# SegataLab/metamlst

Hardware: AMD Instinct MI355X
Metric: Mreads/s aligned+ST-typed, metamlstDB_2022; ST concordance vs CPU ref (higher is better)
Workload: dtype int32

## Files before the change

include/mlst.h:

```cpp
#ifndef MLST_H
#define MLST_H

#include <stdint.h>

#ifdef __cplusplus
extern "C" {
#endif

#define MLST_OK              0
#define MLST_E_INVALID      -1
#define MLST_E_NOGPU        -2
#define MLST_E_HIP          -3
#define MLST_E_CAPACITY     -4
#define MLST_E_LIMIT        -5

typedef struct mlst_handle mlst_handle;

typedef struct mlst_params {
    int32_t minscore;
    int32_t max_xm;
    int32_t min_read_len;
    int32_t minqual;
    int32_t mincov;
    int32_t match_bonus;
// ... 77 lines not shown
                           uint32_t words_per_read, uint32_t qual_stride);

int mlst_submit_packed_device(mlst_handle* h, const uint32_t* d_packed, const uint8_t* d_qual_rows,
                              const uint16_t* d_lens, uint64_t n_reads,
                              uint32_t words_per_read, uint32_t qual_stride, int paired);

int mlst_get_allele_stats(mlst_handle* h, int64_t* sum_score, uint32_t* n_hits,
                          uint64_t* locus_read_len_sum, uint64_t* locus_first_read,
                          uint64_t* counters);

int mlst_stats_flat_sizes(mlst_handle* h, uint64_t* n_sum, uint64_t* n_min);
int mlst_export_stats_device(mlst_handle* h, int64_t* d_sum, int64_t* d_min);
int mlst_import_stats_device(mlst_handle* h, const int64_t* d_sum, const int64_t* d_min);

int mlst_pileup(mlst_handle* h, const uint32_t* chosen_allele_idx, uint32_t n, uint32_t* counts);
int mlst_pileup_device(mlst_handle* h, const uint32_t* chosen_allele_idx, uint32_t n,
                       uint32_t* d_counts , uint64_t* n_cols);
int mlst_set_depth_cap(mlst_handle* h, uint32_t cap);

int mlst_consensus(mlst_handle* h, const uint32_t* chosen_allele_idx, uint32_t n, uint32_t mincov,
                   char none_char, uint8_t* out_seq, uint32_t* counts);

int mlst_consensus_from_counts_device(mlst_handle* h, const uint32_t* d_counts, uint64_t n_cols, uint32_t mincov,
                                      char none_char, uint8_t* out_seq);

int mlst_pileup_alignments(mlst_handle* h, const uint32_t* chosen_allele_idx, uint32_t n_chosen, uint64_t n_rec,
                           const uint32_t* rec_allele, const int32_t* rec_pos0, const int32_t* rec_as, const int32_t* rec_xm,
                           const uint64_t* cigar_off, const uint32_t* cigar, const uint64_t* seq_off,
                           const uint8_t* seq, const uint8_t* qual, int32_t minscore, int32_t max_xm, int32_t minqual,
                           uint32_t* counts);

int mlst_alignments_export(mlst_handle* h, const uint32_t* chosen_allele_idx, uint32_t n,
                           uint64_t* n_rec_out, uint64_t* n_cigar_out, uint64_t* n_bases_out);
int mlst_alignments_fetch(mlst_handle* h, uint64_t* read_index, uint32_t* rec_allele, int32_t* rec_pos0, int32_t* rec_as,
                          int32_t* rec_xm, int32_t* rec_diag, uint8_t* rec_flags ,
                          uint64_t* cigar_off , uint32_t* cigar, uint64_t* seq_off ,
                          uint8_t* seq, uint8_t* qual);

int mlst_alignments_text_open(mlst_handle* h, const uint8_t* names, const uint64_t* name_off , int paired,
                              uint64_t round_bytes );
int mlst_alignments_text_next(mlst_handle* h, uint8_t* text, uint64_t cap, uint64_t* n_bytes, uint64_t* n_records, int* done);
int mlst_alignments_text_close(mlst_handle* h);

int mlst_reads_text_open(mlst_handle* h, int paired, uint64_t round_bytes );
int mlst_reads_text_next(mlst_handle* h, uint8_t* text, uint64_t cap, uint64_t* n_bytes, uint64_t* n_reads, int* done);
int mlst_reads_text_close(mlst_handle* h);

int mlst_set_read_names(mlst_handle* h, int on);
int mlst_get_read_names(mlst_handle* h, int* on);
int mlst_read_names_info(mlst_handle* h, uint64_t out[4]);
int mlst_read_names_fetch(mlst_handle* h, uint64_t* read_index , uint64_t* off , uint8_t* bytes);

typedef struct { uint32_t trim5, trim3, trim_qual, phred_base; } mlst_read_prep;
int mlst_set_read_prep(mlst_handle* h, const mlst_read_prep* p);
int mlst_get_read_prep(mlst_handle* h, mlst_read_prep* out);
int mlst_read_prep_info(mlst_handle* h, uint64_t out[4]);

int mlst_set_read_adapters(mlst_handle* h, const char* adapters, uint32_t min_overlap, uint32_t error_permille);
int mlst_get_read_adapters(mlst_handle* h, char* adapters, uint64_t cap, uint32_t* min_overlap, uint32_t* error_permille);
int mlst_get_read_adapters_info(mlst_handle* h, uint64_t out[12]);

int mlst_set_export_md(mlst_handle* h, int on);
int mlst_get_export_md(mlst_handle* h, int* on);

int mlst_bam_open(mlst_handle* h, int pass, const int32_t* ref_allele, const int32_t* ref_locus, const uint8_t* ref_flags, uint32_t n_ref,
                  uint32_t skip_bytes, const uint32_t* chosen_allele_idx, uint32_t n_chosen);
int mlst_submit_bam_bgzf(mlst_handle* h, const uint8_t* data, uint64_t n_bytes, int final_chunk, uint64_t* n_records_out, uint64_t* n_consumed_out);
int mlst_bam_set_capacity(mlst_handle* h, uint64_t max_entries);
int mlst_bam_pileup_fetch(mlst_handle* h, uint32_t* counts);

int mlst_sam_open(mlst_handle* h, int pass, const uint8_t* names, const uint64_t* name_off ,
                  const int32_t* ref_allele, const int32_t* ref_locus, const uint8_t* ref_flags, uint32_t n_ref,
                  const uint32_t* chosen_allele_idx, uint32_t n_chosen);
int mlst_submit_sam_text(mlst_handle* h, const uint8_t* text, uint64_t n_bytes, int final_chunk, uint64_t* n_records_out);

int mlst_bam_reads_open(mlst_handle* h, uint32_t n_ref, uint32_t skip_bytes, int paired);
int mlst_bam_reads_info(mlst_handle* h, uint64_t out[4]);

int mlst_submit_fasta(mlst_handle* h, const uint8_t* text, uint64_t n_bytes, uint32_t read_len, uint32_t stride, uint32_t min_len,
                      uint64_t* n_contigs_out, uint64_t* n_reads_out);

int mlst_typing_layout(mlst_handle* h, uint64_t* colbase , uint64_t* total_cols);
int mlst_typing_enqueue(mlst_handle* h, int32_t penalty, uint32_t mincov, char none_char);
int mlst_typing_choose_pileup(mlst_handle* h, int32_t penalty, uint32_t* d_counts);
int mlst_typing_finish(mlst_handle* h, uint32_t mincov, char none_char, const uint32_t* d_counts);
int mlst_typing_choose_pileup_compact(mlst_handle* h, int32_t penalty, uint32_t* d_counts, uint64_t cap_cols);
int mlst_typing_finish_compact(mlst_handle* h, uint32_t mincov, char none_char, const uint32_t* d_counts);
int mlst_typing_compact_info(mlst_handle* h, uint64_t* need_cols, uint32_t* overflow);
int mlst_typing_fetch(mlst_handle* h, int64_t* sum_score, uint32_t* n_hits, uint64_t* locus_read_len_sum,
                      uint64_t* locus_first_read, uint64_t* counters, int32_t* chosen, uint8_t* letters);
int mlst_typing_wait(mlst_handle* h);
int mlst_typing_fetch_waited(mlst_handle* h, int64_t* sum_score, uint32_t* n_hits, uint64_t* locus_read_len_sum,
                             uint64_t* locus_first_read, uint64_t* counters, int32_t* chosen, uint8_t* letters);
long long mlst_round_tenths(long long p, uint32_t q);

int mlst_hamming_le(mlst_handle* h, uint32_t locus, const uint8_t* query, uint32_t len,
                    uint32_t z, int32_t* first_allele_idx, uint32_t* n_within);
int mlst_hamming_all(mlst_handle* h, uint32_t locus, const uint8_t* query, uint32_t len,
                     uint32_t* dist);

int mlst_msa_align(mlst_handle* h, const uint8_t* seqs, const uint64_t* off , uint32_t n, uint32_t* center_out, uint32_t* width_out);
int mlst_msa_fetch(mlst_handle* h, uint8_t* rows );

int mlst_set_read_index_base(mlst_handle* h, uint64_t base);

int mlst_reset_sample(mlst_handle* h);

typedef struct mlst_item {
    uint64_t read_index;
    uint32_t locus;
    int32_t  diag;
    uint16_t strand;
    uint16_t votes;
    uint32_t reserved;
} mlst_item;
int mlst_get_items(mlst_handle* h, mlst_item* out, uint64_t cap, uint64_t* n);

int mlst_set_stream(mlst_handle* h, void* stream);
int mlst_set_cu_partition(mlst_handle* h, uint32_t part, uint32_t n_parts);
int mlst_get_stream(mlst_handle* h, void** stream);
int mlst_busy(mlst_handle* h);
int mlst_export_stats_device_async(mlst_handle* h, int64_t* d_sum, int64_t* d_min);
int mlst_import_stats_device_async(mlst_handle* h, const int64_t* d_sum, const int64_t* d_min);

int mlst_set_profiling(mlst_handle* h, int on);
int mlst_get_kernel_time(mlst_handle* h, int which, double* total_ms, uint64_t* launches);
int mlst_reset_kernel_time(mlst_handle* h);
int mlst_get_index_bytes(mlst_handle* h, uint64_t out[4]);
int mlst_get_sieve_info(mlst_handle* h, uint64_t out[4]);
int mlst_get_extend_info(mlst_handle* h, uint64_t out[8]);
int mlst_synchronize(mlst_handle* h);

#ifdef __cplusplus
}
#endif
#endif
```

metamlst_amd/csrc/mlst_engine.hip:

```cpp
#include <hip/hip_runtime.h>
#include <algorithm>
#include <cmath>
#include <cstdarg>
#include <cstdio>
#include <cstdlib>
#include <cstring>
#include <cstddef>
#include <functional>
#include <atomic>
#include <memory>
#include <mutex>
#include <string>
#include <thread>
#include <vector>
#include <chrono>
#include <unistd.h>

#include "mlst.h"
#include "mlst_debug.h"
#include "bgzf_host.h"
#include "inflate_dev.h"
#include "inflate_wave.h"
#include "inflate_lane.h"
#include "inflate_canon.h"
// ... 3079 lines not shown
        else if (i < 2 * nA) E.n_hits[i - nA] = (u32)d_sum[i];
        else if (i < 2 * nA + nL) E.locus_len[i - 2 * nA] = (u64)d_sum[i];
        else if (i < total) E.ctr->cnt[i - 2 * nA - nL] = (u64)d_sum[i];
        else { u64 l = i - total; long long f = d_min[l]; E.locus_first[l] = f == 0x7FFFFFFFFFFFFFFFll ? 0xFFFFFFFFFFFFFFFFull : (u64)f; }
    }
}
__global__ void k_fill_u64(u64* p, u64 n, u64 v) {
    for (u64 i = (u64)blockIdx.x * blockDim.x + threadIdx.x; i < n; i += (u64)gridDim.x * blockDim.x) p[i] = v;
}

#include "bam_dev.h"
#include "sam_dev.h"
#include "bam_reads.h"
#include "fasta_dev.h"
#include "fastq_tile.h"
#include "bam_tile.h"
#include "msa_dev.h"
#include "aln_export.h"
#include "read_names.h"
#include "read_prep.h"
#include "read_adapt.h"
#include "aln_text.h"
#include "reads_text.h"

struct EvPair { hipEvent_t a, b; int which; };

struct mlst_handle {
    int device = 0;
    hipStream_t stream = nullptr;
    mlst_params prm;
    KParams kp;
    std::string err;
    std::vector<LocusDev> loci;
    std::vector<u64> aoff;
    u32 n_alleles = 0, n_loci = 0;
    std::vector<u32> allele_locus;
    u32* d_arena = nullptr; u32* d_planes = nullptr; u32* d_nmask = nullptr; u16* d_allele_len = nullptr; u32* d_allele_locus = nullptr;
    LocusDev* d_loci = nullptr; uint4* d_sieve = nullptr; u32* d_bitmap = nullptr; u32* d_gbitmap = nullptr; u64* d_keys = nullptr; u32* d_vals = nullptr; u32* d_posts = nullptr;
    int* d_floor = nullptr; u8* d_pen = nullptr; u8* d_ascii = nullptr; u64* d_aoff = nullptr;
    HapRec* d_hap_rec = nullptr; u32* d_hap_blk = nullptr; u32* d_hap_id = nullptr; u64 bytes_hap = 0, n_hap_rec = 0; u32 hap_win_max[2] = {0, 0}, hap_loci = 0;
    u32 ext_lds_recs[2] = {0, 0};
    u32 ext_acc_cap = 0;
    u8* h_qc = nullptr; u8* d_qc = nullptr; u64 cap_hostq = 0, cap_qc = 0;
    u64* d_acc64 = nullptr;
    u32* d_xrec[2] = {nullptr, nullptr}; u64 cap_xrec[2] = {0, 0};
    u64 bytes_arena = 0, bytes_sieve = 0, bytes_table = 0; double bitmap_fill = 0.0;
    EngineDev E; EngineDev* d_E = nullptr;
    bool have_ref = false, have_state = false;
    u32* d_cand = nullptr; u64 cap_cand = 0;
    int sieve_kind = 0; u32 sieve_chain = 0; u64 n_keys = 0;
    u32* d_rfilter = nullptr; u32* d_rt_arena = nullptr; u64 cap_rt_arena = 0; u32* d_rt_counts = nullptr; u32* d_rt_emitted = nullptr; u64 cap_rt_emitted = 0;
    u32 rt_prod = 0, rt_cap = 0, rt_tiles_max = 0, rt_nw = 16, rt_pf = 2, rt_exam = RT_EXAM_DEFAULT, rt_wo = 1; u64 rt_slice = 0;
    u64* d_rt_parked = nullptr; u64 cap_rt_parked = 0;
    u64* d_rt_trace = nullptr; bool rt_trace_on = false; const void* rt_last_packed = nullptr;
    std::vector<void*> dbg_pads;
    u32* d_bin_flags = nullptr; u64 cap_bin_flags = 0;
    u8* d_in_bases = nullptr; u8* d_in_quals = nullptr; u64* d_in_off = nullptr; u64 cap_in_bytes = 0, cap_in_reads = 0;
    u32* d_packed = nullptr; u8* d_qrows = nullptr; u16* d_lens = nullptr; u64 cap_packed_words = 0, cap_qrow_bytes = 0, cap_lens = 0;
    u64 reads_seen = 0;
    u32 max_wpr = 0;
    int ext_threads = 64, ext_blocks = 5120;
    int extp_threads = 256, extp_blocks = 1792; u32 pair_loci = 0;
    int sieve_g_blocks = 256 * 5;
    u8* d_fq_text = nullptr;
    u32* d_fq_blk = nullptr; u64 cap_fq_blk = 0;
    u8* d_bgzf = nullptr; u64 cap_bgzf = 0; void* d_bgzf_blk = nullptr; u64 cap_bgzf_blk = 0; u8* d_fq_carry = nullptr; u64 cap_fq_carry = 0, fq_carry_len = 0;
    u64* d_fq_lines = nullptr; u64 cap_fq_lines = 0; u64* d_fq_soff = nullptr; u64* d_fq_qoff = nullptr; u64 cap_fq_reads = 0; u64* d_fq_meta = nullptr;
    int* d_locus_chosen = nullptr; u64* d_locus_colbase = nullptr; u64* d_pl_list = nullptr; u8* d_tb = nullptr;
    u32* d_itok = nullptr; u32* d_intok = nullptr; u64 cap_itok_blocks = 0; int inflate_mode = 0;
    u64 dbg_infl_blocks = 0, dbg_infl_left = 0; bool dbg_infl_known = false;
    struct BlkList { BgzfBlk* d = nullptr; BgzfBlk* h = nullptr; u64 cap = 0; };
    struct BzSlot { BlkList blk; hipEvent_t ev_copied = nullptr, ev_inflated = nullptr; u32* d_err = nullptr; u32* h_err = nullptr; };
    BzSlot bz[2]; int bz_slot = 0, bz_mode = -1; hipStream_t infl_stream = nullptr;
    bool bgzf_verify = false; struct { u32* d_out = nullptr; hipEvent_t e0 = nullptr, e1 = nullptr; } crc_hook;
    enum { BZ_SUB = 8 };
    struct BzChunk { u8* d = nullptr; u64 cap = 0; hipEvent_t ev[BZ_SUB] = {}; u64 upto[BZ_SUB] = {}; int n_ev = 0; hipEvent_t ev_used = nullptr; bool used = false; };
    BzChunk bzc[2]; int bz_chunk = 0;
    struct { bool on = false, counted = false; int slot = 0, tslot = 0, paired = 0; u64 text_bytes = 0; u32 blk_base = 0 ; } bz_pend;
    u8* d_pc[2] = {nullptr, nullptr}; u64 cap_pc[2] = {0, 0}, pc_len[2] = {0, 0}; bool pair_open = false; u64* d_pr_meta = nullptr;
    struct BzPair { bool on = false, counted = false; int slot = 0, tslot = 0; u32 nblk1 = 0; u64 base[2] = {0, 0}, head[2] = {0, 0}, text[2] = {0, 0}; } bzp;
    u32 depth_cap = 0; u64* d_capbuf = nullptr; u64 cap_capcols = 0;
    u32* d_counts = nullptr; u64 cap_counts = 0;
    int* d_allele_no = nullptr; int* d_auto_chosen = nullptr; u64* d_fixed_colbase = nullptr; std::vector<u64> fixed_colbase; u64 fixed_cols = 0;
    u32* d_auto_counts = nullptr; u8* d_auto_letters = nullptr; bool auto_pending = false;
    u8* h_tstats[2] = {nullptr, nullptr}; u8* h_tauto[2] = {nullptr, nullptr}; int t_slot = 0, t_last = 0, t_ready = -1;
    u64* d_compact_colbase = nullptr; int* d_compact_chosen = nullptr; u64* d_compact_info = nullptr; u64 off_compact_info = 0; bool compact_pending = false;
    hipStream_t copy_stream = nullptr; hipEvent_t stage_done = nullptr;
    u8* d_fq_slot[2] = {nullptr, nullptr}; u64 cap_fq_slot[2] = {0, 0}; hipEvent_t ev_packed[2] = {nullptr, nullptr}; int fq_slot = 0;
    u32* d_fq_nl[2] = {nullptr, nullptr};
    int cu_split = 1, cu_part = 0;
    hipStream_t own_stream = nullptr;
    u32* d_dist = nullptr; u8* d_query = nullptr; u64 cap_dist = 0, cap_query = 0;
    u8* d_stats = nullptr; u8* h_stats = nullptr; u64 stats_bytes = 0, stats_zero_bytes = 0;
    u64 off_sum = 0, off_len = 0, off_ctr = 0, off_hits = 0, off_first = 0;
    u8* h_pin = nullptr; u64 cap_pin = 0;
    bool profiling = false;
    bool window = false;
    struct GraphSlot { hipGraphExec_t exec = nullptr; std::vector<u64> sig; };
    GraphSlot g_submit, g_typing; bool use_graphs = true;
    std::vector<EvPair> events;
    std::vector<hipEvent_t> ev_pool;
    double k_ms[20] = {0}; u64 k_n[20] = {0};
    double wall_khz = 100000.0;
    struct BamStream* bam = nullptr;
    u32 bam_force_miss = 0; u64 bam_max_entries = 0;
    struct { u64 n_reads = 0; u32 wpr = 0, qstride = 0; } last_pack;
    struct { FaDev* d_desc = nullptr; FaMeta* d_meta = nullptr; u8* h_fa = nullptr; u8* d_flat = nullptr; u64 cap_flat = 0;
             u32* d_kind = nullptr; u64* d_cseq = nullptr; u64* d_chdr = nullptr; u64 cap_cells = 0; u64* d_cstart = nullptr; u64* d_wcnt = nullptr; u64 cap_contigs = 0;
             u64 last_cells = 0, last_contigs = 0; u32 last_passes = 0; } fa;
    struct { u32 read_len = 0, stride = 0; u64 round = 16ull << 20; u64 info[4] = {0, 0, 0, 0};
             FqtDev* d_desc = nullptr; FqtMeta* d_meta = nullptr; u8* h_fqt = nullptr; u64* d_rlen = nullptr; u64* d_wex = nullptr; u64 cap_recs = 0;
             u64* d_gsum = nullptr; u64 cap_groups = 0; u64* d_soff = nullptr; u64* d_qoff = nullptr; u64 cap_win = 0; } tile;
    struct { u64 batch_bytes = 1ull << 30; bool done = false; u32 n = 0, width = 0;
             u8* d_seq = nullptr; u64 cap_seq = 0; u64* d_off = nullptr; u64 cap_off = 0; u16* d_tab = nullptr; u64 cap_tab = 0;
             u32* d_slot = nullptr; u8* d_end = nullptr; u64 cap_end = 0; u32* d_tb = nullptr; u64 cap_tb = 0; u8* d_rows = nullptr; u64 cap_rows = 0;
             u32* h_width = nullptr; } msa;
    struct { bool done = false; u64 n_rec = 0, n_cig = 0, n_seq = 0; int* d_lc = nullptr; u64 cap_lc = 0; AxItem* d_meta = nullptr; u64* d_dp = nullptr;
             u64* d_off = nullptr; u64 cap_items = 0; u64* d_gs = nullptr; u64 cap_groups = 0; u8* d_desc = nullptr; u8* h_tot = nullptr;
             u8* d_out = nullptr; u64 cap_out = 0; AxOut out; } ax;
    struct AtState { bool open = false, ready = false, with_names = false, md = false, with_md = false, reads = false; u64 max_reads = 0; u16* d_mdw = nullptr; size_t next = 0; std::vector<AtRound> rounds; u64 round_bytes = 0, round_recs = 0, max_pairs = 0;
             u32* d_perm = nullptr; u64* d_pair_off = nullptr; u32* d_item_read = nullptr; u64* d_read_first = nullptr; u8* d_names = nullptr; u64* d_name_off = nullptr;
             AtPair* d_meta = nullptr; AtRead* d_reads = nullptr; u64* d_wex = nullptr; u64* d_gsum = nullptr; u64* d_dp = nullptr; u8* d_desc = nullptr;
             u8* d_text = nullptr; u64 cap_text = 0; u8* h_tot = nullptr; } at;
    struct { bool on = false; u64 want_bytes = 256ull << 20; RnCtr* d_ctr = nullptr; u8* d_bytes = nullptr; u64 cap_bytes = 0; u64* d_off = nullptr; u16* d_len = nullptr;
             RnSrc src = {nullptr, nullptr, 0}; } rn;
    struct { bool on = false; RpSet set = {0, 0, 0, 33}; RpCtr* d_ctr = nullptr; } rp;
    struct { bool on = false; RaSet set = {}; std::string text; RaCtr* d_ctr = nullptr; } ra;
};

static std::string g_create_err;

static int fail(mlst_handle* h, int code, const char* fmt, ...) {
    char buf[512]; va_list ap; va_start(ap, fmt); vsnprintf(buf, sizeof buf, fmt, ap); va_end(ap);
    if (h) h->err = buf; else g_create_err = buf;
    return code;
}
#define HIPCHK(h, call) do { hipError_t e_ = (call); if (e_ != hipSuccess) return fail(h, MLST_E_HIP, "%s: %s", #call, hipGetErrorString(e_)); } while (0)

static int bz_flush(mlst_handle* h);
static int bzp_finish(mlst_handle* h, bool whole, uint64_t* n_reads_out);
static void bz_free(mlst_handle* h);
static int bam_flush(mlst_handle* h);
static void bam_drop(mlst_handle* h, bool release);
static bool bam_is_open(const mlst_handle* h);
static int rn_refuse(mlst_handle* h, const char* entry);
static int rp_refuse(mlst_handle* h, const char* entry);
static int ra_refuse(mlst_handle* h, const char* entry);
static void at_free(mlst_handle* h);
static const char* bam_kind(const mlst_handle* h);
template <typename T> static hipError_t dmalloc(T** p, u64 n) { return hipMalloc((void**)p, (n ? n : 1) * sizeof(T)); }
template <typename T> static hipError_t dmalloc(GP<T>* p, u64 n) { return hipMalloc((void**)&p->p, (n ? n : 1) * sizeof(T)); }

static hipEvent_t ev_get(mlst_handle* h) {
    if (!h->ev_pool.empty()) { hipEvent_t e = h->ev_pool.back(); h->ev_pool.pop_back(); return e; }
    hipEvent_t e; if (hipEventCreateWithFlags(&e, hipEventDisableSystemFence) != hipSuccess) hipEventCreate(&e); return e;
}
__global__ void k_nop() {}
struct Prof {
    mlst_handle* h; int which; hipEvent_t a = nullptr, b = nullptr;
    Prof(mlst_handle* h_, int w) : h(h_), which(w) {
        if (h->profiling) { a = ev_get(h); b = ev_get(h); hipLaunchKernelGGL(k_nop, dim3(1), dim3(64), 0, h->stream); hipEventRecord(a, h->stream); }
    }
    ~Prof() { if (h->profiling) { hipEventRecord(b, h->stream); h->events.push_back({a, b, which}); } }
};
static void drain_events(mlst_handle* h) {
    if (h->events.empty()) return;
    hipStreamSynchronize(h->stream);
    for (auto& e : h->events) { float ms = 0; hipEventElapsedTime(&ms, e.a, e.b); h->k_ms[e.which] += ms; h->k_n[e.which]++; h->ev_pool.push_back(e.a); h->ev_pool.push_back(e.b); }
    h->events.clear();
}

static int graph_enter(mlst_handle* h, mlst_handle::GraphSlot& g, const std::vector<u64>& sig) {
    if (!h->use_graphs || h->profiling || h->stream != h->own_stream) return 0;
    if (g.exec && g.sig == sig) return hipGraphLaunch(g.exec, h->stream) == hipSuccess ? 1 : 0;
    if (g.exec) { hipGraphExecDestroy(g.exec); g.exec = nullptr; }
    if (g.sig != sig) { g.sig = sig; return 0; }
    if (hipStreamBeginCapture(h->stream, hipStreamCaptureModeThreadLocal) != hipSuccess) { h->use_graphs = false; return 0; }
    return 2;
}
static int graph_leave(mlst_handle* h, mlst_handle::GraphSlot& g) {
    hipGraph_t graph = nullptr;
    if (hipStreamEndCapture(h->stream, &graph) != hipSuccess || !graph) { h->use_graphs = false; return fail(h, MLST_E_HIP, "hipStreamEndCapture failed"); }
    hipError_t e = hipGraphInstantiate(&g.exec, graph, nullptr, nullptr, 0);
    hipGraphDestroy(graph);
    if (e != hipSuccess) { g.exec = nullptr; h->use_graphs = false; return fail(h, MLST_E_HIP, "hipGraphInstantiate: %s", hipGetErrorString(e)); }
    HIPCHK(h, hipGraphLaunch(g.exec, h->stream));
    return MLST_OK;
}

extern "C" void mlst_default_params(mlst_params* p) {
    memset(p, 0, sizeof *p);
    p->minscore = MLST_DEF_MINSCORE; p->max_xm = MLST_DEF_MAX_XM; p->min_read_len = MLST_DEF_MIN_READ_LEN;
    p->minqual = MLST_DEF_MINQUAL; p->mincov = MLST_DEF_MINCOV; p->match_bonus = MLST_DEF_MATCH_BONUS;
    p->mm_max = MLST_DEF_MM_MAX; p->mm_min = MLST_DEF_MM_MIN; p->n_penalty = MLST_DEF_N_PENALTY;
    p->gap_open = MLST_DEF_GAP_OPEN; p->gap_ext = MLST_DEF_GAP_EXT; p->gbar = MLST_DEF_GBAR; p->band_w = MLST_DEF_BAND_W;
    p->gap_trigger_mm = MLST_DEF_GAP_TRIGGER_MM; p->xm_field_quirk = MLST_DEF_XM_FIELD_QUIRK; p->gap_trigger_clip = MLST_DEF_GAP_TRIGGER_CLIP;
    p->minscore_const = MLST_DEF_MINSCORE_CONST; p->minscore_coef = MLST_DEF_MINSCORE_COEF;
}

extern "C" const char* mlst_last_error(const mlst_handle* h) { return h ? h->err.c_str() : g_create_err.c_str(); }

extern "C" int mlst_create(int device, const mlst_params* p, mlst_handle** out) {
    if (!out) return fail(nullptr, MLST_E_INVALID, "out is NULL");
    *out = nullptr;
    int ndev = 0;
    if (hipGetDeviceCount(&ndev) != hipSuccess || ndev <= 0)
        return fail(nullptr, MLST_E_NOGPU, "no HIP device visible: this library has no CPU path");
    if (device < 0 || device >= ndev) return fail(nullptr, MLST_E_INVALID, "device %d out of range (%d devices)", device, ndev);
    mlst_params prm; if (p) prm = *p; else mlst_default_params(&prm);
    if (prm.band_w < 1 || prm.band_w > MAX_W) return fail(nullptr, MLST_E_INVALID, "band_w must be in 1..%d", MAX_W);
    if (prm.max_xm > 254 || prm.minscore > 1000) return fail(nullptr, MLST_E_INVALID, "max_xm/minscore out of range");
    if (prm.match_bonus < 1 || prm.match_bonus > 127) return fail(nullptr, MLST_E_INVALID, "match_bonus must be in 1..127");
    {
        const int pmin = std::min(prm.n_penalty, prm.mm_min), gap1 = prm.gap_open + prm.gap_ext;
        if (pmin < 0 || prm.mm_max < prm.mm_min || prm.gap_open < 0 || prm.gap_ext < 0) return fail(nullptr, MLST_E_INVALID, "penalties must not be negative, mm_max not below mm_min");
        if (prm.match_bonus * MLST_MAX_READ_LEN >= 1024)
            return fail(nullptr, MLST_E_LIMIT, "match_bonus %d: the score of a %d-base read does not fit 10 bits", prm.match_bonus, MLST_MAX_READ_LEN);
        if (prm.match_bonus > 4 * pmin)
            return fail(nullptr, MLST_E_LIMIT, "match_bonus %d against a cheapest mismatch of %d: xm of a %d-base read does not fit 8 bits", prm.match_bonus, pmin, MLST_MAX_READ_LEN);
        if (5 * prm.match_bonus > 2 * gap1)
            return fail(nullptr, MLST_E_LIMIT, "match_bonus %d against a one-base gap of %d: xo of a %d-base read does not fit 7 bits", prm.match_bonus, gap1, MLST_MAX_READ_LEN);
    }
    if (!prm.max_retained_reads) prm.max_retained_reads = 4ull << 20;
    if (!prm.max_items) prm.max_items = 8ull << 20;
    if (prm.max_items >= (1ull << 32)) return fail(nullptr, MLST_E_INVALID, "max_items must be below 2^32");
    if (!prm.max_pair_results) prm.max_pair_results = 256ull << 20;
    mlst_handle* h = new mlst_handle();
    h->device = device; h->prm = prm;
    if (hipSetDevice(device) != hipSuccess) { delete h; return fail(nullptr, MLST_E_HIP, "cannot initialise device %d", device); }
    if (hipStreamCreate(&h->stream) != hipSuccess) { delete h; return fail(nullptr, MLST_E_HIP, "cannot initialise device %d", device); }
    h->own_stream = h->stream;
    { const char* g = getenv("MLST_GRAPHS"); if (g && g[0] == '0') h->use_graphs = false; }
    { const char* g = getenv("MLST_BGZF_CRC"); h->bgzf_verify = g && g[0] == '1'; }
    { const char* g = getenv("MLST_MSA_BATCH_BYTES"); if (g && atoll(g) > 0) h->msa.batch_bytes = (u64)atoll(g); }
    { const char* g = getenv("MLST_TILE_ROUND"); if (g && atoll(g) > 0) h->tile.round = (u64)atoll(g); }
    { const char* g = getenv("MLST_NAMES_BYTES"); if (g && atoll(g) > 0) h->rn.want_bytes = (u64)atoll(g); }
    { int khz = 0; if (hipDeviceGetAttribute(&khz, hipDeviceAttributeWallClockRate, device) == hipSuccess && khz > 0) h->wall_khz = (double)khz; }
    KParams& k = h->kp;
    k.minscore = prm.minscore; k.max_xm = prm.max_xm; k.min_read_len = prm.min_read_len; k.minqual = prm.minqual;
    k.match_bonus = prm.match_bonus; k.n_penalty = prm.n_penalty;
    k.open_p = ((prm.gap_open + prm.gap_ext) << MLST_P_SHIFT) + (1 << 8); k.ext_p = prm.gap_ext << MLST_P_SHIFT;
    k.gbar = prm.gbar; k.band_w = prm.band_w; k.trig = prm.gap_trigger_mm; k.quirk = prm.xm_field_quirk; k.clip = prm.gap_trigger_clip;
    memset(&h->E, 0, sizeof h->E);
    *out = h;
    return MLST_OK;
}

static void free_ref(mlst_handle* h) {
    hipFree(h->d_arena); hipFree(h->d_planes); hipFree(h->d_nmask); hipFree(h->d_allele_len); hipFree(h->d_allele_locus); hipFree(h->d_loci);
    hipFree(h->d_sieve); hipFree(h->d_bitmap); h->d_bitmap = nullptr; hipFree(h->d_gbitmap); h->d_gbitmap = nullptr; hipFree(h->d_keys); hipFree(h->d_vals); hipFree(h->d_posts); hipFree(h->d_floor); hipFree(h->d_pen);
    hipFree(h->d_ascii); hipFree(h->d_aoff);
    hipFree(h->d_hap_rec); hipFree(h->d_hap_blk); hipFree(h->d_hap_id); h->d_hap_rec = nullptr; h->d_hap_blk = nullptr; h->d_hap_id = nullptr;
    hipFree(h->d_rfilter); h->d_rfilter = nullptr;
    hipFree(h->d_allele_no); hipFree(h->d_auto_chosen); hipFree(h->d_fixed_colbase); hipFree(h->d_auto_counts); hipFree(h->d_auto_letters);
    hipFree(h->d_compact_colbase); hipFree(h->d_compact_chosen); hipFree(h->d_compact_info); h->d_compact_colbase = nullptr; h->d_compact_chosen = nullptr; h->d_compact_info = nullptr;
    for (int k = 0; k < 2; k++) if (h->h_tauto[k]) { hipHostFree(h->h_tauto[k]); h->h_tauto[k] = nullptr; }
    h->d_allele_no = h->d_auto_chosen = nullptr; h->d_fixed_colbase = nullptr; h->d_auto_counts = nullptr; h->d_auto_letters = nullptr; h->auto_pending = false;
    h->d_arena = h->d_planes = h->d_nmask = nullptr; h->d_allele_len = nullptr; h->d_allele_locus = nullptr; h->d_loci = nullptr; h->d_sieve = nullptr;
    h->d_keys = nullptr; h->d_vals = h->d_posts = nullptr; h->d_floor = nullptr; h->d_pen = nullptr; h->d_ascii = nullptr; h->d_aoff = nullptr;
    h->have_ref = false;
}
static void free_state(mlst_handle* h) {
    EngineDev& E = h->E;
    hipFree(h->d_bin_flags); h->d_bin_flags = nullptr; h->cap_bin_flags = 0;
    hipFree(h->d_rt_arena); hipFree(h->d_rt_counts); hipFree(h->d_rt_emitted); hipFree(h->d_rt_trace); h->d_rt_trace = nullptr;
    hipFree(h->d_rt_parked); h->d_rt_parked = nullptr; h->cap_rt_parked = 0;
    for (void* q : h->dbg_pads) hipFree(q);
    h->dbg_pads.clear();
    h->d_rt_arena = nullptr; h->d_rt_counts = nullptr; h->d_rt_emitted = nullptr; h->cap_rt_arena = 0; h->cap_rt_emitted = 0; h->rt_prod = 0;
    hipFree(h->d_E); h->d_E = nullptr;
    hipFree(h->d_stats); h->d_stats = nullptr; if (h->h_stats) { hipHostFree(h->h_stats); h->h_stats = nullptr; }
    for (int k = 0; k < 2; k++) if (h->h_tstats[k]) { hipHostFree(h->h_tstats[k]); h->h_tstats[k] = nullptr; }
    hipFree(E.ret_bases); hipFree(E.ret_quals); hipFree(E.ret_len); hipFree(E.ret_ridx); hipFree(E.ret_nrec);
    hipFree(E.ret_mate); hipFree(E.ret_item0); hipFree(E.ret_nitems); hipFree(E.ret_cpos); E.ret_mate = nullptr; E.ret_item0 = nullptr; E.ret_nitems = nullptr; E.ret_cpos = nullptr;
    hipFree(E.items); hipFree(E.item_state); hipFree(E.res); hipFree(E.dp_list);
    for (int k = 0; k < 2; k++) { hipFree(h->d_xrec[k]); h->d_xrec[k] = nullptr; h->cap_xrec[k] = 0; }
    hipFree(h->d_acc64); h->d_acc64 = nullptr;
    hipFree(h->rn.d_ctr); hipFree(h->rn.d_bytes); hipFree(h->rn.d_off); hipFree(h->rn.d_len);
    h->rn.d_ctr = nullptr; h->rn.d_bytes = nullptr; h->rn.d_off = nullptr; h->rn.d_len = nullptr; h->rn.cap_bytes = 0;
    hipFree(h->d_qc); h->d_qc = nullptr; h->cap_qc = 0; if (h->h_qc) { hipHostFree(h->h_qc); h->h_qc = nullptr; h->cap_hostq = 0; }
    hipFree(h->d_locus_chosen); hipFree(h->d_locus_colbase); hipFree(h->d_pl_list); hipFree(h->d_tb);
    hipFree(h->d_capbuf); h->d_capbuf = nullptr; h->cap_capcols = 0;
    hipFree(h->d_itok); hipFree(h->d_intok); h->d_itok = nullptr; h->d_intok = nullptr; h->cap_itok_blocks = 0;
    E.sum_score = nullptr; E.n_hits = nullptr; E.locus_len = E.locus_first = nullptr; E.ctr = nullptr; E.ret_bases = nullptr; E.ret_quals = nullptr;
    E.ret_len = nullptr; E.ret_ridx = nullptr; E.ret_nrec = nullptr; E.items = nullptr; E.item_state = nullptr; E.res = nullptr; E.dp_list = nullptr;
    h->d_locus_chosen = nullptr; h->d_locus_colbase = nullptr; h->d_pl_list = nullptr; h->d_tb = nullptr;
    h->have_state = false;
}

extern "C" void mlst_destroy(mlst_handle* h) {
    if (!h) return;
    hipSetDevice(h->device);
    if (h->stream) hipStreamSynchronize(h->stream);
    bz_free(h);
    bam_drop(h, true);
    for (auto& e : h->events) { hipEventDestroy(e.a); hipEventDestroy(e.b); }
    for (auto& e : h->ev_pool) hipEventDestroy(e);
    free_ref(h); free_state(h);
    if (h->h_pin) hipHostFree(h->h_pin);
    for (int k = 0; k < 2; k++) { if (h->ev_packed[k]) hipEventDestroy(h->ev_packed[k]); }
    if (h->stage_done) hipEventDestroy(h->stage_done);
    if (h->copy_stream) hipStreamDestroy(h->copy_stream);
    hipFree(h->d_cand); hipFree(h->d_in_bases); hipFree(h->d_in_quals); hipFree(h->d_in_off);
    hipFree(h->d_fq_slot[0]); hipFree(h->d_fq_slot[1]); hipFree(h->d_fq_nl[0]); hipFree(h->d_fq_nl[1]); hipFree(h->d_fq_blk); hipFree(h->d_fq_lines); hipFree(h->d_fq_soff); hipFree(h->d_fq_qoff); hipFree(h->d_fq_meta);
    hipFree(h->d_pc[0]); hipFree(h->d_pc[1]); hipFree(h->d_pr_meta); hipFree(h->rp.d_ctr); hipFree(h->ra.d_ctr);
    hipFree(h->fa.d_desc); hipFree(h->fa.d_meta); hipFree(h->fa.d_flat); hipFree(h->fa.d_kind); hipFree(h->fa.d_cseq); hipFree(h->fa.d_chdr); hipFree(h->fa.d_cstart); hipFree(h->fa.d_wcnt);
    if (h->fa.h_fa) hipHostFree(h->fa.h_fa);
    hipFree(h->tile.d_desc); hipFree(h->tile.d_meta); hipFree(h->tile.d_rlen); hipFree(h->tile.d_wex); hipFree(h->tile.d_gsum); hipFree(h->tile.d_soff); hipFree(h->tile.d_qoff);
    if (h->tile.h_fqt) hipHostFree(h->tile.h_fqt);
    hipFree(h->msa.d_seq); hipFree(h->msa.d_off); hipFree(h->msa.d_tab); hipFree(h->msa.d_slot); hipFree(h->msa.d_end); hipFree(h->msa.d_tb); hipFree(h->msa.d_rows);
    if (h->msa.h_width) hipHostFree(h->msa.h_width);
    hipFree(h->ax.d_lc); hipFree(h->ax.d_meta); hipFree(h->ax.d_dp); hipFree(h->ax.d_off); hipFree(h->ax.d_gs); hipFree(h->ax.d_desc); hipFree(h->ax.d_out);
    if (h->ax.h_tot) hipHostFree(h->ax.h_tot);
    at_free(h); hipFree(h->at.d_text); hipFree(h->at.d_desc); if (h->at.h_tot) hipHostFree(h->at.h_tot);
    hipFree(h->d_bgzf); hipFree(h->d_bgzf_blk); hipFree(h->d_fq_carry); h->d_bgzf = nullptr; h->d_bgzf_blk = nullptr; h->d_fq_carry = nullptr; h->cap_bgzf = h->cap_bgzf_blk = h->cap_fq_carry = h->fq_carry_len = 0;
    hipFree(h->d_packed); hipFree(h->d_qrows); hipFree(h->d_lens); hipFree(h->d_counts); hipFree(h->d_dist); hipFree(h->d_query);
    for (auto* g : {&h->g_submit, &h->g_typing}) if (g->exec) hipGraphExecDestroy(g->exec);
    if (h->own_stream) hipStreamDestroy(h->own_stream);
    delete h;
}

static inline int base_code(u8 c) {
    switch (c) { case 'A': case 'a': return 0; case 'C': case 'c': return 1; case 'G': case 'g': return 2; case 'T': case 't': return 3; default: return 4; }
}

static int reset_sample_state(mlst_handle* h) {
    HIPCHK(h, hipMemsetAsync(h->d_stats, 0, h->stats_zero_bytes, h->stream));
    HIPCHK(h, hipMemsetAsync(h->d_stats + h->off_first, 0xFF, h->stats_bytes - h->off_first, h->stream));
    if (h->d_acc64 && h->n_alleles) HIPCHK(h, hipMemsetAsync(h->d_acc64, 0, (u64)h->n_alleles * 8, h->stream));
    if (h->rn.d_ctr) HIPCHK(h, hipMemsetAsync(h->rn.d_ctr, 0, sizeof(RnCtr), h->stream));
    if (h->rp.d_ctr) HIPCHK(h, hipMemsetAsync(h->rp.d_ctr, 0, sizeof(RpCtr), h->stream));
    if (h->ra.d_ctr) HIPCHK(h, hipMemsetAsync(h->ra.d_ctr, 0, sizeof(RaCtr), h->stream));
    h->reads_seen = 0; h->fq_carry_len = 0; h->max_wpr = 0;
    h->last_pack.n_reads = 0; h->last_pack.wpr = h->last_pack.qstride = 0;
    for (u64& x : h->tile.info) x = 0;
    h->pc_len[0] = h->pc_len[1] = 0; h->pair_open = false;
    bam_drop(h, false);
    h->at.open = false;
    return MLST_OK;
}

struct HostIndex {
    std::vector<LocusDev> loci; std::vector<u16> alen;
    std::vector<u32> arena, nmask, planes;
    std::vector<HapRec> hap_rec; std::vector<u32> hap_blk; std::vector<u32> hap_id;
    u32 hap_win_max[2] = {0, 0}; u32 hap_loci = 0;
    std::vector<u64> tkeys; std::vector<u32> tvals, posts; u32 tmask = 0;
    std::vector<u16> sv; u64 nb = 0; u32 smask = 0, sieve_chain = 0;
    std::vector<u32> bitmap; double bitmap_fill = 0.0;
    std::vector<u32> gbitmap; u32 gbits = 0;
    std::vector<u32> rfilter;
    u64 n_keys = 0; u32 n_loci = 0; int kind = 0;
    std::string err; int err_code = 0;
};
enum { MLST_SIEVE_LDS = 0, MLST_SIEVE_GLOBAL = 1, MLST_SIEVE_ROUTED = 3 };
struct KP { u64 key; u32 post; };

static u64 fnv1a(const void* p, u64 n, u64 hsh) {
    const u8* b = (const u8*)p; u64 i = 0;
    for (; i + 8 <= n; i += 8) { u64 v; memcpy(&v, b + i, 8); hsh = (hsh ^ v) * 0x100000001B3ull; hsh ^= hsh >> 29; }
    for (; i < n; i++) hsh = (hsh ^ b[i]) * 0x100000001B3ull;
    return hsh;
}

static std::shared_ptr<HostIndex> build_host_index(const uint8_t* ascii, const uint64_t* off, const uint32_t* locus_id,
                                                   const uint32_t* species_id, uint32_t n_alleles, int want_kind) {
    auto H = std::make_shared<HostIndex>();
    auto bad = [&](int code, const char* fmt, ...) { char buf[256]; va_list ap; va_start(ap, fmt); vsnprintf(buf, sizeof buf, fmt, ap); va_end(ap); H->err = buf; H->err_code = code; return H; };
    u32 n_loci = 0;
    for (u32 a = 0; a < n_alleles; a++) {
        if (locus_id[a] > MLST_MAX_LOCI) return bad(MLST_E_LIMIT, "locus id %u exceeds %d", locus_id[a], MLST_MAX_LOCI);
        n_loci = std::max(n_loci, locus_id[a] + 1);
        if (off[a + 1] - off[a] > MLST_MAX_ALLELE_LEN) return bad(MLST_E_LIMIT, "allele %u longer than %d", a, MLST_MAX_ALLELE_LEN);
    }
    H->n_loci = n_loci;
    std::vector<LocusDev>& loci = H->loci; loci.resize(n_loci); for (auto& L : loci) memset(&L, 0, sizeof L);
    std::vector<char> seen(n_loci, 0);
    for (u32 a = 0; a < n_alleles; a++) {
        LocusDev& L = loci[locus_id[a]];
        if (!seen[locus_id[a]]) { seen[locus_id[a]] = 1; L.a_begin = a; L.species = species_id ? species_id[a] : 0; }
        else if (L.a_begin + L.n_alleles != a) return bad(MLST_E_INVALID, "alleles of locus %u are not contiguous", locus_id[a]);
        L.n_alleles++; L.max_len = std::max(L.max_len, (u32)(off[a + 1] - off[a]));
    }
    u64 arena_words = 0, nmask_words = 0, plane_words = 0;
    std::vector<u16>& alen = H->alen; alen.resize(n_alleles);
    for (u32 a = 0; a < n_alleles; a++) alen[a] = (u16)(off[a + 1] - off[a]);
    for (auto& L : loci) {
        if (L.n_alleles >= (1u << 20)) return bad(MLST_E_LIMIT, "locus with %u alleles exceeds 2^20", L.n_alleles);
        L.n_pad = (L.n_alleles + 63) & ~63u; L.words = (L.max_len + 15) / 16 + 2; L.nwords = (L.max_len + 31) / 32 + 1;
        if ((u64)L.words * L.n_pad * 4 >= (1ull << 32)) return bad(MLST_E_LIMIT, "a locus arena exceeds 4 GB");
        L.arena_off = arena_words; arena_words += (u64)L.words * L.n_pad;
        L.pblocks = (L.max_len + 31) / 32 + 1; L.plane_off = plane_words; plane_words += (u64)L.pblocks * 2 * L.n_pad;
    }
    std::vector<u32>& arena = H->arena; std::vector<u32>& planes = H->planes;
    arena.assign(arena_words ? arena_words : 1, 0); planes.assign(plane_words ? plane_words : 1, 0);
    if (planes.size() * 4 >= (1ull << 32)) return bad(MLST_E_LIMIT, "allele bit-plane arena exceeds 4 GB (32-bit offsets in k_extend)");
    std::vector<std::vector<KP>> lkp(n_loci);
    std::vector<std::vector<std::pair<u32, u32>>> lnpos(n_loci);
    std::vector<std::vector<HapRec>> lhrec(n_loci); std::vector<std::vector<u32>> lhblk(n_loci); std::vector<std::vector<u32>> lhid(n_loci);
    {
        unsigned nthr = std::thread::hardware_concurrency(); if (nthr < 1) nthr = 1; if (nthr > 64) nthr = 64; if (nthr > n_loci) nthr = n_loci ? n_loci : 1;
        std::atomic<u32> next(0);
        auto work = [&]() {
            std::vector<u8> code; std::vector<u64> prev;
            struct HK { HapRec r; u32 al; };
            std::vector<HK> hk; std::vector<std::pair<u64, u32>> nmv;
            for (;;) {
                const u32 l = next.fetch_add(1); if (l >= n_loci) break;
                const LocusDev& L = loci[l]; std::vector<KP>& out = lkp[l];
                prev.assign(L.max_len + 1, ~0ull);
                for (u32 a = L.a_begin; a < L.a_begin + L.n_alleles; a++) {
                    const u32 al = a - L.a_begin, len = alen[a];
// ... 254 lines not shown
    {
        u64 key[5];
        key[3] = n_alleles; key[4] = off[n_alleles];
        key[0] = fnv1a(off, ((u64)n_alleles + 1) * 8, 0xCBF29CE484222325ull ^ n_alleles);
        key[1] = fnv1a(ascii, off[n_alleles], fnv1a(locus_id, (u64)n_alleles * 4, 0x9E3779B97F4A7C15ull));
        key[2] = (u64)(want_kind + 2);
        for (const char* v : {"MLST_GBM_BITS"}) { const char* e = getenv(v); if (e) key[2] = fnv1a(e, strlen(e), key[2]); }
        if (species_id) key[2] = fnv1a(species_id, (u64)n_alleles * 4, key[2]);
        std::lock_guard<std::mutex> lk(g_index_mu);
        const char* nocache = getenv("MLST_INDEX_CACHE");
        if (nocache && nocache[0] == '0') g_index_last.reset();
        if (g_index_last && memcmp(g_index_key, key, sizeof key) == 0) HI = g_index_last;
        else {
            std::string rc_path; { std::lock_guard<std::mutex> lk2(g_refcache_mu); rc_path = g_refcache_path; }
            if (!rc_path.empty()) HI = refcache_load(rc_path, key);
            if (!HI) {
                HI = build_host_index(ascii, off, locus_id, species_id, n_alleles, want_kind);
                if (HI->err_code) return fail(h, HI->err_code, "%s", HI->err.c_str());
                if (!rc_path.empty()) refcache_store(rc_path, key, *HI);
            }
            if (!(nocache && nocache[0] == '0')) { g_index_last = HI; memcpy(g_index_key, key, sizeof key); }
        }
    }
    const u32 n_loci = HI->n_loci; h->n_loci = n_loci;
    const std::vector<LocusDev>& loci = HI->loci; const std::vector<u16>& alen = HI->alen;
    const std::vector<u32>&arena = HI->arena, &nmask = HI->nmask, &planes = HI->planes, &posts = HI->posts, &tvals = HI->tvals, &bitmap = HI->bitmap, &gbitmap = HI->gbitmap;
    const std::vector<u64>& tkeys = HI->tkeys; const std::vector<u16>& sv = HI->sv;
    const u64 tcap = tkeys.size(), nb = HI->nb; const u32 tmask = HI->tmask, smask = HI->smask, gbits = HI->gbits;
    h->allele_locus.assign(locus_id, locus_id + n_alleles);
    h->sieve_kind = HI->kind; h->sieve_chain = HI->sieve_chain; h->n_keys = HI->n_keys;
    std::vector<int> floor_tab(MLST_MAX_READ_LEN + 1);
    for (int n = 0; n <= MLST_MAX_READ_LEN; n++) {
        double f = h->prm.minscore_const + h->prm.minscore_coef * log((double)(n > 0 ? n : 1));
        long v = (long)f; if (v < 0) v = 0; floor_tab[n] = (int)v;
    }
    std::vector<u8> pen_tab(256);
    for (int q = 0; q < 256; q++) { int qq = q > 40 ? 40 : q; pen_tab[q] = (u8)(h->prm.mm_min + ((h->prm.mm_max - h->prm.mm_min) * qq) / 40); }
    HIPCHK(h, dmalloc(&h->d_arena, arena.size())); HIPCHK(h, hipMemcpy(h->d_arena, arena.data(), arena.size() * 4, hipMemcpyHostToDevice));
    HIPCHK(h, dmalloc(&h->d_planes, planes.size())); HIPCHK(h, hipMemcpy(h->d_planes, planes.data(), planes.size() * 4, hipMemcpyHostToDevice));
    HIPCHK(h, dmalloc(&h->d_nmask, nmask.size())); HIPCHK(h, hipMemcpy(h->d_nmask, nmask.data(), nmask.size() * 4, hipMemcpyHostToDevice));
    HIPCHK(h, dmalloc(&h->d_allele_len, (u64)n_alleles)); HIPCHK(h, hipMemcpy(h->d_allele_len, alen.data(), (u64)n_alleles * 2, hipMemcpyHostToDevice));
    HIPCHK(h, dmalloc(&h->d_allele_locus, (u64)n_alleles)); HIPCHK(h, hipMemcpy(h->d_allele_locus, locus_id, (u64)n_alleles * 4, hipMemcpyHostToDevice));
    HIPCHK(h, dmalloc(&h->d_loci, (u64)n_loci)); HIPCHK(h, hipMemcpy(h->d_loci, loci.data(), (u64)n_loci * sizeof(LocusDev), hipMemcpyHostToDevice));
    HIPCHK(h, dmalloc(&h->d_sieve, nb)); HIPCHK(h, hipMemcpy(h->d_sieve, sv.data(), nb * 16, hipMemcpyHostToDevice));
    if (!bitmap.empty()) { HIPCHK(h, dmalloc(&h->d_bitmap, (u64)bitmap.size())); HIPCHK(h, hipMemcpy(h->d_bitmap, bitmap.data(), bitmap.size() * 4, hipMemcpyHostToDevice)); }
    if (!HI->rfilter.empty()) { HIPCHK(h, dmalloc(&h->d_rfilter, (u64)HI->rfilter.size())); HIPCHK(h, hipMemcpy(h->d_rfilter, HI->rfilter.data(), HI->rfilter.size() * 4, hipMemcpyHostToDevice)); }
    if (!gbitmap.empty()) { HIPCHK(h, dmalloc(&h->d_gbitmap, (u64)gbitmap.size())); HIPCHK(h, hipMemcpy(h->d_gbitmap, gbitmap.data(), gbitmap.size() * 4, hipMemcpyHostToDevice)); }
    HIPCHK(h, dmalloc(&h->d_keys, tcap)); HIPCHK(h, hipMemcpy(h->d_keys, tkeys.data(), tcap * 8, hipMemcpyHostToDevice));
    HIPCHK(h, dmalloc(&h->d_vals, tcap)); HIPCHK(h, hipMemcpy(h->d_vals, tvals.data(), tcap * 4, hipMemcpyHostToDevice));
    HIPCHK(h, dmalloc(&h->d_posts, (u64)posts.size())); if (!posts.empty()) HIPCHK(h, hipMemcpy(h->d_posts, posts.data(), posts.size() * 4, hipMemcpyHostToDevice));
    HIPCHK(h, dmalloc(&h->d_floor, (u64)floor_tab.size())); HIPCHK(h, hipMemcpy(h->d_floor, floor_tab.data(), floor_tab.size() * 4, hipMemcpyHostToDevice));
    HIPCHK(h, dmalloc(&h->d_pen, (u64)256)); HIPCHK(h, hipMemcpy(h->d_pen, pen_tab.data(), 256, hipMemcpyHostToDevice));
    u64 abytes = off[n_alleles];
    HIPCHK(h, dmalloc(&h->d_ascii, abytes)); if (abytes) HIPCHK(h, hipMemcpy(h->d_ascii, ascii, abytes, hipMemcpyHostToDevice));
    HIPCHK(h, dmalloc(&h->d_aoff, (u64)n_alleles + 1)); HIPCHK(h, hipMemcpy(h->d_aoff, off, ((u64)n_alleles + 1) * 8, hipMemcpyHostToDevice));
    HIPCHK(h, dmalloc(&h->d_hap_rec, (u64)HI->hap_rec.size())); HIPCHK(h, hipMemcpy(h->d_hap_rec, HI->hap_rec.data(), HI->hap_rec.size() * sizeof(HapRec), hipMemcpyHostToDevice));
    HIPCHK(h, dmalloc(&h->d_hap_blk, (u64)HI->hap_blk.size())); HIPCHK(h, hipMemcpy(h->d_hap_blk, HI->hap_blk.data(), HI->hap_blk.size() * 4, hipMemcpyHostToDevice));
    HIPCHK(h, dmalloc(&h->d_hap_id, (u64)HI->hap_id.size())); HIPCHK(h, hipMemcpy(h->d_hap_id, HI->hap_id.data(), HI->hap_id.size() * 4, hipMemcpyHostToDevice));
    h->bytes_hap = HI->hap_rec.size() * sizeof(HapRec) + HI->hap_blk.size() * 4 + HI->hap_id.size() * 4; h->n_hap_rec = HI->hap_rec.size();
    h->hap_win_max[0] = HI->hap_win_max[0]; h->hap_win_max[1] = HI->hap_win_max[1]; h->hap_loci = HI->hap_loci;
    h->bytes_arena = arena.size() * 4 + planes.size() * 4 + nmask.size() * 4; h->bytes_sieve = nb * 16 + bitmap.size() * 4 + gbitmap.size() * 4 + HI->rfilter.size() * 4; h->bytes_table = tcap * 12 + posts.size() * 4;
    h->aoff.assign(off, off + n_alleles + 1);
    {
        HIPCHK(h, dmalloc(&h->d_allele_no, (u64)n_alleles)); HIPCHK(h, hipMemcpy(h->d_allele_no, allele_no, (u64)n_alleles * 4, hipMemcpyHostToDevice));
        h->fixed_colbase.assign(n_loci + 1, 0);
        for (u32 l = 0; l < n_loci; l++) h->fixed_colbase[l + 1] = h->fixed_colbase[l] + loci[l].max_len;
        h->fixed_cols = h->fixed_colbase[n_loci];
        HIPCHK(h, dmalloc(&h->d_fixed_colbase, (u64)n_loci + 1)); HIPCHK(h, hipMemcpy(h->d_fixed_colbase, h->fixed_colbase.data(), ((u64)n_loci + 1) * 8, hipMemcpyHostToDevice));
        HIPCHK(h, dmalloc(&h->d_auto_chosen, (u64)n_loci));
        HIPCHK(h, dmalloc(&h->d_auto_counts, h->fixed_cols * 4 + 4)); HIPCHK(h, dmalloc(&h->d_auto_letters, h->fixed_cols + 16));
        h->off_compact_info = (((u64)n_loci * 4 + 15) & ~15ull) + ((h->fixed_cols + 15) & ~15ull);
        for (int k = 0; k < 2; k++) { if (h->h_tauto[k]) hipHostFree(h->h_tauto[k]); HIPCHK(h, hipHostMalloc((void**)&h->h_tauto[k], h->off_compact_info + 64, hipHostMallocDefault)); }
        HIPCHK(h, dmalloc(&h->d_compact_colbase, (u64)n_loci + 1)); HIPCHK(h, dmalloc(&h->d_compact_chosen, (u64)n_loci + 1)); HIPCHK(h, dmalloc(&h->d_compact_info, 2));
    }
    EngineDev& E = h->E;
    E.arena = h->d_arena; E.planes = h->d_planes; E.nmask = h->d_nmask; E.allele_len = h->d_allele_len; E.allele_locus = h->d_allele_locus; E.loci = h->d_loci;
    h->bitmap_fill = HI->bitmap_fill;
    E.sieve = h->d_sieve; E.sieve_mask = smask; E.bitmap = h->d_bitmap; E.gbitmap = h->d_gbitmap; E.gbitmap_bits = gbitmap.empty() ? 0 : gbits; E.keys = h->d_keys; E.vals = h->d_vals; E.posts = h->d_posts; E.table_mask = tmask;
    E.floor_tab = h->d_floor; E.pen_tab = h->d_pen; E.n_alleles = n_alleles; E.n_loci = n_loci;
    E.hap_rec = h->d_hap_rec; E.hap_blk = h->d_hap_blk; E.hap_id = h->d_hap_id;
    E.cap_ret = h->prm.max_retained_reads; E.cap_items = h->prm.max_items; E.cap_res = h->prm.max_pair_results; E.cap_dp = h->prm.max_items * 4;
    {
        u64 o = 0;
        h->off_sum = o; o += (u64)n_alleles * 8;
        h->off_len = o; o += (u64)n_loci * 8;
        h->off_ctr = o; o += (sizeof(Counters) + 7) & ~7ull;
        h->off_hits = o; o += ((u64)n_alleles * 4 + 7) & ~7ull;
        h->stats_zero_bytes = o;
        h->off_first = o; o += (u64)n_loci * 8;
        h->stats_bytes = o ? o : 8;
        HIPCHK(h, dmalloc(&h->d_stats, h->stats_bytes));
        HIPCHK(h, hipHostMalloc((void**)&h->h_stats, h->stats_bytes, hipHostMallocDefault));
        for (int k = 0; k < 2; k++) { if (h->h_tstats[k]) hipHostFree(h->h_tstats[k]); HIPCHK(h, hipHostMalloc((void**)&h->h_tstats[k], h->stats_bytes, hipHostMallocDefault)); }
        h->t_slot = 0; h->t_ready = -1;
        E.sum_score = (long long*)(h->d_stats + h->off_sum); E.locus_len = (u64*)(h->d_stats + h->off_len);
        E.ctr = (Counters*)(h->d_stats + h->off_ctr); E.n_hits = (u32*)(h->d_stats + h->off_hits);
        E.locus_first = (u64*)(h->d_stats + h->off_first);
    }
    HIPCHK(h, dmalloc(&E.ret_bases, E.cap_ret * RW)); HIPCHK(h, dmalloc(&E.ret_quals, E.cap_ret * RQ));
    HIPCHK(h, dmalloc(&E.ret_len, E.cap_ret)); HIPCHK(h, dmalloc(&E.ret_ridx, E.cap_ret)); HIPCHK(h, dmalloc(&E.ret_nrec, E.cap_ret));
    HIPCHK(h, dmalloc(&E.ret_mate, E.cap_ret)); HIPCHK(h, dmalloc(&E.ret_item0, E.cap_ret)); HIPCHK(h, dmalloc(&E.ret_nitems, E.cap_ret)); HIPCHK(h, dmalloc(&E.ret_cpos, E.cap_ret));
    HIPCHK(h, dmalloc(&E.items, E.cap_items)); HIPCHK(h, dmalloc(&E.item_state, E.cap_items)); HIPCHK(h, dmalloc(&E.res, E.cap_res)); HIPCHK(h, dmalloc(&E.dp_list, E.cap_dp));
    HIPCHK(h, dmalloc(&h->d_locus_colbase, (u64)n_loci * 2 + 2));
    HIPCHK(h, dmalloc(&h->d_pl_list, E.cap_items));
    HIPCHK(h, dmalloc(&h->d_tb, (u64)64 * 64 * MLST_MAX_READ_LEN * (2 * MAX_W + 1)));
    HIPCHK(h, dmalloc(&h->d_acc64, (u64)n_alleles)); HIPCHK(h, hipMemset(h->d_acc64, 0, (u64)(n_alleles ? n_alleles : 1) * 8)); E.acc64 = h->d_acc64;
    HIPCHK(h, dmalloc(&h->d_E, (u64)1)); HIPCHK(h, hipMemcpy(h->d_E, &h->E, sizeof(EngineDev), hipMemcpyHostToDevice));
    {
        u32 hap_max = 512; const char* e0 = getenv("MLST_EXT_HAP_MAX"); if (e0 && atoi(e0) >= 0) hap_max = (u32)atoi(e0);
        u32 budget_kb = 96; const char* e4 = getenv("MLST_EXT_LDS_KB"); if (e4 && atoi(e4) >= 0 && atoi(e4) <= 150) budget_kb = (u32)atoi(e4);
        std::vector<LocusDev> lc = loci;
        u32 mx_hap = 0, mx_pair = 0, n_hap = 0, n_pair = 0; h->hap_win_max[0] = h->hap_win_max[1] = 0;
        for (auto& L : lc) {
            const bool take = L.hap_ok && L.n_alleles <= hap_max && (u64)L.hap_win[1] * 16 <= (u64)budget_kb * 1024;
            L.hap_ok = take ? 1u : 0u;
            if (take) { n_hap++; mx_hap = std::max(mx_hap, L.n_alleles); for (int k = 0; k < 2; k++) h->hap_win_max[k] = std::max(h->hap_win_max[k], L.hap_win[k]); }
            else { n_pair++; mx_pair = std::max(mx_pair, L.n_alleles); }
        }
        h->loci = lc; h->hap_loci = n_hap; h->pair_loci = n_pair;
        HIPCHK(h, hipMemcpy(h->d_loci, lc.data(), (u64)n_loci * sizeof(LocusDev), hipMemcpyHostToDevice));
        int thr = mx_hap <= 512 ? 64 : 256;
        const char* e1 = getenv("MLST_EXT_THREADS"); if (e1 && atoi(e1) >= 64 && atoi(e1) <= 1024 && atoi(e1) % 64 == 0) thr = atoi(e1);
        int blocks = 1280 * 256 / thr;
        const char* e2 = getenv("MLST_EXT_BLOCKS"); if (e2 && atoi(e2) > 0) blocks = atoi(e2);
        h->ext_threads = thr; h->ext_blocks = blocks;
        int thr2 = mx_pair <= 512 ? 64 : 256;
        const char* e5 = getenv("MLST_EXTP_THREADS"); if (e5 && atoi(e5) >= 64 && atoi(e5) <= 1024 && atoi(e5) % 64 == 0) thr2 = atoi(e5);
        int blocks2 = 1792 * 256 / thr2;
        const char* e6 = getenv("MLST_EXTP_BLOCKS"); if (e6 && atoi(e6) > 0) blocks2 = atoi(e6);
        h->extp_threads = thr2; h->extp_blocks = blocks2;
        h->ext_acc_cap = std::min<u32>((mx_hap + 63u) & ~63u, 16384u);
        for (int k = 0; k < 2; k++) {
            h->ext_lds_recs[k] = h->hap_win_max[k];
            if (ext_lds_bytes(h, k) > 48u * 1024u)
                HIPCHK(h, hipFuncSetAttribute(k ? (const void*)k_extend_320 : (const void*)k_extend_160, hipFuncAttributeMaxDynamicSharedMemorySize, (int)ext_lds_bytes(h, k)));
        }
        const char* e3 = getenv("MLST_SIEVE_BLOCKS"); if (e3 && atoi(e3) > 0) h->sieve_g_blocks = atoi(e3);
        const char* e7 = getenv("MLST_RT_SLICE"); h->rt_slice = (e7 && atoll(e7) > 0) ? (u64)atoll(e7) : 0;
    }
    h->have_ref = h->have_state = true;
    int rc = reset_sample_state(h); if (rc) return rc;
    HIPCHK(h, hipStreamSynchronize(h->stream));
    return MLST_OK;
}

extern "C" int mlst_set_read_index_base(mlst_handle* h, uint64_t base) {
    if (!h || !h->have_state) return fail(h, MLST_E_INVALID, "no reference loaded");
    h->reads_seen = base;
    return MLST_OK;
}

extern "C" int mlst_reset_sample(mlst_handle* h) {
    if (!h || !h->have_state) return fail(h, MLST_E_INVALID, "no reference loaded");
    hipSetDevice(h->device);
    drain_events(h);
    if (h->bz_pend.on || h->bzp.on) { if (h->infl_stream) hipStreamSynchronize(h->infl_stream); h->bz_pend.on = false; h->bzp.on = false; }
    return reset_sample_state(h);
}

static int grid_for(u64 n_units, int per_block, int cap = 2048) {
    u64 g = (n_units + per_block - 1) / per_block; if (g < 1) g = 1; if (g > (u64)cap) g = cap; return (int)g;
}
static void zero_words(mlst_handle* h, void* p, u64 n_words) {
    if (!n_words) return;
    hipLaunchKernelGGL(k_zero, dim3(grid_for((n_words + 255) / 256, 1, 1024)), dim3(256), 0, h->stream, (u32*)p, n_words);
}

extern "C" int mlst_pack_reads_device(mlst_handle* h, const uint8_t* d_bases, const uint8_t* d_quals, const uint64_t* d_off,
                                      uint64_t n_reads, uint32_t* d_packed, uint8_t* d_qrows, uint16_t* d_lens,
                                      uint32_t wpr, uint32_t qstride) {
    if (!h) return MLST_E_INVALID;
    hipSetDevice(h->device);
    if (wpr == 0 || wpr > RW || (wpr & 1)) return fail(h, MLST_E_INVALID, "words_per_read must be even and in 2..%d", RW);
    if (qstride < 4 || qstride > RQ || (qstride & 3)) return fail(h, MLST_E_INVALID, "qual_stride must be a multiple of 4 in 4..%d", RQ);
    if (((uintptr_t)d_qrows & 3) != 0) return fail(h, MLST_E_INVALID, "quality rows must be 4-byte aligned");
    if (n_reads == 0) return MLST_OK;
    Prof pf(h, 6);
    hipLaunchKernelGGL(k_pack, dim3(grid_for((n_reads + 63) / 64, 1, 8192)), dim3(256), 0, h->stream, d_bases, d_quals, (const u64*)d_off, (u64)n_reads,
                       d_packed, d_qrows, d_lens, wpr, qstride);
    HIPCHK(h, hipGetLastError());
    return MLST_OK;
}

static int ensure_route_buffers(mlst_handle* h, u64 n_reads, u32 wpr, u64 n_reads_flags = 0) {
    u32 nw = 16;
    { const char* e = getenv("MLST_ROUTE_WAVES"); if (e && atoi(e) == 8) nw = 8; }
    { const char* e = getenv("MLST_ROUTE_WRITEOUT"); h->rt_wo = (e && e[0] == '0' && e[1] == 0) ? 0u : 1u; }
    { const char* e = getenv("MLST_PROBE_PF"); h->rt_pf = (e && atoi(e) == 4) ? 4u : 2u; }
    { const char* e = getenv("MLST_PROBE_EXAM_WAVES"); const int v = e ? atoi(e) : RT_EXAM_DEFAULT; h->rt_exam = (v == 0 || v == 1 || v == 2 || v == 4) ? (u32)v : (u32)RT_EXAM_DEFAULT; }
    const u64 tile = (u64)nw * 64, n_tiles = (n_reads + tile - 1) / tile;
    u32 prod = (wpr <= 10 ? 512u : 256u) * (16u / nw) / (u32)h->cu_split;
    { const char* e = getenv("MLST_ROUTE_BLOCKS"); if (e && atoi(e) > 0) prod = (u32)atoi(e); }
    if (prod > RT_MAXP) prod = RT_MAXP;
    if (prod > n_tiles) prod = (u32)(n_tiles ? n_tiles : 1);
    u64 tiles_max = (n_tiles + prod - 1) / prod * 3 / 2 + 8;
    u64 cap = (u64)((double)tiles_max * ((double)tile / 256.0 * (wpr - 1) + 0.15 * nw + 2.0) * 1.25) + 256; cap = (cap + 31) & ~31ull;
    if (h->rt_prod == prod && h->rt_nw == nw && h->rt_cap >= cap && h->rt_tiles_max >= tiles_max) { cap = h->rt_cap; tiles_max = h->rt_tiles_max; }
    if (cap >= (1ull << 31) || tiles_max > 0xFFFFull || (u64)RT_OWNERS * prod * (cap / 16) >= (1ull << 32)) return fail(h, MLST_E_LIMIT, "batch too large for the routed sieve (%llu tiles per producer workgroup)", (unsigned long long)tiles_max);
    const u64 need = (u64)RT_OWNERS * prod * cap;
    if (h->cap_rt_arena < need || h->rt_prod != prod || h->rt_cap != (u32)cap) {
        hipStreamSynchronize(h->stream);
        if (h->cap_rt_arena < need) { hipFree(h->d_rt_arena); h->d_rt_arena = nullptr; HIPCHK(h, dmalloc(&h->d_rt_arena, need)); h->cap_rt_arena = need; }
        hipFree(h->d_rt_counts); h->d_rt_counts = nullptr; HIPCHK(h, dmalloc(&h->d_rt_counts, (u64)RT_OWNERS * prod));
        h->rt_prod = prod; h->rt_cap = (u32)cap;
    }
    const u64 need_e = (u64)prod * (tiles_max + 1);
    if (h->cap_rt_emitted < need_e) { hipStreamSynchronize(h->stream); hipFree(h->d_rt_emitted); h->d_rt_emitted = nullptr; HIPCHK(h, dmalloc(&h->d_rt_emitted, need_e)); h->cap_rt_emitted = need_e; }
    h->rt_tiles_max = (u32)tiles_max; h->rt_nw = nw;
    if (h->rt_trace_on && !h->d_rt_trace) { hipStreamSynchronize(h->stream); HIPCHK(h, dmalloc(&h->d_rt_trace, (u64)(RT_MAXP + RT_OWNERS) * 4)); HIPCHK(h, hipMemsetAsync(h->d_rt_trace, 0, (u64)(RT_MAXP + RT_OWNERS) * 32, h->stream)); }
    const u64 need_p = std::max<u64>(n_reads / 4, 1ull << 16);
    if (h->cap_rt_parked < need_p) { hipStreamSynchronize(h->stream); hipFree(h->d_rt_parked); h->d_rt_parked = nullptr; HIPCHK(h, dmalloc(&h->d_rt_parked, need_p)); h->cap_rt_parked = need_p; }
    const u64 n_flag_words = ((n_reads_flags > n_reads ? n_reads_flags : n_reads) + 31) >> 5;
    if (h->cap_bin_flags < n_flag_words) { hipStreamSynchronize(h->stream); hipFree(h->d_bin_flags); h->d_bin_flags = nullptr; HIPCHK(h, dmalloc(&h->d_bin_flags, n_flag_words)); h->cap_bin_flags = n_flag_words;
                                            HIPCHK(h, hipMemsetAsync(h->d_bin_flags, 0, n_flag_words * 4, h->stream)); }
    return MLST_OK;
}

static int submit_impl(mlst_handle* h, const uint32_t* d_packed, const uint8_t* d_qrows, const uint16_t* d_lens,
                       uint64_t n_reads, uint32_t wpr, uint32_t qstride, int paired, int phase);
extern "C" int mlst_submit_packed_device(mlst_handle* h, const uint32_t* d_packed, const uint8_t* d_qrows, const uint16_t* d_lens,
                                         uint64_t n_reads, uint32_t wpr, uint32_t qstride, int paired) {
    { int rc_ = rn_refuse(h, "mlst_submit_packed_device"); if (rc_) return rc_; }
    { int rc_ = rp_refuse(h, "mlst_submit_packed_device"); if (rc_) return rc_; }
    { int rc_ = ra_refuse(h, "mlst_submit_packed_device"); if (rc_) return rc_; }
    return submit_impl(h, d_packed, d_qrows, d_lens, n_reads, wpr, qstride, paired, 0);
}
static int submit_impl(mlst_handle* h, const uint32_t* d_packed, const uint8_t* d_qrows, const uint16_t* d_lens,
                       uint64_t n_reads, uint32_t wpr, uint32_t qstride, int paired, int phase) {
    if (!h || !h->have_state) return fail(h, MLST_E_INVALID, "no reference loaded");
    hipSetDevice(h->device);
    if (wpr == 0 || wpr > RW || (wpr & 1)) return fail(h, MLST_E_INVALID, "words_per_read must be even and in 2..%d", RW);
    if (qstride < 4 || qstride > RQ || (qstride & 3)) return fail(h, MLST_E_INVALID, "qual_stride must be a multiple of 4 in 4..%d", RQ);
    if (phase != 1 && (!d_qrows || ((uintptr_t)d_qrows & 3) != 0)) return fail(h, MLST_E_INVALID, "quality rows must be 4-byte aligned");
    if (n_reads >= (1ull << 32)) return fail(h, MLST_E_LIMIT, "a batch holds at most 2^32-1 reads");
    if (((uintptr_t)d_packed & 15) != 0) return fail(h, MLST_E_INVALID, "packed rows must be 16-byte aligned");
    if (n_reads == 0) return MLST_OK;
    paired = paired ? 1 : 0;
    if (paired && ((n_reads | h->reads_seen) & 1ull)) return fail(h, MLST_E_INVALID, "paired submissions hold whole pairs (reads 2k, 2k+1) and start at an even read index");
    if (h->cap_cand < n_reads) { hipStreamSynchronize(h->stream); hipFree(h->d_cand); h->d_cand = nullptr; HIPCHK(h, dmalloc(&h->d_cand, n_reads)); h->cap_cand = n_reads; }
    EngineDev& E = h->E;
    if (wpr > h->max_wpr) h->max_wpr = wpr;
    u64 rt_slice = 0;
    if (h->sieve_kind == MLST_SIEVE_ROUTED && h->rt_slice) { rt_slice = (h->rt_slice + 1023) & ~1023ull; if (rt_slice >= n_reads) rt_slice = 0; }
    if (h->sieve_kind == MLST_SIEVE_ROUTED) { int rc = ensure_route_buffers(h, rt_slice ? rt_slice : n_reads, wpr, n_reads); if (rc) return rc; }
    {
        const int k = wpr <= 10 ? 0 : 1; const u64 words = k ? (u64)XRec<RW / 2>::WORDS : (u64)XRec<5>::WORDS;
        if (h->hap_loci && !h->d_xrec[k]) { hipStreamSynchronize(h->stream); HIPCHK(h, dmalloc(&h->d_xrec[k], h->E.cap_items * words)); h->cap_xrec[k] = h->E.cap_items; }
    }
    const int gs = phase ? 0 : graph_enter(h, h->g_submit, {(u64)(uintptr_t)d_packed, (u64)(uintptr_t)d_qrows, (u64)(uintptr_t)d_lens, (u64)n_reads, (u64)wpr,
                                               (u64)qstride, (u64)h->reads_seen, (u64)(uintptr_t)h->d_cand,
                                               (u64)(uintptr_t)h->d_bin_flags, (u64)(uintptr_t)h->d_rt_arena, (u64)(uintptr_t)h->d_rt_counts,
                                               (u64)(uintptr_t)h->d_rt_emitted, (u64)h->rt_cap, (u64)h->rt_prod, (u64)h->rt_nw, (u64)paired, (u64)(uintptr_t)h->d_rt_trace, (u64)(uintptr_t)h->d_rt_parked, (u64)h->cap_rt_parked, (u64)h->rt_pf, rt_slice, (u64)h->rt_exam, (u64)h->rt_wo});
    if (gs == 1) { h->reads_seen += n_reads; return MLST_OK; }
    if (phase != 2) { Prof pf(h, 0);
      if (h->sieve_kind == MLST_SIEVE_LDS) {
        dim3 grid(grid_for((n_reads + 1023) / 1024, 1, 256)), block(1024);
#define SIEVE_CASE(W) case W: hipLaunchKernelGGL((k_sieve_q<W, true>), grid, block, 0, h->stream, d_packed, d_lens, (u64)n_reads, E.sieve, E.sieve_mask, E.bitmap, 0u, h->d_cand, E.ctr, paired); break;
        switch (wpr) { SIEVE_CASE(2) SIEVE_CASE(4) SIEVE_CASE(6) SIEVE_CASE(8) SIEVE_CASE(10) SIEVE_CASE(12) SIEVE_CASE(14)
                       SIEVE_CASE(16) SIEVE_CASE(18) SIEVE_CASE(20) default: return fail(h, MLST_E_INVALID, "words_per_read %u unsupported", wpr); }
#undef SIEVE_CASE
      } else if (h->sieve_kind == MLST_SIEVE_ROUTED) {
        const u64 n_flag_words = (n_reads + 31) >> 5;
        for (u64 sl_first = 0; sl_first < n_reads; sl_first += (rt_slice ? rt_slice : n_reads)) {
        const u64 sl_n = rt_slice ? std::min<u64>(rt_slice, n_reads - sl_first) : n_reads;
        const u32* sl_packed = d_packed + (sl_first >> 6) * 64 * wpr; const u16* sl_lens = d_lens + sl_first;
        if (sl_first) hipLaunchKernelGGL(k_rt_reset, dim3(1), dim3(1), 0, h->stream, E.ctr);
        RouteDev R; R.arena = h->d_rt_arena; R.counts = h->d_rt_counts; R.emitted = h->d_rt_emitted; R.filter = h->d_rfilter; R.flags = h->d_bin_flags + (sl_first >> 5); R.trace = h->d_rt_trace; R.parked = h->d_rt_parked; R.parked_cap = h->cap_rt_parked;
        h->rt_last_packed = d_packed;
        R.cap = h->rt_cap; R.n_prod = h->rt_prod; R.tiles_max = h->rt_tiles_max; R.nw = h->rt_nw;
        { const char* e = getenv("MLST_RT_DEBUG"); R.dbg = e ? (u32)atoi(e) : 0u; if (R.dbg & 2u) R.parked_cap = 0; }
        { Prof pa(h, 9);
#define ROUTE_LAUNCH(W, N, WO) hipLaunchKernelGGL((k_route<W, N, WO>), dim3(h->rt_prod), dim3(N * 64), 0, h->stream, sl_packed, sl_lens, (u64)sl_n, R, E.ctr)
#define SIEVE_CASE(W) case W: if (h->rt_nw == 8) { if (h->rt_wo) ROUTE_LAUNCH(W, 8, true); else ROUTE_LAUNCH(W, 8, false); } \
                              else { if (h->rt_wo) ROUTE_LAUNCH(W, 16, true); else ROUTE_LAUNCH(W, 16, false); } break;
        switch (wpr) { SIEVE_CASE(2) SIEVE_CASE(4) SIEVE_CASE(6) SIEVE_CASE(8) SIEVE_CASE(10) SIEVE_CASE(12) SIEVE_CASE(14)
                       SIEVE_CASE(16) SIEVE_CASE(18) SIEVE_CASE(20) default: return fail(h, MLST_E_INVALID, "words_per_read %u unsupported", wpr); }
#undef SIEVE_CASE
#undef ROUTE_LAUNCH
        }
        { Prof pb(h, 10);
#define PROBE_LAUNCH(W, PF, EX) hipLaunchKernelGGL((k_route_probe<W, PF, EX>), dim3(RT_OWNERS), dim3(1024), 0, h->stream, sl_packed, (u64)sl_n, E.sieve, E.sieve_mask, R, E.ctr)
#define SIEVE_CASE(W) case W: if (h->rt_exam == 1) PROBE_LAUNCH(W, 2, 1); else if (h->rt_exam == 2) PROBE_LAUNCH(W, 2, 2); else if (h->rt_exam == 4) PROBE_LAUNCH(W, 2, 4); \
                              else if (h->rt_pf == 4) PROBE_LAUNCH(W, 4, 0); else PROBE_LAUNCH(W, 2, 0); break;
        switch (wpr) { SIEVE_CASE(2) SIEVE_CASE(4) SIEVE_CASE(6) SIEVE_CASE(8) SIEVE_CASE(10) SIEVE_CASE(12) SIEVE_CASE(14)
                       SIEVE_CASE(16) SIEVE_CASE(18) SIEVE_CASE(20) default: return fail(h, MLST_E_INVALID, "words_per_read %u unsupported", wpr); }
#undef SIEVE_CASE
#undef PROBE_LAUNCH
        }
        { Prof pc(h, 11);
#define SIEVE_CASE(W) case W: hipLaunchKernelGGL(k_route_verify<W>, dim3(2048), dim3(256), 0, h->stream, sl_packed, (u64)sl_n, E.sieve, E.sieve_mask, R, E.ctr); break;
        switch (wpr) { SIEVE_CASE(2) SIEVE_CASE(4) SIEVE_CASE(6) SIEVE_CASE(8) SIEVE_CASE(10) SIEVE_CASE(12) SIEVE_CASE(14)
                       SIEVE_CASE(16) SIEVE_CASE(18) SIEVE_CASE(20) default: return fail(h, MLST_E_INVALID, "words_per_read %u unsupported", wpr); }
#undef SIEVE_CASE
        }
        }
        hipLaunchKernelGGL(k_flag_compact, dim3(grid_for((n_flag_words + FLAG_U - 1) / FLAG_U, 1024, 512)), dim3(1024), 0, h->stream, h->d_bin_flags, (u64)n_reads, h->d_cand, E.ctr, paired);
      } else {
        dim3 grid(grid_for((n_reads + 255) / 256, 1, h->sieve_g_blocks)), block(256);
#define SIEVE_CASE(W) case W: hipLaunchKernelGGL((k_sieve_q<W, false>), grid, block, 0, h->stream, d_packed, d_lens, (u64)n_reads, E.sieve, E.sieve_mask, E.gbitmap.p, E.gbitmap_bits, h->d_cand, E.ctr, paired); break;
        switch (wpr) { SIEVE_CASE(2) SIEVE_CASE(4) SIEVE_CASE(6) SIEVE_CASE(8) SIEVE_CASE(10) SIEVE_CASE(12) SIEVE_CASE(14)
                       SIEVE_CASE(16) SIEVE_CASE(18) SIEVE_CASE(20) default: return fail(h, MLST_E_INVALID, "words_per_read %u unsupported", wpr); }
#undef SIEVE_CASE
      }
    }
    if (phase == 1) { HIPCHK(h, hipGetLastError()); return MLST_OK; }
    { Prof pf(h, 1);
      hipLaunchKernelGGL(k_seed, dim3(1024), dim3(256), 0, h->stream, h->d_E, d_packed, d_qrows, d_lens, wpr, qstride, h->reads_seen, h->d_cand, paired, phase == 2 ? 1 : 0);
      hipLaunchKernelGGL(k_retain, dim3(2048), dim3(256), 0, h->stream, h->d_E, d_packed, d_qrows, wpr, qstride, h->reads_seen, phase == 2 ? 1 : 0); }
    if (h->hap_loci) {
      { Prof pf(h, 12);
        if (wpr <= 10) hipLaunchKernelGGL(k_ext_prep<5>, dim3(2048), dim3(256), 0, h->stream, h->d_E, h->kp, h->d_xrec[0], h->cap_xrec[0]);
        else hipLaunchKernelGGL(k_ext_prep<RW / 2>, dim3(2048), dim3(256), 0, h->stream, h->d_E, h->kp, h->d_xrec[1], h->cap_xrec[1]); }
      { Prof pf(h, 2);
        const int thr = h->ext_threads, blocks = h->ext_blocks;
        if (wpr <= 10) hipLaunchKernelGGL(k_extend_160, dim3(blocks), dim3(thr), ext_lds_bytes(h, 0), h->stream, h->d_E, h->kp, h->ext_lds_recs[0], h->ext_acc_cap, h->d_xrec[0], h->cap_xrec[0]);
        else hipLaunchKernelGGL(k_extend_320, dim3(blocks), dim3(std::min(thr, 512)), ext_lds_bytes(h, 1), h->stream, h->d_E, h->kp, h->ext_lds_recs[1], h->ext_acc_cap, h->d_xrec[1], h->cap_xrec[1]); }
    }
    if (h->pair_loci) { Prof pf(h, 2);
      const int thr = h->extp_threads, blocks = h->extp_blocks;
      if (wpr <= 10) hipLaunchKernelGGL(k_extend_pairs_160, dim3(blocks), dim3(thr), 0, h->stream, h->d_E, h->kp);
      else hipLaunchKernelGGL(k_extend_pairs_320, dim3(blocks), dim3(thr), 0, h->stream, h->d_E, h->kp); }
    { Prof pf(h, 3); hipLaunchKernelGGL(k_banded, dim3(1024), dim3(256), 0, h->stream, h->d_E, h->kp); }
    { Prof pf(h, 4); hipLaunchKernelGGL(k_accumulate, dim3(1024), dim3(256), 0, h->stream, h->d_E, h->kp);
      hipLaunchKernelGGL(k_locus, dim3(128), dim3(1024), 0, h->stream, h->d_E, paired); }
    hipLaunchKernelGGL(k_advance, dim3(1), dim3(1), 0, h->stream, E.ctr, n_reads);
    if (gs == 2) { int rc = graph_leave(h, h->g_submit); if (rc) return rc; }
    HIPCHK(h, hipGetLastError());
    h->reads_seen += n_reads;
    return MLST_OK;
}

static int ensure_pack_buffers(mlst_handle* h, u64 n_reads, u32 wpr, u32 qstride) {
    h->last_pack.n_reads = 0; h->last_pack.wpr = h->last_pack.qstride = 0;
    if (h->cap_packed_words < packed_words(n_reads, wpr) + 4 || h->cap_qrow_bytes < n_reads * qstride || h->cap_lens < n_reads + 2) {
        hipStreamSynchronize(h->stream);
        hipFree(h->d_packed); hipFree(h->d_qrows); hipFree(h->d_lens); h->d_packed = nullptr; h->d_qrows = nullptr; h->d_lens = nullptr;
        HIPCHK(h, dmalloc(&h->d_packed, packed_words(n_reads, wpr) + 4)); HIPCHK(h, dmalloc(&h->d_qrows, n_reads * qstride)); HIPCHK(h, dmalloc(&h->d_lens, n_reads + 2));
        h->cap_packed_words = packed_words(n_reads, wpr) + 4; h->cap_qrow_bytes = n_reads * qstride; h->cap_lens = n_reads + 2;
    }
    return MLST_OK;
}

static int h2d_overlapped(mlst_handle* h, void* d_dst, const void* src, u64 n, hipEvent_t before) {
    if (n == 0) return MLST_OK;
    if (!h->copy_stream) HIPCHK(h, hipStreamCreateWithFlags(&h->copy_stream, hipStreamNonBlocking));
    if (!h->stage_done) HIPCHK(h, hipEventCreateWithFlags(&h->stage_done, hipEventDisableTiming));
    if (before) HIPCHK(h, hipStreamWaitEvent(h->copy_stream, before, 0));
    HIPCHK(h, hipMemcpyAsync(d_dst, src, n, hipMemcpyHostToDevice, h->copy_stream));
    HIPCHK(h, hipEventRecord(h->stage_done, h->copy_stream));
    HIPCHK(h, hipStreamWaitEvent(h->stream, h->stage_done, 0));
    HIPCHK(h, hipStreamSynchronize(h->copy_stream));
    return MLST_OK;
}

extern "C" int mlst_submit_reads_device(mlst_handle* h, const uint8_t* d_bases, const uint8_t* d_quals, const uint64_t* d_off,
                                        uint64_t n_reads, uint32_t max_len, int paired) {
    if (!h || !h->have_state) return fail(h, MLST_E_INVALID, "no reference loaded");
    { int rc_ = rn_refuse(h, "mlst_submit_reads_device"); if (rc_) return rc_; }
    { int rc_ = rp_refuse(h, "mlst_submit_reads_device"); if (rc_) return rc_; }
    { int rc_ = ra_refuse(h, "mlst_submit_reads_device"); if (rc_) return rc_; }
    if (bam_is_open(h)) return fail(h, MLST_E_INVALID, "a %s stream is open (its last chunk was not marked final)", bam_kind(h));
    { int rc_ = bz_flush(h); if (rc_) return rc_; }
    hipSetDevice(h->device);
    if (n_reads == 0) return MLST_OK;
    if (max_len > MLST_MAX_READ_LEN) return fail(h, MLST_E_LIMIT, "read longer than %d bases", MLST_MAX_READ_LEN);
    u32 wpr = (max_len + 15) / 16; if (wpr < 2) wpr = 2; wpr = (wpr + 1) & ~1u;
    u32 qstride = (max_len + 7) & ~7u; if (qstride < 8) qstride = 8;
    int rc = ensure_pack_buffers(h, n_reads, wpr, qstride); if (rc) return rc;
    rc = mlst_pack_reads_device(h, d_bases, d_quals, d_off, n_reads, h->d_packed, h->d_qrows, h->d_lens, wpr, qstride); if (rc) return rc;
    return mlst_submit_packed_device(h, h->d_packed, h->d_qrows, h->d_lens, n_reads, wpr, qstride, paired);
}

extern "C" int mlst_submit_reads(mlst_handle* h, const uint8_t* bases, const uint8_t* quals, const uint64_t* off,
                                 uint64_t n_reads, int paired) {
    if (!h || !h->have_state) return fail(h, MLST_E_INVALID, "no reference loaded");
    { int rc_ = rn_refuse(h, "mlst_submit_reads"); if (rc_) return rc_; }
    { int rc_ = rp_refuse(h, "mlst_submit_reads"); if (rc_) return rc_; }
    { int rc_ = ra_refuse(h, "mlst_submit_reads"); if (rc_) return rc_; }
    if (bam_is_open(h)) return fail(h, MLST_E_INVALID, "a %s stream is open (its last chunk was not marked final)", bam_kind(h));
    { int rc_ = bz_flush(h); if (rc_) return rc_; }
    if (n_reads == 0) return MLST_OK;
    if (!bases || !quals || !off) return fail(h, MLST_E_INVALID, "NULL argument");
    hipSetDevice(h->device);
    u64 nbytes = off[n_reads] - off[0]; u32 max_len = 0;
    for (u64 r = 0; r < n_reads; r++) { u64 l = off[r + 1] - off[r]; if (l > MLST_MAX_READ_LEN) return fail(h, MLST_E_LIMIT, "read %llu longer than %d bases", (unsigned long long)r, MLST_MAX_READ_LEN); max_len = std::max(max_len, (u32)l); }
    if (h->cap_in_bytes < nbytes || h->cap_in_reads < n_reads + 1) {
        hipStreamSynchronize(h->stream);
        hipFree(h->d_in_bases); hipFree(h->d_in_quals); hipFree(h->d_in_off); h->d_in_bases = h->d_in_quals = nullptr; h->d_in_off = nullptr;
        HIPCHK(h, dmalloc(&h->d_in_bases, nbytes)); HIPCHK(h, dmalloc(&h->d_in_quals, nbytes)); HIPCHK(h, dmalloc(&h->d_in_off, n_reads + 1));
        h->cap_in_bytes = nbytes; h->cap_in_reads = n_reads + 1;
    }
    hipStreamSynchronize(h->stream);
    std::vector<u64> rel(n_reads + 1); for (u64 r = 0; r <= n_reads; r++) rel[r] = off[r] - off[0];
    HIPCHK(h, hipMemcpyAsync(h->d_in_bases, bases + off[0], nbytes, hipMemcpyHostToDevice, h->stream));
    HIPCHK(h, hipMemcpyAsync(h->d_in_quals, quals + off[0], nbytes, hipMemcpyHostToDevice, h->stream));
    HIPCHK(h, hipMemcpyAsync(h->d_in_off, rel.data(), (n_reads + 1) * 8, hipMemcpyHostToDevice, h->stream));
    HIPCHK(h, hipStreamSynchronize(h->stream));
    return mlst_submit_reads_device(h, h->d_in_bases, h->d_in_quals, (const uint64_t*)h->d_in_off, n_reads, max_len, paired);
}

static int next_text_slot(mlst_handle* h, u64 bytes) {
    const int slot = h->fq_slot ^= 1;
    if (!h->ev_packed[slot]) HIPCHK(h, hipEventCreateWithFlags(&h->ev_packed[slot], hipEventDisableTiming));
    if (h->cap_fq_slot[slot] < bytes) {
        HIPCHK(h, hipEventSynchronize(h->ev_packed[slot]));
        hipFree(h->d_fq_slot[slot]); h->d_fq_slot[slot] = nullptr; HIPCHK(h, dmalloc(&h->d_fq_slot[slot], bytes + 16)); h->cap_fq_slot[slot] = bytes;
        hipFree(h->d_fq_nl[slot]); h->d_fq_nl[slot] = nullptr; HIPCHK(h, dmalloc(&h->d_fq_nl[slot], bytes / 4096 + 8));
    }
    h->d_fq_text = h->d_fq_slot[slot];
    return MLST_OK;
// ... 1812 lines not shown
    if (!h || !out) return fail(h, MLST_E_INVALID, "NULL argument");
    hipSetDevice(h->device);
    { int rc_ = bz_flush(h); if (rc_) return rc_; }
    RaCtr c; memset(&c, 0, sizeof c);
    if (h->ra.on && h->ra.d_ctr) {
        HIPCHK(h, hipMemcpyAsync(&c, h->ra.d_ctr, sizeof c, hipMemcpyDeviceToHost, h->stream));
        HIPCHK(h, hipStreamSynchronize(h->stream));
    }
    out[0] = c.trimmed; out[1] = c.removed; out[2] = c.emptied; out[3] = h->ra.set.K;
    for (int k = 0; k < RA_MAX_ADAPTERS; k++) out[4 + k] = c.per_adapter[k];
    return MLST_OK;
}
extern "C" int mlst_set_export_md(mlst_handle* h, int on) {
    if (!h) return MLST_E_INVALID;
    if (h->at.open && !h->at.reads) return fail(h, MLST_E_INVALID, "an export is open: mlst_set_export_md changes only before mlst_alignments_text_open or behind mlst_alignments_text_close");
    h->at.md = on != 0;
    return MLST_OK;
}
extern "C" int mlst_get_export_md(mlst_handle* h, int* on) {
    if (!h || !on) return fail(h, MLST_E_INVALID, "NULL argument");
    *on = h->at.md ? 1 : 0;
    return MLST_OK;
}
extern "C" int mlst_get_read_names(mlst_handle* h, int* on) {
    if (!h || !on) return fail(h, MLST_E_INVALID, "NULL argument");
    *on = h->rn.on ? 1 : 0;
    return MLST_OK;
}
extern "C" int mlst_read_names_info(mlst_handle* h, uint64_t out[4]) {
    if (!h || !out) return fail(h, MLST_E_INVALID, "NULL argument");
    hipSetDevice(h->device);
    { int rc_ = bz_flush(h); if (rc_) return rc_; }
    RnCtr c; { int rc_ = rn_fetch(h, &c); if (rc_) return rc_; }
    out[0] = c.done - c.fallbacks; out[1] = c.bytes; out[2] = c.fallbacks; out[3] = c.longest;
    return MLST_OK;
}
extern "C" int mlst_read_names_fetch(mlst_handle* h, uint64_t* read_index, uint64_t* off, uint8_t* bytes) {
    if (!h || !read_index || !off || !bytes) return fail(h, MLST_E_INVALID, "NULL argument");
    hipSetDevice(h->device);
    { int rc_ = bz_flush(h); if (rc_) return rc_; }
    RnCtr c; { int rc_ = rn_fetch(h, &c); if (rc_) return rc_; }
    off[0] = 0;
    if (!c.done) return MLST_OK;
    std::vector<u64> ridx(c.done), noff(c.done); std::vector<u16> nlen(c.done); std::vector<u8> arena(c.bytes ? c.bytes : 1);
    HIPCHK(h, hipMemcpyAsync(ridx.data(), h->E.ret_ridx, c.done * 8, hipMemcpyDeviceToHost, h->stream));
    HIPCHK(h, hipMemcpyAsync(noff.data(), h->rn.d_off, c.done * 8, hipMemcpyDeviceToHost, h->stream));
    HIPCHK(h, hipMemcpyAsync(nlen.data(), h->rn.d_len, c.done * 2, hipMemcpyDeviceToHost, h->stream));
    if (c.bytes) HIPCHK(h, hipMemcpyAsync(arena.data(), h->rn.d_bytes, c.bytes, hipMemcpyDeviceToHost, h->stream));
    HIPCHK(h, hipStreamSynchronize(h->stream));
    u64 n = 0, at = 0;
    for (u64 s = 0; s < c.done; s++) {
        if (!nlen[s]) continue;
        if (noff[s] + nlen[s] > c.bytes) return fail(h, MLST_E_HIP, "name arena inconsistent at slot %llu", (unsigned long long)s);
        read_index[n] = ridx[s]; memcpy(bytes + at, arena.data() + noff[s], nlen[s]); at += nlen[s]; off[++n] = at;
    }
    return MLST_OK;
}

extern "C" int mlst_selftest_inflate_canon(const uint8_t* in, uint64_t n_in, uint8_t* out, uint64_t cap, uint64_t* produced, int* left_to_other_kernel) {
    unsigned long long p = 0; bool over = false;
    const int rc = inflate_canon::inflate_raw_host(in, n_in, out, cap, &p, &over);
    if (produced) *produced = p;
    if (left_to_other_kernel) *left_to_other_kernel = over ? 1 : 0;
    return rc;
}
extern "C" int mlst_selftest_inflate(const uint8_t* in, uint64_t n_in, uint8_t* out, uint64_t cap, uint64_t* produced) {
    uint64_t p = 0; mlst_inflate::Tables tb; const int rc = mlst_inflate::inflate_raw(in, n_in, out, cap, &p, &tb);
    if (produced) *produced = p;
    return rc;
}

static int fetch_stats(mlst_handle* h, Counters** c_out) {
    HIPCHK(h, hipMemcpyAsync(h->h_stats, h->d_stats, h->stats_bytes, hipMemcpyDeviceToHost, h->stream));
    HIPCHK(h, hipStreamSynchronize(h->stream));
    Counters* c = (Counters*)(h->h_stats + h->off_ctr);
    if (c_out) *c_out = c;
    if (c->err) return fail(h, MLST_E_CAPACITY, "capacity exceeded (flags 0x%llx: 1=retained reads %llu/%llu, 2=items %llu/%llu, 4=pair results %llu/%llu, 8=banded-SW list); raise mlst_params.max_*",
                            (unsigned long long)c->err, (unsigned long long)c->n_ret, (unsigned long long)h->E.cap_ret, (unsigned long long)c->n_items, (unsigned long long)h->E.cap_items,
                            (unsigned long long)c->n_res, (unsigned long long)h->E.cap_res);
    if (h->rn.on) { RnCtr rnc; int rc_ = rn_fetch(h, &rnc); if (rc_) return rc_; }
    return MLST_OK;
}
static int check_overflow(mlst_handle* h) { return fetch_stats(h, nullptr); }
static void note_sieve_window(mlst_handle* h, const Counters* c) {
    if (!h->window || !c->sv_t1 || !c->sv_t0n) return;
    const u64 t0 = ~c->sv_t0n;
    if (c->sv_t1 > t0) { h->k_ms[7] += (double)(c->sv_t1 - t0) / h->wall_khz; h->k_n[7]++; }
    if (c->sv_wgmax) { h->k_ms[8] += (double)c->sv_wgmax / h->wall_khz; h->k_n[8]++; }
}

extern "C" int mlst_get_allele_stats(mlst_handle* h, int64_t* sum_score, uint32_t* n_hits, uint64_t* locus_len,
                                     uint64_t* locus_first, uint64_t* counters) {
    if (!h || !h->have_state) return fail(h, MLST_E_INVALID, "no reference loaded");
    { int rc_ = bz_flush(h); if (rc_) return rc_; }
    hipSetDevice(h->device);
    Counters* c = nullptr;
    int rc = fetch_stats(h, &c); if (rc) return rc;
    note_sieve_window(h, c);
    if (sum_score) memcpy(sum_score, h->h_stats + h->off_sum, (u64)h->n_alleles * 8);
    if (n_hits) memcpy(n_hits, h->h_stats + h->off_hits, (u64)h->n_alleles * 4);
    if (locus_len) memcpy(locus_len, h->h_stats + h->off_len, (u64)h->n_loci * 8);
    if (locus_first) memcpy(locus_first, h->h_stats + h->off_first, (u64)h->n_loci * 8);
    if (counters) { for (int i = 0; i < MLST_CNT_N; i++) counters[i] = c->cnt[i]; counters[MLST_CNT_RETAINED] = c->n_ret; counters[MLST_CNT_ITEMS] = c->n_items; }
    return MLST_OK;
}

extern "C" int mlst_stats_flat_sizes(mlst_handle* h, uint64_t* n_sum, uint64_t* n_min) {
    if (!h || !h->have_state) return fail(h, MLST_E_INVALID, "no reference loaded");
    if (n_sum) *n_sum = 2ull * h->n_alleles + h->n_loci + MLST_CNT_N;
    if (n_min) *n_min = h->n_loci;
    return MLST_OK;
}
extern "C" int mlst_export_stats_device(mlst_handle* h, int64_t* d_sum, int64_t* d_min) {
    if (!h || !h->have_state) return fail(h, MLST_E_INVALID, "no reference loaded");
    { int rc_ = bz_flush(h); if (rc_) return rc_; }
    hipSetDevice(h->device);
    int rc = check_overflow(h); if (rc) return rc;
    hipLaunchKernelGGL(k_export, dim3(256), dim3(256), 0, h->stream, h->d_E, (long long*)d_sum, (long long*)d_min);
    HIPCHK(h, hipGetLastError()); HIPCHK(h, hipStreamSynchronize(h->stream));
    return MLST_OK;
}
extern "C" int mlst_import_stats_device(mlst_handle* h, const int64_t* d_sum, const int64_t* d_min) {
    if (!h || !h->have_state) return fail(h, MLST_E_INVALID, "no reference loaded");
    hipSetDevice(h->device);
    hipLaunchKernelGGL(k_import, dim3(256), dim3(256), 0, h->stream, h->d_E, (const long long*)d_sum, (const long long*)d_min);
    HIPCHK(h, hipGetLastError()); HIPCHK(h, hipStreamSynchronize(h->stream));
    return MLST_OK;
}

static int ensure_pin(mlst_handle* h, u64 bytes) {
    if (h->cap_pin >= bytes) return MLST_OK;
    hipStreamSynchronize(h->stream);
    if (h->h_pin) hipHostFree(h->h_pin);
    h->h_pin = nullptr; h->cap_pin = 0;
    HIPCHK(h, hipHostMalloc((void**)&h->h_pin, bytes, hipHostMallocDefault));
    h->cap_pin = bytes;
    return MLST_OK;
}

static void launch_pileup(mlst_handle* h, const int* d_chosen, const u64* d_colbase, u32* d_counts) {
    if (h->max_wpr <= 10) hipLaunchKernelGGL(k_pileup_160, dim3(8192), dim3(64), 0, h->stream, h->d_E, h->kp, d_chosen, d_colbase, d_counts, h->d_pl_list);
    else hipLaunchKernelGGL(k_pileup_320, dim3(8192), dim3(64), 0, h->stream, h->d_E, h->kp, d_chosen, d_colbase, d_counts, h->d_pl_list);
}
static int pile_all(mlst_handle* h, const int* d_chosen, const u64* d_colbase, u32* d_counts, u64 ncols) {
    if (!h->depth_cap) {
        launch_pileup(h, d_chosen, d_colbase, d_counts);
        hipLaunchKernelGGL(k_pileup_dp, dim3(64), dim3(64), 0, h->stream, h->d_E, h->kp, d_chosen, d_colbase, d_counts, h->d_pl_list, h->d_tb, (const u64*)nullptr, 0u);
        return MLST_OK;
    }
    if (ncols == 0) return MLST_OK;
    if (h->cap_capcols < ncols) {
        HIPCHK(h, hipStreamSynchronize(h->stream));
        hipFree(h->d_capbuf); h->d_capbuf = nullptr; h->cap_capcols = 0;
        HIPCHK(h, hipMalloc((void**)&h->d_capbuf, ncols * 28));
        h->cap_capcols = ncols;
    }
    u64* lo = h->d_capbuf; u64* hi = lo + h->cap_capcols; u64* thr = hi + h->cap_capcols; u32* cnt = reinterpret_cast<u32*>(thr + h->cap_capcols);
    const unsigned gs = grid_for(ncols, 256, 1024);
    auto pass = [&](u32* out, u32 mode) {
        if (h->max_wpr <= 10) hipLaunchKernelGGL(k_pileup_cap_160, dim3(8192), dim3(64), 0, h->stream, h->d_E, h->kp, d_chosen, d_colbase, out, h->d_pl_list, (const u64*)thr, mode);
        else hipLaunchKernelGGL(k_pileup_cap_320, dim3(8192), dim3(64), 0, h->stream, h->d_E, h->kp, d_chosen, d_colbase, out, h->d_pl_list, (const u64*)thr, mode);
        hipLaunchKernelGGL(k_pileup_dp, dim3(64), dim3(64), 0, h->stream, h->d_E, h->kp, d_chosen, d_colbase, out, h->d_pl_list, h->d_tb, (const u64*)thr, mode);
    };
    hipLaunchKernelGGL(k_cap_search, dim3(gs), dim3(256), 0, h->stream, lo, hi, thr, cnt, (u64)ncols, h->depth_cap, 0);
    for (int it = 0; it < CAP_KEY_BITS; it++) {
        pass(cnt, 1u | (it ? 4u : 0u));
        hipLaunchKernelGGL(k_cap_search, dim3(gs), dim3(256), 0, h->stream, lo, hi, thr, cnt, (u64)ncols, h->depth_cap, it == CAP_KEY_BITS - 1 ? 2 : 1);
    }
    pass(d_counts, 2u | 4u);
    HIPCHK(h, hipGetLastError());
    return MLST_OK;
}
extern "C" int mlst_set_depth_cap(mlst_handle* h, uint32_t cap) {
    if (!h) return MLST_E_INVALID;
    hipSetDevice(h->device);
    HIPCHK(h, hipStreamSynchronize(h->stream));
    h->depth_cap = cap;
    if (h->g_typing.exec) { hipGraphExecDestroy(h->g_typing.exec); h->g_typing.exec = nullptr; }
    h->g_typing.sig.clear();
    return MLST_OK;
}
// ... 496 lines not shown
    if (T.with_names) hipLaunchKernelGGL((k_rt_mark<true>), dim3(gr), dim3(64), 0, h->stream, h->d_E, d_D, R);
    else hipLaunchKernelGGL((k_rt_mark<false>), dim3(gr), dim3(64), 0, h->stream, h->d_E, d_D, R);
    hipLaunchKernelGGL(k_at_local, dim3((unsigned)ng), dim3(1024), 0, h->stream, T.d_wex, n_ent, T.d_gsum);
    hipLaunchKernelGGL(k_fqt_scan, dim3(1), dim3(1024), 0, h->stream, (const FqtDev*)d_F, ng);
    hipLaunchKernelGGL(k_fqt_add, dim3((unsigned)ng), dim3(1024), 0, h->stream, (const FqtDev*)d_F);
    HIPCHK(h, hipGetLastError());
    HIPCHK(h, hipMemcpyAsync(T.h_tot, d_M, sizeof(FqtMeta), hipMemcpyDeviceToHost, h->stream));
    HIPCHK(h, hipMemcpyAsync(T.h_tot + sizeof(FqtMeta), dp_n + 1, 8, hipMemcpyDeviceToHost, h->stream));
    HIPCHK(h, hipStreamSynchronize(h->stream));
    T.round_bytes = ((const FqtMeta*)T.h_tot)->n_windows; memcpy(&T.round_recs, T.h_tot + sizeof(FqtMeta), 8);
    T.ready = true;
    return MLST_OK;
}
extern "C" int mlst_reads_text_next(mlst_handle* h, uint8_t* text, uint64_t cap, uint64_t* n_bytes, uint64_t* n_reads, int* done) {
    if (!h || !h->have_state) return fail(h, MLST_E_INVALID, "no reference loaded");
    auto& T = h->at;
    if (!T.open) return fail(h, MLST_E_INVALID, "no export is open (mlst_reads_text_open comes first)");
    if (!T.reads) return fail(h, MLST_E_INVALID, "the open export is the one of mlst_alignments_text_open: mlst_alignments_text_next takes its rounds");
    { int rc_ = ax_refuse_open(h); if (rc_) return rc_; }
    if (!n_bytes || !n_reads || !done) return fail(h, MLST_E_INVALID, "NULL argument");
    hipSetDevice(h->device);
    *n_bytes = 0; *n_reads = 0;
    while (T.next < T.rounds.size()) {
        if (!T.ready) { int rc_ = rt_prepare(h); if (rc_) return rc_; }
        if (T.round_bytes) break;
        T.next++; T.ready = false;
    }
    if (T.next >= T.rounds.size()) { *done = 1; return MLST_OK; }
    *n_bytes = T.round_bytes; *n_reads = T.round_recs; *done = 0;
    if (!text && !cap) return MLST_OK;
    if (!text) return fail(h, MLST_E_INVALID, "NULL argument");
    if (cap < T.round_bytes) return fail(h, MLST_E_INVALID, "cap %llu is smaller than the round: %llu bytes", (unsigned long long)cap, (unsigned long long)T.round_bytes);
    {
        const AtRound R = T.rounds[T.next];
        if (T.cap_text < T.round_bytes) { hipFree(T.d_text); T.d_text = nullptr; T.cap_text = 0; HIPCHK(h, dmalloc(&T.d_text, T.round_bytes)); T.cap_text = T.round_bytes; }
        const AtDev* d_D = (const AtDev*)T.d_desc;
        const unsigned gr = (unsigned)grid_for(R.r1 - R.r0, 1, 8192);
        if (T.with_names) hipLaunchKernelGGL((k_rt_write<true>), dim3(gr), dim3(64), 0, h->stream, h->d_E, d_D, R, T.d_text);
        else hipLaunchKernelGGL((k_rt_write<false>), dim3(gr), dim3(64), 0, h->stream, h->d_E, d_D, R, T.d_text);
        HIPCHK(h, hipGetLastError());
        HIPCHK(h, hipMemcpyAsync(text, T.d_text, T.round_bytes, hipMemcpyDeviceToHost, h->stream));
        HIPCHK(h, hipStreamSynchronize(h->stream));
    }
    T.next++; T.ready = false;
    while (T.next < T.rounds.size()) {
        int rc_ = rt_prepare(h); if (rc_) return rc_;
        if (T.round_bytes) break;
        T.next++; T.ready = false;
    }
    *done = T.next >= T.rounds.size() ? 1 : 0;
    return MLST_OK;
}
extern "C" int mlst_reads_text_close(mlst_handle* h) { return mlst_alignments_text_close(h); }

extern "C" long long mlst_round_tenths(long long p, uint32_t q) { return q ? round_tenths(p, q) : 0; }

extern "C" int mlst_typing_layout(mlst_handle* h, uint64_t* colbase, uint64_t* total_cols) {
    if (!h || !h->have_state) return fail(h, MLST_E_INVALID, "no reference loaded");
    if (colbase) memcpy(colbase, h->fixed_colbase.data(), ((u64)h->n_loci + 1) * 8);
    if (total_cols) *total_cols = h->fixed_cols;
    return MLST_OK;
}

extern "C" int mlst_typing_choose_pileup(mlst_handle* h, int32_t penalty, uint32_t* d_counts) {
    if (!h || !h->have_state) return fail(h, MLST_E_INVALID, "no reference loaded");
    { int rc_ = bz_flush(h); if (rc_) return rc_; }
    hipSetDevice(h->device);
    const u64 nl = h->n_loci, ncols = h->fixed_cols;
    u32* cnt = d_counts ? d_counts : h->d_auto_counts;
    if (nl) hipLaunchKernelGGL(k_choose, dim3((unsigned)nl), dim3(256), 0, h->stream, h->d_E, h->d_allele_no, (int)penalty, h->d_auto_chosen);
    zero_words(h, cnt, (ncols ? ncols : 1) * 4);
    { Prof pf(h, 5);
      const int rc = pile_all(h, h->d_auto_chosen, h->d_fixed_colbase, cnt, ncols); if (rc) return rc; }
    HIPCHK(h, hipGetLastError());
    return MLST_OK;
}
static int typing_finish_kernels(mlst_handle* h, uint32_t mincov, char none_char, const uint32_t* d_counts) {
    const u64 ncols = h->fixed_cols;
    const u32* cnt = d_counts ? d_counts : h->d_auto_counts;
    if (ncols) hipLaunchKernelGGL(k_consensus, dim3(grid_for(ncols, 256, 256)), dim3(256), 0, h->stream, cnt, (u64)ncols, mincov, (u8)none_char, h->d_auto_letters);
    HIPCHK(h, hipGetLastError());
    return MLST_OK;
}
static int typing_finish_copies(mlst_handle* h) {
    const u64 nl = h->n_loci, ncols = h->fixed_cols;
    u8* hs = h->h_tstats[h->t_slot]; u8* ha = h->h_tauto[h->t_slot];
    HIPCHK(h, hipMemcpyAsync(hs, h->d_stats, h->stats_bytes, hipMemcpyDeviceToHost, h->stream));
    if (nl) HIPCHK(h, hipMemcpyAsync(ha, h->d_auto_chosen, nl * 4, hipMemcpyDeviceToHost, h->stream));
    if (ncols) HIPCHK(h, hipMemcpyAsync(ha + ((nl * 4 + 15) & ~15ull), h->d_auto_letters, ncols, hipMemcpyDeviceToHost, h->stream));
    h->auto_pending = true; h->t_last = h->t_slot; h->t_slot ^= 1;
    return MLST_OK;
}
extern "C" int mlst_typing_finish(mlst_handle* h, uint32_t mincov, char none_char, const uint32_t* d_counts) {
    if (!h || !h->have_state) return fail(h, MLST_E_INVALID, "no reference loaded");
    hipSetDevice(h->device);
    int rc = typing_finish_kernels(h, mincov, none_char, d_counts);
    return rc ? rc : typing_finish_copies(h);
}
extern "C" int mlst_typing_choose_pileup_compact(mlst_handle* h, int32_t penalty, uint32_t* d_counts, uint64_t cap_cols) {
    if (!h || !h->have_state) return fail(h, MLST_E_INVALID, "no reference loaded");
    { int rc_ = bz_flush(h); if (rc_) return rc_; }
    if (!d_counts || cap_cols == 0) return fail(h, MLST_E_INVALID, "mlst_typing_choose_pileup_compact needs a counts buffer");
    hipSetDevice(h->device);
    const u64 nl = h->n_loci;
    if (nl) hipLaunchKernelGGL(k_choose, dim3((unsigned)nl), dim3(256), 0, h->stream, h->d_E, h->d_allele_no, (int)penalty, h->d_auto_chosen);
    hipLaunchKernelGGL(k_layout_compact, dim3(1), dim3(1024), 0, h->stream, h->d_auto_chosen, h->d_fixed_colbase, (u32)nl, (u64)cap_cols,
                       h->d_compact_colbase, h->d_compact_chosen, h->d_compact_info);
    zero_words(h, d_counts, cap_cols * 4);
    { Prof pf(h, 5);
      const int rc = pile_all(h, h->d_compact_chosen, h->d_compact_colbase, d_counts, cap_cols); if (rc) return rc; }
    HIPCHK(h, hipGetLastError());
    return MLST_OK;
}
extern "C" int mlst_typing_finish_compact(mlst_handle* h, uint32_t mincov, char none_char, const uint32_t* d_counts) {
    if (!h || !h->have_state) return fail(h, MLST_E_INVALID, "no reference loaded");
    if (!d_counts) return fail(h, MLST_E_INVALID, "mlst_typing_finish_compact needs the counts buffer");
    hipSetDevice(h->device);
    if (h->n_loci) hipLaunchKernelGGL(k_consensus_expand, dim3((unsigned)h->n_loci), dim3(256), 0, h->stream, d_counts, h->d_compact_chosen, h->d_compact_colbase,
                                      h->d_fixed_colbase, mincov, (u8)none_char, h->d_auto_letters);
    HIPCHK(h, hipGetLastError());
    HIPCHK(h, hipMemcpyAsync(h->h_tauto[h->t_slot] + h->off_compact_info, h->d_compact_info, 16, hipMemcpyDeviceToHost, h->stream));
    h->compact_pending = true;
    return typing_finish_copies(h);
}
extern "C" int mlst_typing_compact_info(mlst_handle* h, uint64_t* need_cols, uint32_t* overflow) {
    if (!h || !h->have_state) return fail(h, MLST_E_INVALID, "no reference loaded");
    if (!h->compact_pending || h->t_ready < 0) return fail(h, MLST_E_INVALID, "mlst_typing_compact_info follows mlst_typing_finish_compact and mlst_typing_fetch");
    const u64* info = (const u64*)(h->h_tauto[h->t_ready] + h->off_compact_info);
    if (need_cols) *need_cols = info[0];
    if (overflow) *overflow = (uint32_t)info[1];
    return MLST_OK;
}
extern "C" int mlst_typing_enqueue(mlst_handle* h, int32_t penalty, uint32_t mincov, char none_char) {
    if (!h || !h->have_state) return fail(h, MLST_E_INVALID, "no reference loaded");
    { int rc_ = bz_flush(h); if (rc_) return rc_; }
    hipSetDevice(h->device);
    const int gs = h->depth_cap ? 0 : graph_enter(h, h->g_typing, {(u64)(u32)penalty, (u64)mincov, (u64)(u8)none_char, (u64)(h->max_wpr <= 10)});
    int rc = MLST_OK;
    if (gs != 1) {
        rc = mlst_typing_choose_pileup(h, penalty, nullptr);
        if (!rc) rc = typing_finish_kernels(h, mincov, none_char, nullptr);
        if (gs == 2) { int rc2 = graph_leave(h, h->g_typing); if (!rc) rc = rc2; }
    }
    return rc ? rc : typing_finish_copies(h);
}

extern "C" int mlst_set_cu_partition(mlst_handle* h, uint32_t part, uint32_t n_parts) {
    if (!h) return MLST_E_INVALID;
    if (n_parts == 0 || part >= n_parts) return fail(h, MLST_E_INVALID, "CU partition %u of %u", part, n_parts);
    if (n_parts == 1 && h->cu_split == 1) return MLST_OK;
    if (h->cu_split == (int)n_parts && h->cu_part == (int)part && h->own_stream) return MLST_OK;
    hipSetDevice(h->device);
    { int rc_ = bz_flush(h); if (rc_) return rc_; }
    drain_events(h);
    HIPCHK(h, hipStreamSynchronize(h->stream));
    int n_cu_i = 0; HIPCHK(h, hipDeviceGetAttribute(&n_cu_i, hipDeviceAttributeMultiprocessorCount, h->device));
    const u32 n_cu = (u32)n_cu_i;
    if (n_parts > n_cu) return fail(h, MLST_E_INVALID, "more CU partitions (%u) than CUs (%u)", n_parts, n_cu);
    hipStream_t ns = nullptr;
    if (n_parts == 1) HIPCHK(h, hipStreamCreate(&ns));
    else {
        std::vector<uint32_t> mask((n_cu + 31) / 32, 0u);
        const u32 lo = (u32)((u64)n_cu * part / n_parts), hi = (u32)((u64)n_cu * (part + 1) / n_parts);
        for (u32 c = lo; c < hi; c++) mask[c >> 5] |= 1u << (c & 31);
        HIPCHK(h, hipExtStreamCreateWithCUMask(&ns, (uint32_t)mask.size(), mask.data()));
    }
    const bool was_own = h->stream == h->own_stream;
    for (auto& e : h->ev_packed) if (e) { hipEventDestroy(e); e = nullptr; }
    if (h->own_stream) hipStreamDestroy(h->own_stream);
    h->own_stream = ns;
    if (was_own) h->stream = ns;
    h->cu_split = (int)n_parts; h->cu_part = (int)part;
    for (auto* g : {&h->g_submit, &h->g_typing}) { if (g->exec) { hipGraphExecDestroy(g->exec); g->exec = nullptr; } g->sig.clear(); }
    return MLST_OK;
}
extern "C" int mlst_get_stream(mlst_handle* h, void** stream) {
    if (!h || !stream) return MLST_E_INVALID;
    *stream = (void*)h->own_stream;
    return MLST_OK;
}
extern "C" int mlst_busy(mlst_handle* h) {
    if (!h) return MLST_E_INVALID;
    hipSetDevice(h->device);
    const hipError_t e = hipStreamQuery(h->stream);
    if (e == hipSuccess) return 0;
    if (e == hipErrorNotReady) return 1;
    return fail(h, MLST_E_HIP, "hipStreamQuery: %s", hipGetErrorString(e));
}

extern "C" int mlst_set_stream(mlst_handle* h, void* stream) {
    if (!h) return MLST_E_INVALID;
    hipSetDevice(h->device);
    { int rc_ = bz_flush(h); if (rc_) return rc_; }
    drain_events(h);
    HIPCHK(h, hipStreamSynchronize(h->stream));
    h->stream = stream ? (hipStream_t)stream : h->own_stream;
    return MLST_OK;
}
extern "C" int mlst_export_stats_device_async(mlst_handle* h, int64_t* d_sum, int64_t* d_min) {
    if (!h || !h->have_state) return fail(h, MLST_E_INVALID, "no reference loaded");
    { int rc_ = bz_flush(h); if (rc_) return rc_; }
    hipSetDevice(h->device);
    hipLaunchKernelGGL(k_export, dim3(256), dim3(256), 0, h->stream, h->d_E, (long long*)d_sum, (long long*)d_min);
    HIPCHK(h, hipGetLastError());
    return MLST_OK;
}
extern "C" int mlst_import_stats_device_async(mlst_handle* h, const int64_t* d_sum, const int64_t* d_min) {
    if (!h || !h->have_state) return fail(h, MLST_E_INVALID, "no reference loaded");
    hipSetDevice(h->device);
    hipLaunchKernelGGL(k_import, dim3(256), dim3(256), 0, h->stream, h->d_E, (const long long*)d_sum, (const long long*)d_min);
    HIPCHK(h, hipGetLastError());
    return MLST_OK;
}

static int typing_hand_over(mlst_handle* h, int slot, int64_t* sum_score, uint32_t* n_hits, uint64_t* locus_len, uint64_t* locus_first,
                            uint64_t* counters, int32_t* chosen, uint8_t* letters) {
    const u8* hs = h->h_tstats[slot]; const u8* ha = h->h_tauto[slot];
    Counters* c = (Counters*)(hs + h->off_ctr);
    if (c->err) return fail(h, MLST_E_CAPACITY, "capacity exceeded (flags 0x%llx); raise mlst_params.max_*", (unsigned long long)c->err);
    const u64 nl = h->n_loci;
    if (sum_score) memcpy(sum_score, hs + h->off_sum, (u64)h->n_alleles * 8);
    if (n_hits) memcpy(n_hits, hs + h->off_hits, (u64)h->n_alleles * 4);
    if (locus_len) memcpy(locus_len, hs + h->off_len, nl * 8);
    if (locus_first) memcpy(locus_first, hs + h->off_first, nl * 8);
    note_sieve_window(h, c);
    if (counters) { for (int i = 0; i < MLST_CNT_N; i++) counters[i] = c->cnt[i]; counters[MLST_CNT_RETAINED] = c->n_ret; counters[MLST_CNT_ITEMS] = c->n_items; }
    if (chosen) memcpy(chosen, ha, nl * 4);
    if (letters) memcpy(letters, ha + ((nl * 4 + 15) & ~15ull), h->fixed_cols);
    return MLST_OK;
}
extern "C" int mlst_typing_fetch(mlst_handle* h, int64_t* sum_score, uint32_t* n_hits, uint64_t* locus_len, uint64_t* locus_first,
                                 uint64_t* counters, int32_t* chosen, uint8_t* letters) {
    if (!h || !h->have_state) return fail(h, MLST_E_INVALID, "no reference loaded");
    if (!h->auto_pending) return fail(h, MLST_E_INVALID, "mlst_typing_fetch without mlst_typing_enqueue");
    hipSetDevice(h->device);
    HIPCHK(h, hipStreamSynchronize(h->stream));
    h->auto_pending = false; h->t_ready = h->t_last;
    return typing_hand_over(h, h->t_ready, sum_score, n_hits, locus_len, locus_first, counters, chosen, letters);
}
extern "C" int mlst_typing_wait(mlst_handle* h) {
    if (!h || !h->have_state) return fail(h, MLST_E_INVALID, "no reference loaded");
    if (!h->auto_pending) return fail(h, MLST_E_INVALID, "mlst_typing_wait without mlst_typing_enqueue");
    hipSetDevice(h->device);
    HIPCHK(h, hipStreamSynchronize(h->stream));
    h->auto_pending = false; h->t_ready = h->t_last;
    return MLST_OK;
}
extern "C" int mlst_typing_fetch_waited(mlst_handle* h, int64_t* sum_score, uint32_t* n_hits, uint64_t* locus_len, uint64_t* locus_first,
                                        uint64_t* counters, int32_t* chosen, uint8_t* letters) {
    if (!h || !h->have_state) return fail(h, MLST_E_INVALID, "no reference loaded");
    if (h->t_ready < 0) return fail(h, MLST_E_INVALID, "mlst_typing_fetch_waited without mlst_typing_wait");
    return typing_hand_over(h, h->t_ready, sum_score, n_hits, locus_len, locus_first, counters, chosen, letters);
}

extern "C" int mlst_hamming_all(mlst_handle* h, uint32_t locus, const uint8_t* query, uint32_t len, uint32_t* dist) {
    if (!h || !h->have_ref) return fail(h, MLST_E_INVALID, "no reference loaded");
    if (locus >= h->n_loci) return fail(h, MLST_E_INVALID, "locus %u out of range", locus);
    hipSetDevice(h->device);
    const LocusDev& L = h->loci[locus];
    if (h->cap_dist < L.n_alleles) { hipFree(h->d_dist); h->d_dist = nullptr; HIPCHK(h, dmalloc(&h->d_dist, (u64)L.n_alleles)); h->cap_dist = L.n_alleles; }
    if (h->cap_query < (u64)len + 1) { hipFree(h->d_query); h->d_query = nullptr; HIPCHK(h, dmalloc(&h->d_query, (u64)len + 1)); h->cap_query = (u64)len + 1; }
    if (len > 60000) return fail(h, MLST_E_LIMIT, "query longer than 60000 bytes");
    if (len) HIPCHK(h, hipMemcpyAsync(h->d_query, query, len, hipMemcpyHostToDevice, h->stream));
    hipLaunchKernelGGL(k_hamming, dim3((L.n_alleles + 255) / 256), dim3(256), len ? len : 1, h->stream, h->d_ascii, h->d_aoff, L.a_begin,
                       L.n_alleles, h->d_query, len, h->d_dist);
    HIPCHK(h, hipGetLastError());
    HIPCHK(h, hipMemcpyAsync(dist, h->d_dist, (u64)L.n_alleles * 4, hipMemcpyDeviceToHost, h->stream));
    HIPCHK(h, hipStreamSynchronize(h->stream));
    return MLST_OK;
}

extern "C" int mlst_hamming_le(mlst_handle* h, uint32_t locus, const uint8_t* query, uint32_t len, uint32_t z,
                               int32_t* first_allele_idx, uint32_t* n_within) {
    if (!h || !h->have_ref) return fail(h, MLST_E_INVALID, "no reference loaded");
    if (locus >= h->n_loci) return fail(h, MLST_E_INVALID, "locus %u out of range", locus);
    std::vector<u32> d(h->loci[locus].n_alleles);
    int rc = mlst_hamming_all(h, locus, query, len, d.data()); if (rc) return rc;
    int first = -1; u32 nw = 0;
    for (u32 a = 0; a < d.size(); a++) if (d[a] <= z) { if (first < 0) first = (int)(h->loci[locus].a_begin + a); nw++; }
    if (first_allele_idx) *first_allele_idx = first;
    if (n_within) *n_within = nw;
    return MLST_OK;
}

extern "C" int mlst_get_items(mlst_handle* h, mlst_item* out, uint64_t cap, uint64_t* n) {
    if (!h || !h->have_state) return fail(h, MLST_E_INVALID, "no reference loaded");
    hipSetDevice(h->device);
    Counters c; HIPCHK(h, hipMemcpy(&c, h->E.ctr, sizeof c, hipMemcpyDeviceToHost));
    u64 ni = std::min<u64>(c.n_items, h->E.cap_items);
    if (n) *n = ni;
    u64 k = std::min<u64>(ni, cap);
    if (!k || !out) return MLST_OK;
    std::vector<ItemDev> items(k); HIPCHK(h, hipMemcpy(items.data(), h->E.items, k * sizeof(ItemDev), hipMemcpyDeviceToHost));
    u64 nr = std::min<u64>(c.n_ret, h->E.cap_ret);
    std::vector<u64> ridx(nr ? nr : 1); if (nr) HIPCHK(h, hipMemcpy(ridx.data(), h->E.ret_ridx, nr * 8, hipMemcpyDeviceToHost));
    for (u64 i = 0; i < k; i++) {
        out[i].read_index = items[i].ret < nr ? ridx[items[i].ret] : ~0ull; out[i].locus = items[i].locus; out[i].diag = items[i].diag;
        out[i].strand = items[i].strand; out[i].votes = items[i].votes; out[i].reserved = 0;
    }
    return MLST_OK;
}

extern "C" int mlst_set_profiling(mlst_handle* h, int on) { if (!h) return MLST_E_INVALID; drain_events(h); h->profiling = on == 1; h->window = on != 0; return MLST_OK; }
extern "C" int mlst_get_kernel_time(mlst_handle* h, int which, double* total_ms, uint64_t* launches) {
    if (!h || which < 0 || which >= 20) return MLST_E_INVALID;
    hipSetDevice(h->device); drain_events(h);
    if (total_ms) *total_ms = h->k_ms[which];
    if (launches) *launches = h->k_n[which];
    return MLST_OK;
}
extern "C" int mlst_reset_kernel_time(mlst_handle* h) { if (!h) return MLST_E_INVALID; drain_events(h); for (int i = 0; i < 20; i++) { h->k_ms[i] = 0; h->k_n[i] = 0; } return MLST_OK; }
extern "C" int mlst_get_index_bytes(mlst_handle* h, uint64_t out[4]) {
    if (!h || !out) return MLST_E_INVALID;
    out[0] = h->bytes_arena + h->bytes_hap; out[1] = h->bytes_sieve; out[2] = h->bytes_table; out[3] = (u64)(h->bitmap_fill * 1e6); return MLST_OK;
}
extern "C" int mlst_get_sieve_info(mlst_handle* h, uint64_t out[4]) {
    if (!h || !out || !h->have_ref) return fail(h, MLST_E_INVALID, "no reference loaded");
    out[0] = (u64)h->sieve_kind; out[1] = h->n_keys; out[2] = h->sieve_chain; out[3] = (u64)h->E.sieve_mask + 1; return MLST_OK;
}
extern "C" int mlst_get_extend_info(mlst_handle* h, uint64_t out[8]) {
    if (!h || !out || !h->have_ref) return fail(h, MLST_E_INVALID, "no reference loaded");
    out[0] = h->n_hap_rec; out[1] = h->bytes_hap; out[2] = h->hap_loci; out[3] = h->hap_win_max[0]; out[4] = h->hap_win_max[1];
    out[5] = h->ext_lds_recs[0] ? (u64)ext_lds_bytes(h, 0) : 0; out[6] = h->ext_lds_recs[1] ? (u64)ext_lds_bytes(h, 1) : 0; out[7] = (u64)h->ext_threads; return MLST_OK;
}
extern "C" void mlst_release_index_cache(void) { std::lock_guard<std::mutex> lk(g_index_mu); g_index_last.reset(); memset(g_index_key, 0, sizeof g_index_key); }
extern "C" int mlst_get_route_trace(mlst_handle* h, uint64_t* out, uint64_t cap_words, uint64_t* n_words) {
    if (!h) return MLST_E_INVALID;
    hipSetDevice(h->device);
    if (n_words) *n_words = 0;
    if (!h->rt_trace_on) { h->rt_trace_on = true; return MLST_OK; }
    if (!h->d_rt_trace || !h->rt_prod) return MLST_OK;
    HIPCHK(h, hipStreamSynchronize(h->stream));
    const u64 n_wg = (u64)h->rt_prod + RT_OWNERS, need = 8 + n_wg * 4;
    if (n_words) *n_words = need;
// ... 116 lines not shown
```

metamlst_amd/engine.py:

```python
from __future__ import annotations

import ctypes as C
import dataclasses
import os

import numpy as np

from .index import AlleleIndex
from .typing import SampleStats

_HERE = os.path.dirname(os.path.abspath(__file__))
LIB_PATH = os.environ.get("MLST_LIB", os.path.join(_HERE, "libmlst_hip.so"))

MLST_CNT_N = 8
CNT_TOTAL_RECORDS, CNT_IGNORED, CNT_READS_SEEN, CNT_CANDIDATES, CNT_RETAINED, CNT_ITEMS, CNT_DP_PAIRS = range(7)
KERNELS = ("sieve", "seed", "extend", "banded_sw", "accumulate", "pileup", "pack", "sieve_inkernel", "sieve_wg_longest",
           "sieve_route", "sieve_probe", "sieve_verify", "extend_prep")
SIEVE_KINDS = ("lds", "global", "binned (round 1, removed)", "routed")


class MlstParams(C.Structure):
    _fields_ = [("minscore", C.c_int32), ("max_xm", C.c_int32), ("min_read_len", C.c_int32),
                ("minqual", C.c_int32), ("mincov", C.c_int32), ("match_bonus", C.c_int32),
                ("mm_max", C.c_int32), ("mm_min", C.c_int32), ("n_penalty", C.c_int32),
                ("gap_open", C.c_int32), ("gap_ext", C.c_int32), ("gbar", C.c_int32),
                ("band_w", C.c_int32), ("gap_trigger_mm", C.c_int32), ("xm_field_quirk", C.c_int32),
                ("gap_trigger_clip", C.c_int32), ("minscore_const", C.c_double), ("minscore_coef", C.c_double),
                ("max_retained_reads", C.c_uint64), ("max_items", C.c_uint64), ("max_pair_results", C.c_uint64)]


class MlstItem(C.Structure):
    _fields_ = [("read_index", C.c_uint64), ("locus", C.c_uint32), ("diag", C.c_int32),
                ("strand", C.c_uint16), ("votes", C.c_uint16), ("reserved", C.c_uint32)]


def default_params() -> MlstParams:
    p = MlstParams()
    p.minscore, p.max_xm, p.min_read_len, p.minqual, p.mincov = 80, 5, 50, 20, 1
    p.match_bonus, p.mm_max, p.mm_min, p.n_penalty = 2, 6, 2, 1
    p.gap_open, p.gap_ext, p.gbar, p.band_w = 5, 3, 4, 8
    p.gap_trigger_mm, p.xm_field_quirk, p.gap_trigger_clip = 12, 1, 8
    p.minscore_const, p.minscore_coef = 20.0, 8.0
    p.max_retained_reads = p.max_items = p.max_pair_results = 0
    return p


class MlstError(RuntimeError):
    pass


@dataclasses.dataclass
class Alignments:
    read_index: np.ndarray
    allele: np.ndarray
    pos0: np.ndarray
    as_: np.ndarray
    xm: np.ndarray
    diag: np.ndarray
    flags: np.ndarray
    cigar_off: np.ndarray
    cigar: np.ndarray
    seq_off: np.ndarray
    seq: np.ndarray
    qual: np.ndarray

    def __len__(self) -> int:
        return len(self.read_index)

    def pileup_arrays(self) -> tuple:
        return (self.allele, self.pos0, self.as_, self.xm, self.cigar_off, self.cigar, self.seq_off, self.seq, self.qual)


class BgzfCrcMismatch(MlstError):

    def __init__(self, text: str, file: int | None):
        super().__init__(text)
        self.file = file


class HostPathNeeded(MlstError):
    """The library's "host path needed: <reason> at record <n>" (mlst_submit_bam_bgzf, mlst_submit_sam_text): the BAM or the SAM
    text holds a record the device does not treat; the caller runs samin.AlignmentSample on the file, which raises or answers as
    the reference would.  Also "... at byte
    <n>" (mlst_submit_fasta): a sequence line only Python's strip() treats; the caller tiles the file with fastq.tile_fasta."""


class CorruptInput(Exception):

    def __init__(self, path: str, message: str):
        super().__init__("%s: %s" % (path, message))
        self.path = path


def crc_checked(paths, fn):
    from .fastq import BgzfCrcError
    try:
        return fn()
# ... 5 lines not shown

_lib = None


def load_library(path: str | None = None):
    global _lib
    if _lib is not None and path is None:
        return _lib
    path = path or LIB_PATH
    try:
        import torch
    except Exception:
        pass
    if not os.path.exists(path):
        raise MlstError("HIP engine library not built: %s is missing (run __graft_entry__.build()); "
                        "there is no CPU fallback" % path)
    lib = C.CDLL(path)
    vp, u8p, u64p, u32p, i32p, i64p, u16p = (C.c_void_p, C.c_void_p, C.c_void_p, C.c_void_p, C.c_void_p, C.c_void_p, C.c_void_p)
    H = C.c_void_p
    sig = {
        "mlst_default_params": (None, [C.POINTER(MlstParams)]),
        "mlst_create": (C.c_int, [C.c_int, C.POINTER(MlstParams), C.POINTER(H)]),
        "mlst_destroy": (None, [H]),
        "mlst_last_error": (C.c_char_p, [H]),
        "mlst_load_reference": (C.c_int, [H, u8p, u64p, u32p, u32p, i32p, C.c_uint32]),
        "mlst_set_reference_cache": (C.c_int, [C.c_char_p]),
        "mlst_submit_reads": (C.c_int, [H, u8p, u8p, u64p, C.c_uint64, C.c_int]),
        "mlst_submit_fastq": (C.c_int, [H, u8p, C.c_uint64, C.c_int, C.POINTER(C.c_uint64)]),
        "mlst_submit_fasta": (C.c_int, [H, u8p, C.c_uint64, C.c_uint32, C.c_uint32, C.c_uint32, C.POINTER(C.c_uint64), C.POINTER(C.c_uint64)]),
        "mlst_submit_fastq_bgzf": (C.c_int, [H, u8p, C.c_uint64, C.c_int, C.c_int, C.POINTER(C.c_uint64), C.POINTER(C.c_uint64)]),
        "mlst_submit_fastq_bgzf_pair": (C.c_int, [H, u8p, C.c_uint64, u8p, C.c_uint64, C.c_int, C.POINTER(C.c_uint64), C.POINTER(C.c_uint64),
                                                  C.POINTER(C.c_uint64)]),
        "mlst_selftest_inflate": (C.c_int, [u8p, C.c_uint64, u8p, C.c_uint64, C.POINTER(C.c_uint64)]),
        "mlst_selftest_inflate_canon": (C.c_int, [u8p, C.c_uint64, u8p, C.c_uint64, C.POINTER(C.c_uint64), C.POINTER(C.c_int)]),
        "mlst_debug_bgzf_walk": (C.c_int, [u8p, C.c_uint64, C.POINTER(C.c_uint64), C.POINTER(C.c_uint64), C.POINTER(C.c_int)]),
        "mlst_selftest_inflate_device": (C.c_int, [H, u8p, C.c_uint64, u8p, C.c_uint64, C.POINTER(C.c_uint64), C.POINTER(C.c_double)]),
        "mlst_selftest_bgzf_crc": (C.c_int, [H, u8p, C.c_uint64, u32p, C.c_uint64, C.POINTER(C.c_uint64), C.POINTER(C.c_double)]),
        "mlst_debug_inflate_paths": (C.c_int, [H, C.POINTER(C.c_uint64), C.POINTER(C.c_uint64)]),
        "mlst_set_bgzf_verify": (C.c_int, [H, C.c_int]),
        "mlst_get_bgzf_verify": (C.c_int, [H, C.POINTER(C.c_int)]),
        "mlst_set_read_tiling": (C.c_int, [H, C.c_uint32, C.c_uint32]),
        "mlst_get_read_tiling": (C.c_int, [H, C.POINTER(C.c_uint32), C.POINTER(C.c_uint32)]),
        "mlst_get_read_tiling_info": (C.c_int, [H, C.POINTER(C.c_uint64)]),
        "mlst_set_read_names": (C.c_int, [H, C.c_int]),
        "mlst_get_read_names": (C.c_int, [H, C.POINTER(C.c_int)]),
        "mlst_set_read_prep": (C.c_int, [H, C.POINTER(C.c_uint32)]),
        "mlst_get_read_prep": (C.c_int, [H, C.POINTER(C.c_uint32)]),
        "mlst_read_prep_info": (C.c_int, [H, C.POINTER(C.c_uint64)]),
        "mlst_set_read_adapters": (C.c_int, [H, C.c_char_p, C.c_uint32, C.c_uint32]),
        "mlst_get_read_adapters": (C.c_int, [H, C.c_char_p, C.c_uint64, C.POINTER(C.c_uint32), C.POINTER(C.c_uint32)]),
        "mlst_get_read_adapters_info": (C.c_int, [H, C.POINTER(C.c_uint64)]),
        "mlst_set_export_md": (C.c_int, [H, C.c_int]),
        "mlst_get_export_md": (C.c_int, [H, C.POINTER(C.c_int)]),
        "mlst_read_names_info": (C.c_int, [H, C.POINTER(C.c_uint64)]),
        "mlst_read_names_fetch": (C.c_int, [H, C.POINTER(C.c_uint64), C.POINTER(C.c_uint64), C.POINTER(C.c_uint8)]),
        "mlst_submit_reads_device": (C.c_int, [H, u8p, u8p, u64p, C.c_uint64, C.c_uint32, C.c_int]),
        "mlst_pack_reads_device": (C.c_int, [H, u8p, u8p, u64p, C.c_uint64, u32p, u8p, u16p, C.c_uint32, C.c_uint32]),
        "mlst_submit_packed_device": (C.c_int, [H, u32p, u8p, u16p, C.c_uint64, C.c_uint32, C.c_uint32, C.c_int]),
        "mlst_pack_fastq_host": (C.c_int, [u8p, C.c_uint64, C.c_uint32, C.c_uint32, u32p, u8p, u16p, C.c_uint64, C.POINTER(C.c_uint64), C.c_int]),
        "mlst_submit_packed_host": (C.c_int, [H, u32p, u8p, u16p, C.c_uint64, C.c_uint32, C.c_uint32, C.c_int]),
        "mlst_alloc_host": (C.c_int, [C.c_uint64, C.POINTER(C.c_void_p)]),
        "mlst_free_host": (C.c_int, [C.c_void_p]),
        "mlst_get_allele_stats": (C.c_int, [H, i64p, u32p, u64p, u64p, u64p]),
        "mlst_stats_flat_sizes": (C.c_int, [H, C.POINTER(C.c_uint64), C.POINTER(C.c_uint64)]),
        "mlst_export_stats_device": (C.c_int, [H, i64p, i64p]),
        "mlst_import_stats_device": (C.c_int, [H, i64p, i64p]),
        "mlst_pileup": (C.c_int, [H, u32p, C.c_uint32, u32p]),
        "mlst_set_depth_cap": (C.c_int, [H, C.c_uint32]),
        "mlst_pileup_device": (C.c_int, [H, u32p, C.c_uint32, u32p, C.POINTER(C.c_uint64)]),
        "mlst_consensus": (C.c_int, [H, u32p, C.c_uint32, C.c_uint32, C.c_char, u8p, u32p]),
        "mlst_consensus_from_counts_device": (C.c_int, [H, u32p, C.c_uint64, C.c_uint32, C.c_char, u8p]),
        "mlst_pileup_alignments": (C.c_int, [H, u32p, C.c_uint32, C.c_uint64, u32p, i32p, i32p, i32p, u64p, u32p, u64p, u8p, u8p,
                                             C.c_int32, C.c_int32, C.c_int32, u32p]),
        "mlst_alignments_export": (C.c_int, [H, u32p, C.c_uint32, C.POINTER(C.c_uint64), C.POINTER(C.c_uint64), C.POINTER(C.c_uint64)]),
        "mlst_alignments_fetch": (C.c_int, [H, u64p, u32p, i32p, i32p, i32p, i32p, u8p, u64p, u32p, u64p, u8p, u8p]),
        "mlst_alignments_text_open": (C.c_int, [H, u8p, u64p, C.c_int, C.c_uint64]),
        "mlst_alignments_text_next": (C.c_int, [H, u8p, C.c_uint64, C.POINTER(C.c_uint64), C.POINTER(C.c_uint64), C.POINTER(C.c_int)]),
        "mlst_alignments_text_close": (C.c_int, [H]),
        "mlst_reads_text_open": (C.c_int, [H, C.c_int, C.c_uint64]),
        "mlst_reads_text_next": (C.c_int, [H, u8p, C.c_uint64, C.POINTER(C.c_uint64), C.POINTER(C.c_uint64), C.POINTER(C.c_int)]),
        "mlst_reads_text_close": (C.c_int, [H]),
        "mlst_typing_layout": (C.c_int, [H, u64p, C.POINTER(C.c_uint64)]),
        "mlst_typing_enqueue": (C.c_int, [H, C.c_int32, C.c_uint32, C.c_char]),
        "mlst_typing_choose_pileup": (C.c_int, [H, C.c_int32, u32p]),
        "mlst_typing_finish": (C.c_int, [H, C.c_uint32, C.c_char, u32p]),
        "mlst_typing_choose_pileup_compact": (C.c_int, [H, C.c_int32, u32p, C.c_uint64]),
        "mlst_typing_finish_compact": (C.c_int, [H, C.c_uint32, C.c_char, u32p]),
        "mlst_typing_compact_info": (C.c_int, [H, C.POINTER(C.c_uint64), C.POINTER(C.c_uint32)]),
        "mlst_set_stream": (C.c_int, [H, C.c_void_p]),
        "mlst_set_cu_partition": (C.c_int, [H, C.c_uint32, C.c_uint32]),
        "mlst_get_stream": (C.c_int, [H, C.POINTER(C.c_void_p)]),
        "mlst_busy": (C.c_int, [H]),
        "mlst_export_stats_device_async": (C.c_int, [H, i64p, i64p]),
        "mlst_import_stats_device_async": (C.c_int, [H, i64p, i64p]),
        "mlst_typing_fetch": (C.c_int, [H, i64p, u32p, u64p, u64p, u64p, i32p, u8p]),
        "mlst_typing_wait": (C.c_int, [H]),
        "mlst_typing_fetch_waited": (C.c_int, [H, i64p, u32p, u64p, u64p, u64p, i32p, u8p]),
        "mlst_round_tenths": (C.c_longlong, [C.c_longlong, C.c_uint32]),
        "mlst_hamming_le": (C.c_int, [H, C.c_uint32, u8p, C.c_uint32, C.c_uint32, C.POINTER(C.c_int32), C.POINTER(C.c_uint32)]),
        "mlst_hamming_all": (C.c_int, [H, C.c_uint32, u8p, C.c_uint32, u32p]),
        "mlst_msa_align": (C.c_int, [H, u8p, u64p, C.c_uint32, C.POINTER(C.c_uint32), C.POINTER(C.c_uint32)]),
        "mlst_msa_fetch": (C.c_int, [H, u8p]),
        "mlst_reset_sample": (C.c_int, [H]),
        "mlst_set_read_index_base": (C.c_int, [H, C.c_uint64]),
        "mlst_get_items": (C.c_int, [H, C.c_void_p, C.c_uint64, C.POINTER(C.c_uint64)]),
        "mlst_set_profiling": (C.c_int, [H, C.c_int]),
        "mlst_get_kernel_time": (C.c_int, [H, C.c_int, C.POINTER(C.c_double), C.POINTER(C.c_uint64)]),
        "mlst_reset_kernel_time": (C.c_int, [H]),
        "mlst_get_index_bytes": (C.c_int, [H, C.POINTER(C.c_uint64)]),
        "mlst_get_sieve_info": (C.c_int, [H, C.POINTER(C.c_uint64)]),
        "mlst_get_extend_info": (C.c_int, [H, C.POINTER(C.c_uint64)]),
        "mlst_release_index_cache": (None, []),
        "mlst_submit_fastq_stream": (C.c_int, [H, u8p, C.c_uint64, C.c_int, C.c_int, C.POINTER(C.c_uint64)]),
        "mlst_submit_fastq_pair": (C.c_int, [H, u8p, C.c_uint64, u8p, C.c_uint64, C.POINTER(C.c_uint64)]),
        "mlst_get_route_trace": (C.c_int, [H, u64p, C.c_uint64, C.POINTER(C.c_uint64)]),
        "mlst_debug_route_realloc": (C.c_int, [H, C.c_uint64]),
        "mlst_debug_route_probe": (C.c_int, [H, C.POINTER(C.c_uint64), u32p, C.c_uint64, C.POINTER(C.c_uint64)]),
        "mlst_bam_open": (C.c_int, [H, C.c_int, i32p, i32p, u8p, C.c_uint32, C.c_uint32, u32p, C.c_uint32]),
        "mlst_submit_bam_bgzf": (C.c_int, [H, u8p, C.c_uint64, C.c_int, C.POINTER(C.c_uint64), C.POINTER(C.c_uint64)]),
        "mlst_bam_set_capacity": (C.c_int, [H, C.c_uint64]),
        "mlst_bam_pileup_fetch": (C.c_int, [H, u32p]),
        "mlst_debug_bam_split": (C.c_int, [H, C.c_uint32, C.POINTER(C.c_uint64)]),
        "mlst_sam_open": (C.c_int, [H, C.c_int, u8p, u64p, i32p, i32p, u8p, C.c_uint32, u32p, C.c_uint32]),
        "mlst_submit_sam_text": (C.c_int, [H, u8p, C.c_uint64, C.c_int, C.POINTER(C.c_uint64)]),
        "mlst_bam_reads_open": (C.c_int, [H, C.c_uint32, C.c_uint32, C.c_int]),
        "mlst_bam_reads_info": (C.c_int, [H, C.POINTER(C.c_uint64)]),
        "mlst_debug_last_packed": (C.c_int, [H, u32p, C.c_uint64, u8p, C.c_uint64, u16p, C.c_uint64, C.POINTER(C.c_uint64)]),
        "mlst_debug_fasta_info": (C.c_int, [H, C.POINTER(C.c_uint64)]),
        "mlst_synchronize": (C.c_int, [H]),
    }
    tolerant = bool(os.environ.get("MLST_LIB_ALLOW_MISSING"))
    for name, (res, args) in sig.items():
        if tolerant and not hasattr(lib, name):
            continue
        fn = getattr(lib, name)
        fn.restype, fn.argtypes = res, args
    lib._mlst_symbols = tuple(sig)
    if path == LIB_PATH:
        _lib = lib
    return lib


def _ptr(a: np.ndarray):
    return a.ctypes.data_as(C.c_void_p)


def pack_fastq_host(text, read_len_max: int = 160, threads: int = 0):
    lib = load_library()
    buf = np.frombuffer(text, dtype=np.uint8) if not isinstance(text, np.ndarray) else text
    wpr = ((int(read_len_max) + 31) // 32) * 2
    qstride = (int(read_len_max) + 7) // 8 * 8
    cap = int(buf.size // 8 + 64)
    cap = min(cap, int(np.count_nonzero(buf[:1 << 20] == 10) * (buf.size / max(1, min(buf.size, 1 << 20))) / 4 * 1.1) + 4096)
    packed = np.zeros(((cap + 63) // 64) * 64 * wpr, np.uint32)
    qrows = np.empty((cap, qstride), np.uint8)
    lens = np.empty(cap, np.uint16)
    n = C.c_uint64()
    rc = lib.mlst_pack_fastq_host(_ptr(buf), buf.size, wpr, qstride, _ptr(packed), _ptr(qrows), _ptr(lens), cap, C.byref(n), int(threads))
    if rc == -4:
        cap = int(buf.size // 8 + 64)
        packed = np.zeros(((cap + 63) // 64) * 64 * wpr, np.uint32); qrows = np.empty((cap, qstride), np.uint8); lens = np.empty(cap, np.uint16)
        rc = lib.mlst_pack_fastq_host(_ptr(buf), buf.size, wpr, qstride, _ptr(packed), _ptr(qrows), _ptr(lens), cap, C.byref(n), int(threads))
    if rc != 0:
        raise MlstError("mlst_pack_fastq_host failed (%d): not whole 4-line FASTQ records, or a read longer than %d bases" % (rc, read_len_max))
    return packed, qrows, lens, int(n.value), wpr, qstride

# ... 549 lines not shown
        s = SampleStats(np.zeros(nA, np.int64), np.zeros(nA, np.uint32), np.zeros(nL, np.uint64),
                        np.zeros(nL, np.uint64), np.zeros(MLST_CNT_N, np.uint64))
        self._check(self.lib.mlst_get_allele_stats(self._h, _ptr(s.sum_score), _ptr(s.n_hits), _ptr(s.locus_len_sum),
                                                   _ptr(s.locus_first), _ptr(s.counters)), "mlst_get_allele_stats")
        return s

    def pileup_alignments(self, chosen, rec_allele, rec_pos0, rec_as, rec_xm, cigar_off, cigar, seq_off, seq, qual,
                          minscore: int = 80, max_xm: int = 5, minqual: int = 20) -> dict[int, np.ndarray]:
        ch = np.ascontiguousarray(chosen, np.uint32)
        lens = [int(self.index.off[a + 1] - self.index.off[a]) for a in ch]
        counts = np.zeros((max(1, sum(lens)), 4), np.uint32)
        arr = [np.ascontiguousarray(x, t) for x, t in ((rec_allele, np.uint32), (rec_pos0, np.int32), (rec_as, np.int32), (rec_xm, np.int32),
                                                       (cigar_off, np.uint64), (cigar, np.uint32), (seq_off, np.uint64), (seq, np.uint8), (qual, np.uint8))]
        self._check(self.lib.mlst_pileup_alignments(self._h, _ptr(ch), len(ch), len(arr[0]), *[_ptr(x) for x in arr],
                                                    int(minscore), int(max_xm), int(minqual), _ptr(counts)), "mlst_pileup_alignments")
        out, at = {}, 0
        for a, L in zip(ch, lens):
            out[int(a)] = counts[at:at + L]
            at += L
        return out

    def export_alignments(self, chosen) -> Alignments:
        ch = np.ascontiguousarray(chosen, np.uint32)
        nr, nc, ns = C.c_uint64(), C.c_uint64(), C.c_uint64()
        self._check(self.lib.mlst_alignments_export(self._h, _ptr(ch) if len(ch) else None, len(ch), C.byref(nr), C.byref(nc), C.byref(ns)),
                    "mlst_alignments_export")
        nr, nc, ns = int(nr.value), int(nc.value), int(ns.value)
        a = Alignments(np.zeros(nr, np.uint64), np.zeros(nr, np.uint32), np.zeros(nr, np.int32), np.zeros(nr, np.int32), np.zeros(nr, np.int32),
                       np.zeros(nr, np.int32), np.zeros(nr, np.uint8), np.zeros(nr + 1, np.uint64), np.zeros(nc, np.uint32),
                       np.zeros(nr + 1, np.uint64), np.zeros(ns, np.uint8), np.zeros(ns, np.uint8))
        self._check(self.lib.mlst_alignments_fetch(self._h, *[_ptr(getattr(a, f.name)) for f in dataclasses.fields(a)]), "mlst_alignments_fetch")
        return a

    def export_sam_text(self, idx, paired: bool = False, round_bytes: int = 0, md: bool = False):
        labels = [idx.label(a).encode() for a in range(idx.n_alleles)]
        name_off = np.zeros(len(labels) + 1, np.uint64)
        name_off[1:] = np.cumsum([len(x) for x in labels], dtype=np.uint64)
        names = np.frombuffer(b"".join(labels) or b"\0", np.uint8)
        set_md = bool(md) and not self.get_export_md()
        if set_md:
            self.lib.mlst_alignments_text_close(self._h)
            self.set_export_md(True)
        try:
            self._check(self.lib.mlst_alignments_text_open(self._h, _ptr(names), _ptr(name_off), int(bool(paired)), int(round_bytes)), "mlst_alignments_text_open")
            buf = None
            nb, nr, done = C.c_uint64(), C.c_uint64(), C.c_int()
            while True:
                self._check(self.lib.mlst_alignments_text_next(self._h, None, 0, C.byref(nb), C.byref(nr), C.byref(done)), "mlst_alignments_text_next")
                if done.value:
                    break
                need = int(nb.value)
                if buf is None or len(buf) < need:
                    buf = pinned_array(max(need, 1 << 16))
                self._check(self.lib.mlst_alignments_text_next(self._h, _ptr(buf), len(buf), C.byref(nb), C.byref(nr), C.byref(done)), "mlst_alignments_text_next")
                if nb.value:
                    yield buf[:int(nb.value)].tobytes()
                if done.value:
                    break
        finally:
            self.lib.mlst_alignments_text_close(self._h)
            if set_md:
                self.set_export_md(False)

    def export_reads_text(self, paired: bool = False, round_bytes: int = 0):
        try:
            self._check(self.lib.mlst_reads_text_open(self._h, int(bool(paired)), int(round_bytes)), "mlst_reads_text_open")
            buf = None
            nb, nr, done = C.c_uint64(), C.c_uint64(), C.c_int()
            while True:
                self._check(self.lib.mlst_reads_text_next(self._h, None, 0, C.byref(nb), C.byref(nr), C.byref(done)), "mlst_reads_text_next")
                if done.value:
                    break
                need = int(nb.value)
                if buf is None or len(buf) < need:
                    buf = pinned_array(max(need, 1 << 16))
                self._check(self.lib.mlst_reads_text_next(self._h, _ptr(buf), len(buf), C.byref(nb), C.byref(nr), C.byref(done)), "mlst_reads_text_next")
                if nb.value:
                    yield buf[:int(nb.value)].tobytes()
                if done.value:
                    break
        finally:
            self.lib.mlst_reads_text_close(self._h)

    def typing_enqueue(self, penalty: int = 100, mincov: int = 1, none_char: str = "N"):
        self._check(self.lib.mlst_typing_enqueue(self._h, int(penalty), int(mincov), none_char.encode()), "mlst_typing_enqueue")

    def typing_choose_pileup(self, penalty: int = 100, d_counts: int = 0):
        self._check(self.lib.mlst_typing_choose_pileup(self._h, int(penalty), d_counts or None), "mlst_typing_choose_pileup")

    def typing_finish(self, mincov: int = 1, none_char: str = "N", d_counts: int = 0):
        self._check(self.lib.mlst_typing_finish(self._h, int(mincov), none_char.encode(), d_counts or None), "mlst_typing_finish")

    def typing_choose_pileup_compact(self, penalty: int, d_counts: int, cap_cols: int):
        self._check(self.lib.mlst_typing_choose_pileup_compact(self._h, int(penalty), d_counts, int(cap_cols)), "mlst_typing_choose_pileup_compact")

    def typing_finish_compact(self, mincov: int, none_char: str, d_counts: int):
        self._check(self.lib.mlst_typing_finish_compact(self._h, int(mincov), none_char.encode(), d_counts), "mlst_typing_finish_compact")

    def typing_compact_info(self) -> tuple[int, bool]:
        need, over = C.c_uint64(), C.c_uint32()
        self._check(self.lib.mlst_typing_compact_info(self._h, C.byref(need), C.byref(over)), "mlst_typing_compact_info")
        return int(need.value), bool(over.value)

    def typing_total_cols(self) -> int:
        tot = C.c_uint64()
        self._check(self.lib.mlst_typing_layout(self._h, None, C.byref(tot)), "mlst_typing_layout")
        return int(tot.value)

    def set_stream(self, stream: int = 0):
        self._check(self.lib.mlst_set_stream(self._h, stream or None), "mlst_set_stream")

    def set_cu_partition(self, part: int, n_parts: int):
        self._check(self.lib.mlst_set_cu_partition(self._h, int(part), int(n_parts)), "mlst_set_cu_partition")

    def own_stream(self) -> int:
        p = C.c_void_p()
        self._check(self.lib.mlst_get_stream(self._h, C.byref(p)), "mlst_get_stream")
        return int(p.value or 0)

    def busy(self) -> bool:
        rc = self.lib.mlst_busy(self._h)
        if rc < 0:
            self._check(rc, "mlst_busy")
        return rc == 1

    def export_stats_device_async(self, d_sum: int, d_min: int):
        self._check(self.lib.mlst_export_stats_device_async(self._h, d_sum, d_min), "mlst_export_stats_device_async")

    def import_stats_device_async(self, d_sum: int, d_min: int):
        self._check(self.lib.mlst_import_stats_device_async(self._h, d_sum, d_min), "mlst_import_stats_device_async")

    def typing_wait(self):
        self._check(self.lib.mlst_typing_wait(self._h), "mlst_typing_wait")

    def typing_fetch(self, per_allele: bool = True, waited: bool = False):
        nA, nL = self.index.n_alleles, self.index.n_loci
        if getattr(self, "_colbase", None) is None or len(self._colbase) != nL + 1:
            self._colbase = np.zeros(nL + 1, np.uint64)
            tot = C.c_uint64()
            self._check(self.lib.mlst_typing_layout(self._h, _ptr(self._colbase), C.byref(tot)), "mlst_typing_layout")
            self._cb_list = [int(x) for x in self._colbase]
        nA_out = nA if per_allele else 0
        s = SampleStats(np.empty(nA_out, np.int64), np.empty(nA_out, np.uint32), np.empty(nL, np.uint64),
                        np.empty(nL, np.uint64), np.empty(MLST_CNT_N, np.uint64))
        chosen = np.empty(nL, np.int32)
        letters = np.empty(self._cb_list[-1], np.uint8)
        fn = self.lib.mlst_typing_fetch_waited if waited else self.lib.mlst_typing_fetch
        self._check(fn(self._h, _ptr(s.sum_score) if per_allele else None, _ptr(s.n_hits) if per_allele else None,
                       _ptr(s.locus_len_sum), _ptr(s.locus_first), _ptr(s.counters), _ptr(chosen), _ptr(letters)), "mlst_typing_fetch")
        raw = letters.tobytes()
        ch, let = {}, {}
        off = self.index.off
        for l in np.nonzero(chosen >= 0)[0].tolist():
            a = int(chosen[l]); ch[l] = a
            b = self._cb_list[l]
            let[a] = raw[b:b + int(off[a + 1] - off[a])]
        return s, ch, let

    def flat_sizes(self) -> tuple[int, int]:
        a, b = C.c_uint64(), C.c_uint64()
        self._check(self.lib.mlst_stats_flat_sizes(self._h, C.byref(a), C.byref(b)), "mlst_stats_flat_sizes")
        return int(a.value), int(b.value)

    def export_stats_device(self, d_sum: int, d_min: int):
        self._check(self.lib.mlst_export_stats_device(self._h, d_sum, d_min), "mlst_export_stats_device")

    def import_stats_device(self, d_sum: int, d_min: int):
        self._check(self.lib.mlst_import_stats_device(self._h, d_sum, d_min), "mlst_import_stats_device")
# ... 138 lines not shown
```

metamlst_amd/pipeline.py:

```python
from __future__ import annotations

import time
from collections import deque
from typing import Callable, Iterable

_END = object()


class TypingPipeline:

    def __init__(self, engines: list, penalty: int = 100, mincov: int = 1, none_char: str = "N", shards: list | None = None,
                 stagger_s: float = 0.0, feed_threads: bool = False):
        if not engines:
            raise ValueError("a pipeline needs at least one engine")
        self.engines = list(engines)
        self.depth = len(self.engines)
        self.penalty, self.mincov, self.none_char = penalty, mincov, none_char
        self.shards = shards
        self.stagger_s = stagger_s
        self.feed_threads = bool(feed_threads) and shards is None
        self._pool = None
        self._pending: dict = {}
        self.partitions = 1
        self.host_ms = {"submit": 0.0, "wait_device": 0.0, "tail": 0.0}

    def place(self, partitions: int) -> None:
        partitions = max(1, min(int(partitions), self.depth))
        for k, e in enumerate(self.engines):
            e.synchronize()
            e.set_cu_partition(k % partitions if partitions > 1 else 0, partitions)
        self.partitions = partitions

    @staticmethod
    def default_partitions(depth: int) -> int:
        return max(p for p in (1, 2, 4, 8) if p <= depth)

    def _launch(self, k: int, job, feed: Callable) -> None:
        t0 = time.perf_counter()
        e = self.engines[k % self.depth]
        if self.shards is not None:
            self.shards[k % self.depth].enqueue(lambda: self._pass1(e, job, feed), penalty=self.penalty)
        elif self.feed_threads:
            if self._pool is None:
                from concurrent.futures import ThreadPoolExecutor
                self._pool = ThreadPoolExecutor(self.depth, thread_name_prefix="feed")
            self._pending[k % self.depth] = self._pool.submit(self._feed_and_enqueue, e, job, feed)
        else:
            self._feed_and_enqueue(e, job, feed)
        self.host_ms["submit"] += (time.perf_counter() - t0) * 1e3

    def _feed_and_enqueue(self, e, job, feed: Callable) -> None:
        self._pass1(e, job, feed)
        e.typing_enqueue(penalty=self.penalty, mincov=self.mincov, none_char=self.none_char)

    def _fed(self, slot: int) -> None:
        fut = self._pending.pop(slot, None)
        if fut is not None:
            fut.result()

    @staticmethod
    def _pass1(e, job, feed: Callable) -> None:
        e.reset_sample()
        feed(e, job)

    def run(self, jobs: Iterable, feed: Callable, tail: Callable, per_allele: bool = True) -> list:
        it = iter(jobs)
        inflight: deque = deque()
        results = []
        k = 0
        for _ in range(self.depth):
            job = next(it, _END)
            if job is _END:
                break
            if k and self.stagger_s and self.partitions > 1:
                time.sleep(self.stagger_s)
            self._launch(k, job, feed)
            inflight.append((k, job))
            k += 1
        while inflight:
            kk, job = inflight.popleft()
            e = self.engines[kk % self.depth]
            t0 = time.perf_counter()
            if self.shards is not None:
                got = self.shards[kk % self.depth].fetch(per_allele)
                self.host_ms["wait_device"] += (time.perf_counter() - t0) * 1e3
                nxt = next(it, _END)
                if nxt is not _END:
                    self._launch(k, nxt, feed)
                    inflight.append((k, nxt))
                    k += 1
            else:
                self._fed(kk % self.depth)
                e.typing_wait()
                self.host_ms["wait_device"] += (time.perf_counter() - t0) * 1e3
                got = e.typing_fetch(per_allele, waited=True) if self.feed_threads else None
                nxt = next(it, _END)
                if nxt is not _END:
                    self._launch(k, nxt, feed)
                    inflight.append((k, nxt))
                    k += 1
                if got is None:
                    got = e.typing_fetch(per_allele, waited=True)
            t1 = time.perf_counter()
            results.append(tail(job, *got))
            self.host_ms["tail"] += (time.perf_counter() - t1) * 1e3
        return results

    def synchronize(self) -> None:
        for slot in list(self._pending):
            self._fed(slot)
        for e in self.engines:
            e.synchronize()

    def stop_feeders(self) -> None:
        if self._pool is not None:
            self._pool.shutdown(wait=True)
            self._pool = None

    def close(self) -> None:
        self.stop_feeders()
        for e in self.engines:
            e.close()


def make_engines(idx, device: int = 0, depth: int = 4, params=None, read_prep: dict | None = None) -> list:
    from .engine import Engine
    engines = [Engine(device, params) for _ in range(depth)]
    for e in engines:
        if read_prep:
            e.set_read_prep(**read_prep)
        e.load_reference(idx)
    return engines
```

Baseline: 21930.

## Allow two queued typing steps per engine and skip per-allele copies

Each engine can now hold two typing steps in flight, each with its own pinned host slot and completion event. The pipeline runner uses this to launch the next sample on the same engine before the previous one is fetched, aiming to remove the device idle gap between consensus and the next routing. The stats buffer is laid out again so per-locus and counter fields sit at the front, which lets an optional flag copy only that front part and skip the per-allele arrays. The accumulator memset is skipped unless the accumulator was left dirty. The new slot bookkeeping and the error fallback in the runner make the code more complex and add risk.

```diff
diff --git a/include/mlst.h b/include/mlst.h
--- a/include/mlst.h
+++ b/include/mlst.h
@@ -183,6 +183,8 @@
 
 int mlst_typing_layout(mlst_handle* h, uint64_t* colbase , uint64_t* total_cols);
 int mlst_typing_enqueue(mlst_handle* h, int32_t penalty, uint32_t mincov, char none_char);
+#define MLST_TYPING_NO_PER_ALLELE 1u
+int mlst_typing_enqueue_ex(mlst_handle* h, int32_t penalty, uint32_t mincov, char none_char, uint32_t flags);
 int mlst_typing_choose_pileup(mlst_handle* h, int32_t penalty, uint32_t* d_counts);
 int mlst_typing_finish(mlst_handle* h, uint32_t mincov, char none_char, const uint32_t* d_counts);
 int mlst_typing_choose_pileup_compact(mlst_handle* h, int32_t penalty, uint32_t* d_counts, uint64_t cap_cols);
diff --git a/metamlst_amd/csrc/mlst_engine.hip b/metamlst_amd/csrc/mlst_engine.hip
--- a/metamlst_amd/csrc/mlst_engine.hip
+++ b/metamlst_amd/csrc/mlst_engine.hip
@@ -3185,16 +3185,19 @@
     u32 depth_cap = 0; u64* d_capbuf = nullptr; u64 cap_capcols = 0;
     u32* d_counts = nullptr; u64 cap_counts = 0;
     int* d_allele_no = nullptr; int* d_auto_chosen = nullptr; u64* d_fixed_colbase = nullptr; std::vector<u64> fixed_colbase; u64 fixed_cols = 0;
-    u32* d_auto_counts = nullptr; u8* d_auto_letters = nullptr; bool auto_pending = false;
-    u8* h_tstats[2] = {nullptr, nullptr}; u8* h_tauto[2] = {nullptr, nullptr}; int t_slot = 0, t_last = 0, t_ready = -1;
-    u64* d_compact_colbase = nullptr; int* d_compact_chosen = nullptr; u64* d_compact_info = nullptr; u64 off_compact_info = 0; bool compact_pending = false;
+    u32* d_auto_counts = nullptr; u8* d_auto_letters = nullptr;
+    struct TSlot { hipEvent_t done = nullptr; bool synced = false ,
+                   no_per_allele = false, compact = false, window = false; };
+    u8* h_tstats[2] = {nullptr, nullptr}; u8* h_tauto[2] = {nullptr, nullptr}; TSlot t_slots[2]; int t_slot = 0, t_pend[2] = {0, 0}, t_npend = 0, t_ready = -1;
+    bool acc_dirty = false;
+    u64* d_compact_colbase = nullptr; int* d_compact_chosen = nullptr; u64* d_compact_info = nullptr; u64 off_compact_info = 0;
     hipStream_t copy_stream = nullptr; hipEvent_t stage_done = nullptr;
     u8* d_fq_slot[2] = {nullptr, nullptr}; u64 cap_fq_slot[2] = {0, 0}; hipEvent_t ev_packed[2] = {nullptr, nullptr}; int fq_slot = 0;
     u32* d_fq_nl[2] = {nullptr, nullptr};
     int cu_split = 1, cu_part = 0;
     hipStream_t own_stream = nullptr;
     u32* d_dist = nullptr; u8* d_query = nullptr; u64 cap_dist = 0, cap_query = 0;
-    u8* d_stats = nullptr; u8* h_stats = nullptr; u64 stats_bytes = 0, stats_zero_bytes = 0;
+    u8* d_stats = nullptr; u8* h_stats = nullptr; u64 stats_bytes = 0, stats_front_bytes = 0;
     u64 off_sum = 0, off_len = 0, off_ctr = 0, off_hits = 0, off_first = 0;
     u8* h_pin = nullptr; u64 cap_pin = 0;
     bool profiling = false;
@@ -3358,7 +3361,7 @@
     hipFree(h->d_allele_no); hipFree(h->d_auto_chosen); hipFree(h->d_fixed_colbase); hipFree(h->d_auto_counts); hipFree(h->d_auto_letters);
     hipFree(h->d_compact_colbase); hipFree(h->d_compact_chosen); hipFree(h->d_compact_info); h->d_compact_colbase = nullptr; h->d_compact_chosen = nullptr; h->d_compact_info = nullptr;
     for (int k = 0; k < 2; k++) if (h->h_tauto[k]) { hipHostFree(h->h_tauto[k]); h->h_tauto[k] = nullptr; }
-    h->d_allele_no = h->d_auto_chosen = nullptr; h->d_fixed_colbase = nullptr; h->d_auto_counts = nullptr; h->d_auto_letters = nullptr; h->auto_pending = false;
+    h->d_allele_no = h->d_auto_chosen = nullptr; h->d_fixed_colbase = nullptr; h->d_auto_counts = nullptr; h->d_auto_letters = nullptr; h->t_npend = 0; h->t_ready = -1;
     h->d_arena = h->d_planes = h->d_nmask = nullptr; h->d_allele_len = nullptr; h->d_allele_locus = nullptr; h->d_loci = nullptr; h->d_sieve = nullptr;
     h->d_keys = nullptr; h->d_vals = h->d_posts = nullptr; h->d_floor = nullptr; h->d_pen = nullptr; h->d_ascii = nullptr; h->d_aoff = nullptr;
     h->have_ref = false;
@@ -3399,6 +3402,7 @@
     bam_drop(h, true);
     for (auto& e : h->events) { hipEventDestroy(e.a); hipEventDestroy(e.b); }
     for (auto& e : h->ev_pool) hipEventDestroy(e);
+    for (auto& s : h->t_slots) if (s.done) hipEventDestroy(s.done);
     free_ref(h); free_state(h);
     if (h->h_pin) hipHostFree(h->h_pin);
     for (int k = 0; k < 2; k++) { if (h->ev_packed[k]) hipEventDestroy(h->ev_packed[k]); }
@@ -3428,9 +3432,9 @@
 }
 
 static int reset_sample_state(mlst_handle* h) {
-    HIPCHK(h, hipMemsetAsync(h->d_stats, 0, h->stats_zero_bytes, h->stream));
-    HIPCHK(h, hipMemsetAsync(h->d_stats + h->off_first, 0xFF, h->stats_bytes - h->off_first, h->stream));
-    if (h->d_acc64 && h->n_alleles) HIPCHK(h, hipMemsetAsync(h->d_acc64, 0, (u64)h->n_alleles * 8, h->stream));
+    HIPCHK(h, hipMemsetAsync(h->d_stats + h->off_first, 0xFF, h->off_len - h->off_first, h->stream));
+    HIPCHK(h, hipMemsetAsync(h->d_stats + h->off_len, 0, h->stats_bytes - h->off_len, h->stream));
+    if (h->acc_dirty && h->d_acc64 && h->n_alleles) { HIPCHK(h, hipMemsetAsync(h->d_acc64, 0, (u64)h->n_alleles * 8, h->stream)); h->acc_dirty = false; }
     if (h->rn.d_ctr) HIPCHK(h, hipMemsetAsync(h->rn.d_ctr, 0, sizeof(RnCtr), h->stream));
     if (h->rp.d_ctr) HIPCHK(h, hipMemsetAsync(h->rp.d_ctr, 0, sizeof(RpCtr), h->stream));
     if (h->ra.d_ctr) HIPCHK(h, hipMemsetAsync(h->ra.d_ctr, 0, sizeof(RaCtr), h->stream));
@@ -3851,17 +3855,19 @@
     E.cap_ret = h->prm.max_retained_reads; E.cap_items = h->prm.max_items; E.cap_res = h->prm.max_pair_results; E.cap_dp = h->prm.max_items * 4;
     {
         u64 o = 0;
-        h->off_sum = o; o += (u64)n_alleles * 8;
+        h->off_first = o; o += (u64)n_loci * 8;
         h->off_len = o; o += (u64)n_loci * 8;
         h->off_ctr = o; o += (sizeof(Counters) + 7) & ~7ull;
+        h->stats_front_bytes = o;
+        o = (o + 255) & ~255ull;
+        h->off_sum = o; o += (u64)n_alleles * 8;
         h->off_hits = o; o += ((u64)n_alleles * 4 + 7) & ~7ull;
-        h->stats_zero_bytes = o;
-        h->off_first = o; o += (u64)n_loci * 8;
-        h->stats_bytes = o ? o : 8;
+        h->stats_bytes = o;
         HIPCHK(h, dmalloc(&h->d_stats, h->stats_bytes));
         HIPCHK(h, hipHostMalloc((void**)&h->h_stats, h->stats_bytes, hipHostMallocDefault));
         for (int k = 0; k < 2; k++) { if (h->h_tstats[k]) hipHostFree(h->h_tstats[k]); HIPCHK(h, hipHostMalloc((void**)&h->h_tstats[k], h->stats_bytes, hipHostMallocDefault)); }
-        h->t_slot = 0; h->t_ready = -1;
+        h->t_slot = 0; h->t_ready = -1; h->t_npend = 0; h->acc_dirty = false;
+        for (auto& s : h->t_slots) if (!s.done) HIPCHK(h, hipEventCreateWithFlags(&s.done, hipEventDisableTiming));
         E.sum_score = (long long*)(h->d_stats + h->off_sum); E.locus_len = (u64*)(h->d_stats + h->off_len);
         E.ctr = (Counters*)(h->d_stats + h->off_ctr); E.n_hits = (u32*)(h->d_stats + h->off_hits);
         E.locus_first = (u64*)(h->d_stats + h->off_first);
@@ -4021,6 +4027,8 @@
                                                (u64)(uintptr_t)h->d_bin_flags, (u64)(uintptr_t)h->d_rt_arena, (u64)(uintptr_t)h->d_rt_counts,
                                                (u64)(uintptr_t)h->d_rt_emitted, (u64)h->rt_cap, (u64)h->rt_prod, (u64)h->rt_nw, (u64)paired, (u64)(uintptr_t)h->d_rt_trace, (u64)(uintptr_t)h->d_rt_parked, (u64)h->cap_rt_parked, (u64)h->rt_pf, rt_slice, (u64)h->rt_exam, (u64)h->rt_wo});
     if (gs == 1) { h->reads_seen += n_reads; return MLST_OK; }
+    const bool acc_was_dirty = h->acc_dirty;
+    h->acc_dirty = true;
     if (phase != 2) { Prof pf(h, 0);
       if (h->sieve_kind == MLST_SIEVE_LDS) {
         dim3 grid(grid_for((n_reads + 1023) / 1024, 1, 256)), block(1024);
@@ -4072,7 +4080,7 @@
 #undef SIEVE_CASE
       }
     }
-    if (phase == 1) { HIPCHK(h, hipGetLastError()); return MLST_OK; }
+    if (phase == 1) { HIPCHK(h, hipGetLastError()); h->acc_dirty = acc_was_dirty; return MLST_OK; }
     { Prof pf(h, 1);
       hipLaunchKernelGGL(k_seed, dim3(1024), dim3(256), 0, h->stream, h->d_E, d_packed, d_qrows, d_lens, wpr, qstride, h->reads_seen, h->d_cand, paired, phase == 2 ? 1 : 0);
       hipLaunchKernelGGL(k_retain, dim3(2048), dim3(256), 0, h->stream, h->d_E, d_packed, d_qrows, wpr, qstride, h->reads_seen, phase == 2 ? 1 : 0); }
@@ -4095,6 +4103,7 @@
     hipLaunchKernelGGL(k_advance, dim3(1), dim3(1), 0, h->stream, E.ctr, n_reads);
     if (gs == 2) { int rc = graph_leave(h, h->g_submit); if (rc) return rc; }
     HIPCHK(h, hipGetLastError());
+    h->acc_dirty = false;
     h->reads_seen += n_reads;
     return MLST_OK;
 }
@@ -6073,8 +6082,8 @@
     return MLST_OK;
 }
 static int check_overflow(mlst_handle* h) { return fetch_stats(h, nullptr); }
-static void note_sieve_window(mlst_handle* h, const Counters* c) {
-    if (!h->window || !c->sv_t1 || !c->sv_t0n) return;
+static void note_sieve_window(mlst_handle* h, const Counters* c, bool window) {
+    if (!window || !c->sv_t1 || !c->sv_t0n) return;
     const u64 t0 = ~c->sv_t0n;
     if (c->sv_t1 > t0) { h->k_ms[7] += (double)(c->sv_t1 - t0) / h->wall_khz; h->k_n[7]++; }
     if (c->sv_wgmax) { h->k_ms[8] += (double)c->sv_wgmax / h->wall_khz; h->k_n[8]++; }
@@ -6087,7 +6096,7 @@
     hipSetDevice(h->device);
     Counters* c = nullptr;
     int rc = fetch_stats(h, &c); if (rc) return rc;
-    note_sieve_window(h, c);
+    note_sieve_window(h, c, h->window);
     if (sum_score) memcpy(sum_score, h->h_stats + h->off_sum, (u64)h->n_alleles * 8);
     if (n_hits) memcpy(n_hits, h->h_stats + h->off_hits, (u64)h->n_alleles * 4);
     if (locus_len) memcpy(locus_len, h->h_stats + h->off_len, (u64)h->n_loci * 8);
@@ -6750,20 +6759,32 @@
     HIPCHK(h, hipGetLastError());
     return MLST_OK;
 }
-static int typing_finish_copies(mlst_handle* h) {
+static int typing_admit(mlst_handle* h, const char* who) {
+    if (h->t_npend >= 2) return fail(h, MLST_E_INVALID, "%s: two typing steps are queued already; mlst_typing_wait for the older one and copy it out first", who);
+    if (h->t_npend && h->profiling) return fail(h, MLST_E_INVALID, "%s: with kernel timing on (mlst_set_profiling(1)) one typing step is queued at a time", who);
+    return MLST_OK;
+}
+static int typing_finish_copies(mlst_handle* h, u32 flags, bool compact) {
     const u64 nl = h->n_loci, ncols = h->fixed_cols;
-    u8* hs = h->h_tstats[h->t_slot]; u8* ha = h->h_tauto[h->t_slot];
-    HIPCHK(h, hipMemcpyAsync(hs, h->d_stats, h->stats_bytes, hipMemcpyDeviceToHost, h->stream));
+    const int slot = h->t_slot; mlst_handle::TSlot& S = h->t_slots[slot];
+    u8* hs = h->h_tstats[slot]; u8* ha = h->h_tauto[slot];
+    const bool front_only = (flags & MLST_TYPING_NO_PER_ALLELE) != 0;
+    HIPCHK(h, hipMemcpyAsync(hs, h->d_stats, front_only ? h->stats_front_bytes : h->stats_bytes, hipMemcpyDeviceToHost, h->stream));
     if (nl) HIPCHK(h, hipMemcpyAsync(ha, h->d_auto_chosen, nl * 4, hipMemcpyDeviceToHost, h->stream));
     if (ncols) HIPCHK(h, hipMemcpyAsync(ha + ((nl * 4 + 15) & ~15ull), h->d_auto_letters, ncols, hipMemcpyDeviceToHost, h->stream));
-    h->auto_pending = true; h->t_last = h->t_slot; h->t_slot ^= 1;
-    return MLST_OK;
-}
+    HIPCHK(h, hipEventRecord(S.done, h->stream));
+    S.synced = false; S.no_per_allele = front_only; S.compact = compact; S.window = h->window;
+    if (h->t_ready == slot) h->t_ready = -1;
+    h->t_pend[h->t_npend++] = slot; h->t_slot ^= 1;
+    return MLST_OK;
+}
+static void typing_all_synced(mlst_handle* h) { for (int i = 0; i < h->t_npend; i++) h->t_slots[h->t_pend[i]].synced = true; }
 extern "C" int mlst_typing_finish(mlst_handle* h, uint32_t mincov, char none_char, const uint32_t* d_counts) {
     if (!h || !h->have_state) return fail(h, MLST_E_INVALID, "no reference loaded");
+    { int rc_ = typing_admit(h, "mlst_typing_finish"); if (rc_) return rc_; }
     hipSetDevice(h->device);
     int rc = typing_finish_kernels(h, mincov, none_char, d_counts);
-    return rc ? rc : typing_finish_copies(h);
+    return rc ? rc : typing_finish_copies(h, 0, false);
 }
 extern "C" int mlst_typing_choose_pileup_compact(mlst_handle* h, int32_t penalty, uint32_t* d_counts, uint64_t cap_cols) {
     if (!h || !h->have_state) return fail(h, MLST_E_INVALID, "no reference loaded");
@@ -6783,24 +6804,27 @@
 extern "C" int mlst_typing_finish_compact(mlst_handle* h, uint32_t mincov, char none_char, const uint32_t* d_counts) {
     if (!h || !h->have_state) return fail(h, MLST_E_INVALID, "no reference loaded");
     if (!d_counts) return fail(h, MLST_E_INVALID, "mlst_typing_finish_compact needs the counts buffer");
+    { int rc_ = typing_admit(h, "mlst_typing_finish_compact"); if (rc_) return rc_; }
     hipSetDevice(h->device);
     if (h->n_loci) hipLaunchKernelGGL(k_consensus_expand, dim3((unsigned)h->n_loci), dim3(256), 0, h->stream, d_counts, h->d_compact_chosen, h->d_compact_colbase,
                                       h->d_fixed_colbase, mincov, (u8)none_char, h->d_auto_letters);
     HIPCHK(h, hipGetLastError());
     HIPCHK(h, hipMemcpyAsync(h->h_tauto[h->t_slot] + h->off_compact_info, h->d_compact_info, 16, hipMemcpyDeviceToHost, h->stream));
-    h->compact_pending = true;
-    return typing_finish_copies(h);
+    return typing_finish_copies(h, 0, true);
 }
 extern "C" int mlst_typing_compact_info(mlst_handle* h, uint64_t* need_cols, uint32_t* overflow) {
     if (!h || !h->have_state) return fail(h, MLST_E_INVALID, "no reference loaded");
-    if (!h->compact_pending || h->t_ready < 0) return fail(h, MLST_E_INVALID, "mlst_typing_compact_info follows mlst_typing_finish_compact and mlst_typing_fetch");
+    if (h->t_ready < 0 || !h->t_slots[h->t_ready].compact) return fail(h, MLST_E_INVALID, "mlst_typing_compact_info follows mlst_typing_finish_compact and mlst_typing_fetch");
     const u64* info = (const u64*)(h->h_tauto[h->t_ready] + h->off_compact_info);
     if (need_cols) *need_cols = info[0];
     if (overflow) *overflow = (uint32_t)info[1];
     return MLST_OK;
 }
-extern "C" int mlst_typing_enqueue(mlst_handle* h, int32_t penalty, uint32_t mincov, char none_char) {
+extern "C" int mlst_typing_enqueue(mlst_handle* h, int32_t penalty, uint32_t mincov, char none_char) { return mlst_typing_enqueue_ex(h, penalty, mincov, none_char, 0); }
+extern "C" int mlst_typing_enqueue_ex(mlst_handle* h, int32_t penalty, uint32_t mincov, char none_char, uint32_t flags) {
     if (!h || !h->have_state) return fail(h, MLST_E_INVALID, "no reference loaded");
+    if (flags & ~(uint32_t)MLST_TYPING_NO_PER_ALLELE) return fail(h, MLST_E_INVALID, "mlst_typing_enqueue_ex: unknown flags 0x%x", flags);
+    { int rc_ = typing_admit(h, "mlst_typing_enqueue"); if (rc_) return rc_; }
     { int rc_ = bz_flush(h); if (rc_) return rc_; }
     hipSetDevice(h->device);
     const int gs = h->depth_cap ? 0 : graph_enter(h, h->g_typing, {(u64)(u32)penalty, (u64)mincov, (u64)(u8)none_char, (u64)(h->max_wpr <= 10)});
@@ -6810,7 +6834,7 @@
         if (!rc) rc = typing_finish_kernels(h, mincov, none_char, nullptr);
         if (gs == 2) { int rc2 = graph_leave(h, h->g_typing); if (!rc) rc = rc2; }
     }
-    return rc ? rc : typing_finish_copies(h);
+    return rc ? rc : typing_finish_copies(h, flags, false);
 }
 
 extern "C" int mlst_set_cu_partition(mlst_handle* h, uint32_t part, uint32_t n_parts) {
@@ -6835,6 +6859,8 @@
     }
     const bool was_own = h->stream == h->own_stream;
     for (auto& e : h->ev_packed) if (e) { hipEventDestroy(e); e = nullptr; }
+    typing_all_synced(h);
+    for (auto& s : h->t_slots) if (s.done) { hipEventDestroy(s.done); s.done = nullptr; HIPCHK(h, hipEventCreateWithFlags(&s.done, hipEventDisableTiming)); }
     if (h->own_stream) hipStreamDestroy(h->own_stream);
     h->own_stream = ns;
     if (was_own) h->stream = ns;
@@ -6862,6 +6888,7 @@
     { int rc_ = bz_flush(h); if (rc_) return rc_; }
     drain_events(h);
     HIPCHK(h, hipStreamSynchronize(h->stream));
+    typing_all_synced(h);
     h->stream = stream ? (hipStream_t)stream : h->own_stream;
     return MLST_OK;
 }
@@ -6883,7 +6910,9 @@
 
 static int typing_hand_over(mlst_handle* h, int slot, int64_t* sum_score, uint32_t* n_hits, uint64_t* locus_len, uint64_t* locus_first,
                             uint64_t* counters, int32_t* chosen, uint8_t* letters) {
-    const u8* hs = h->h_tstats[slot]; const u8* ha = h->h_tauto[slot];
+    const u8* hs = h->h_tstats[slot]; const u8* ha = h->h_tauto[slot]; const mlst_handle::TSlot& S = h->t_slots[slot];
+    if ((sum_score || n_hits) && S.no_per_allele)
+        return fail(h, MLST_E_INVALID, "the step was queued with MLST_TYPING_NO_PER_ALLELE: its sum_score / n_hits were not copied out");
     Counters* c = (Counters*)(hs + h->off_ctr);
     if (c->err) return fail(h, MLST_E_CAPACITY, "capacity exceeded (flags 0x%llx); raise mlst_params.max_*", (unsigned long long)c->err);
     const u64 nl = h->n_loci;
@@ -6891,33 +6920,36 @@
     if (n_hits) memcpy(n_hits, hs + h->off_hits, (u64)h->n_alleles * 4);
     if (locus_len) memcpy(locus_len, hs + h->off_len, nl * 8);
     if (locus_first) memcpy(locus_first, hs + h->off_first, nl * 8);
-    note_sieve_window(h, c);
+    note_sieve_window(h, c, S.window);
     if (counters) { for (int i = 0; i < MLST_CNT_N; i++) counters[i] = c->cnt[i]; counters[MLST_CNT_RETAINED] = c->n_ret; counters[MLST_CNT_ITEMS] = c->n_items; }
     if (chosen) memcpy(chosen, ha, nl * 4);
     if (letters) memcpy(letters, ha + ((nl * 4 + 15) & ~15ull), h->fixed_cols);
     return MLST_OK;
 }
+static int typing_wait_oldest(mlst_handle* h) {
+    const int slot = h->t_pend[0]; mlst_handle::TSlot& S = h->t_slots[slot];
+    if (!S.synced) HIPCHK(h, hipEventSynchronize(S.done));
+    h->t_pend[0] = h->t_pend[1]; h->t_npend--; h->t_ready = slot;
+    return MLST_OK;
+}
 extern "C" int mlst_typing_fetch(mlst_handle* h, int64_t* sum_score, uint32_t* n_hits, uint64_t* locus_len, uint64_t* locus_first,
                                  uint64_t* counters, int32_t* chosen, uint8_t* letters) {
     if (!h || !h->have_state) return fail(h, MLST_E_INVALID, "no reference loaded");
-    if (!h->auto_pending) return fail(h, MLST_E_INVALID, "mlst_typing_fetch without mlst_typing_enqueue");
+    if (!h->t_npend) return fail(h, MLST_E_INVALID, "mlst_typing_fetch without mlst_typing_enqueue");
     hipSetDevice(h->device);
-    HIPCHK(h, hipStreamSynchronize(h->stream));
-    h->auto_pending = false; h->t_ready = h->t_last;
+    { int rc_ = typing_wait_oldest(h); if (rc_) return rc_; }
     return typing_hand_over(h, h->t_ready, sum_score, n_hits, locus_len, locus_first, counters, chosen, letters);
 }
 extern "C" int mlst_typing_wait(mlst_handle* h) {
     if (!h || !h->have_state) return fail(h, MLST_E_INVALID, "no reference loaded");
-    if (!h->auto_pending) return fail(h, MLST_E_INVALID, "mlst_typing_wait without mlst_typing_enqueue");
+    if (!h->t_npend) return fail(h, MLST_E_INVALID, "mlst_typing_wait without mlst_typing_enqueue");
     hipSetDevice(h->device);
-    HIPCHK(h, hipStreamSynchronize(h->stream));
-    h->auto_pending = false; h->t_ready = h->t_last;
-    return MLST_OK;
+    return typing_wait_oldest(h);
 }
 extern "C" int mlst_typing_fetch_waited(mlst_handle* h, int64_t* sum_score, uint32_t* n_hits, uint64_t* locus_len, uint64_t* locus_first,
                                         uint64_t* counters, int32_t* chosen, uint8_t* letters) {
     if (!h || !h->have_state) return fail(h, MLST_E_INVALID, "no reference loaded");
-    if (h->t_ready < 0) return fail(h, MLST_E_INVALID, "mlst_typing_fetch_waited without mlst_typing_wait");
+    if (h->t_ready < 0) return fail(h, MLST_E_INVALID, "mlst_typing_fetch_waited without mlst_typing_wait (or after the enqueue that wrote the waited slot again)");
     return typing_hand_over(h, h->t_ready, sum_score, n_hits, locus_len, locus_first, counters, chosen, letters);
 }
 
diff --git a/metamlst_amd/engine.py b/metamlst_amd/engine.py
--- a/metamlst_amd/engine.py
+++ b/metamlst_amd/engine.py
@@ -13,6 +13,7 @@
 LIB_PATH = os.environ.get("MLST_LIB", os.path.join(_HERE, "libmlst_hip.so"))
 
 MLST_CNT_N = 8
+MLST_TYPING_NO_PER_ALLELE = 1
 CNT_TOTAL_RECORDS, CNT_IGNORED, CNT_READS_SEEN, CNT_CANDIDATES, CNT_RETAINED, CNT_ITEMS, CNT_DP_PAIRS = range(7)
 KERNELS = ("sieve", "seed", "extend", "banded_sw", "accumulate", "pileup", "pack", "sieve_inkernel", "sieve_wg_longest",
            "sieve_route", "sieve_probe", "sieve_verify", "extend_prep")
@@ -184,6 +185,7 @@
         "mlst_reads_text_close": (C.c_int, [H]),
         "mlst_typing_layout": (C.c_int, [H, u64p, C.POINTER(C.c_uint64)]),
         "mlst_typing_enqueue": (C.c_int, [H, C.c_int32, C.c_uint32, C.c_char]),
+        "mlst_typing_enqueue_ex": (C.c_int, [H, C.c_int32, C.c_uint32, C.c_char, C.c_uint32]),
         "mlst_typing_choose_pileup": (C.c_int, [H, C.c_int32, u32p]),
         "mlst_typing_finish": (C.c_int, [H, C.c_uint32, C.c_char, u32p]),
         "mlst_typing_choose_pileup_compact": (C.c_int, [H, C.c_int32, u32p, C.c_uint64]),
@@ -899,8 +901,12 @@
         finally:
             self.lib.mlst_reads_text_close(self._h)
 
-    def typing_enqueue(self, penalty: int = 100, mincov: int = 1, none_char: str = "N"):
-        self._check(self.lib.mlst_typing_enqueue(self._h, int(penalty), int(mincov), none_char.encode()), "mlst_typing_enqueue")
+    def typing_enqueue(self, penalty: int = 100, mincov: int = 1, none_char: str = "N", per_allele: bool = True):
+        if per_allele:
+            self._check(self.lib.mlst_typing_enqueue(self._h, int(penalty), int(mincov), none_char.encode()), "mlst_typing_enqueue")
+        else:
+            self._check(self.lib.mlst_typing_enqueue_ex(self._h, int(penalty), int(mincov), none_char.encode(), MLST_TYPING_NO_PER_ALLELE),
+                        "mlst_typing_enqueue_ex")
 
     def typing_choose_pileup(self, penalty: int = 100, d_counts: int = 0):
         self._check(self.lib.mlst_typing_choose_pileup(self._h, int(penalty), d_counts or None), "mlst_typing_choose_pileup")
diff --git a/metamlst_amd/pipeline.py b/metamlst_amd/pipeline.py
--- a/metamlst_amd/pipeline.py
+++ b/metamlst_amd/pipeline.py
@@ -64,6 +64,8 @@
         feed(e, job)
 
     def run(self, jobs: Iterable, feed: Callable, tail: Callable, per_allele: bool = True) -> list:
+        if self.shards is None and not self.feed_threads:
+            return self._run_two_queued(jobs, feed, tail, per_allele)
         it = iter(jobs)
         inflight: deque = deque()
         results = []
@@ -106,6 +108,74 @@
             self.host_ms["tail"] += (time.perf_counter() - t1) * 1e3
         return results
 
+    def _run_two_queued(self, jobs: Iterable, feed: Callable, tail: Callable, per_allele: bool) -> list:
+        from .engine import MlstError
+        it = iter(jobs)
+        inflight: deque = deque()
+        queued = [0] * self.depth
+        held: set = set()
+        ahead = 2
+        results = []
+        k = 0
+
+        def launch(k: int, job) -> None:
+            nonlocal ahead
+            t0 = time.perf_counter()
+            slot = k % self.depth
+            e = self.engines[slot]
+            self._pass1(e, job, feed)
+            try:
+                self._enqueue(e, per_allele)
+                queued[slot] += 1
+            except MlstError:
+                if not queued[slot]:
+                    raise
+                held.add(slot)
+                ahead = 1
+            inflight.append((k, job))
+            self.host_ms["submit"] += (time.perf_counter() - t0) * 1e3
+
+        for rnd in range(2):
+            for _ in range(self.depth):
+                if ahead <= rnd:
+                    break
+                job = next(it, _END)
+                if job is _END:
+                    break
+                if rnd == 0 and k and self.stagger_s and self.partitions > 1:
+                    time.sleep(self.stagger_s)
+                launch(k, job)
+                k += 1
+        while inflight:
+            kk, job = inflight.popleft()
+            slot = kk % self.depth
+            e = self.engines[slot]
+            t0 = time.perf_counter()
+            e.typing_wait()
+            self.host_ms["wait_device"] += (time.perf_counter() - t0) * 1e3
+            got = e.typing_fetch(per_allele, waited=True)
+            queued[slot] -= 1
+            if slot in held:
+                t0 = time.perf_counter()
+                held.discard(slot)
+                self._enqueue(e, per_allele)
+                queued[slot] += 1
+                self.host_ms["submit"] += (time.perf_counter() - t0) * 1e3
+            while it is not None and (k % self.depth) not in held and queued[k % self.depth] < ahead:
+                nxt = next(it, _END)
+                if nxt is _END:
+                    it = None
+                    break
+                launch(k, nxt)
+                k += 1
+            t1 = time.perf_counter()
+            results.append(tail(job, *got))
+            self.host_ms["tail"] += (time.perf_counter() - t1) * 1e3
+        return results
+
+    def _enqueue(self, e, per_allele: bool) -> None:
+        e.typing_enqueue(penalty=self.penalty, mincov=self.mincov, none_char=self.none_char, per_allele=per_allele)
+
     def synchronize(self) -> None:
         for slot in list(self._pending):
             self._fed(slot)
diff --git a/profiles/round9/engine_gap.py b/profiles/round9/engine_gap.py
--- /dev/null
+++ b/profiles/round9/engine_gap.py
@@ -0,0 +1,43 @@
+#!/usr/bin/env python3
+import collections
+import csv
+import statistics
+import sys
+
+path = sys.argv[1]
+last = int(sys.argv[2]) if len(sys.argv) > 2 else 4
+per_stream = collections.defaultdict(list)
+with open(path, newline="") as f:
+    for r in csv.DictReader(f):
+        per_stream[(r["Queue_Id"], r.get("Stream_Id", "0"))].append((int(r["Start_Timestamp"]), int(r["End_Timestamp"]), r["Kernel_Name"].split("(")[0]))
+rows = []
+t_end = max(k[1] for ks in per_stream.values() for k in ks)
+for sid, ks in sorted(per_stream.items()):
+    ks.sort()
+    if not any("k_route<" in n for _, _, n in ks) or ks[-1][1] < t_end - 50_000_000:
+        continue
+    is_route = lambda n: "k_route<" in n and "k_route_" not in n
+    trans = []
+    i_cons = None
+    for i, (s, e, n) in enumerate(ks):
+        if "k_consensus" in n:
+            i_cons = i
+        elif is_route(n) and i_cons is not None:
+            between = ks[i_cons + 1:i]
+            prev_route = next((ks[j][0] for j in range(i_cons, -1, -1) if is_route(ks[j][2])), None)
+            trans.append({"gap": s - ks[i_cons][1], "busy": sum(b[1] - b[0] for b in between), "n": len(between),
+                          "names": collections.Counter(b[2] for b in between), "cycle": (s - prev_route) if prev_route else None})
+            i_cons = None
+    for t in trans[-last:]:
+        rows.append((sid, t))
+print("stream (queue, id) | gap us | copy+fill kernels in it: n, us | cycle ms | gap / cycle")
+for sid, t in rows:
+    print("%-12s | %8.1f | %2d %7.1f | %7.3f | %5.2f %%" % ("%s,%s" % sid, t["gap"] / 1e3, t["n"], t["busy"] / 1e3, (t["cycle"] or 0) / 1e6, 100.0 * t["gap"] / t["cycle"] if t["cycle"] else 0.0))
+if rows:
+    gaps = [t["gap"] / 1e3 for _, t in rows]; busy = [t["busy"] / 1e3 for _, t in rows]; cyc = [t["cycle"] / 1e6 for _, t in rows if t["cycle"]]
+    names = collections.Counter()
+    for _, t in rows:
+        names.update(t["names"])
+    print("transitions %d: gap median %.1f us (min %.1f, max %.1f), copy+fill kernels in it median %.1f us, cycle median %.3f ms, median gap / median cycle %.2f %%"
+          % (len(rows), statistics.median(gaps), min(gaps), max(gaps), statistics.median(busy), statistics.median(cyc), 0.1 * statistics.median(gaps) / statistics.median(cyc)))
+    print("kernels inside the gaps:", dict(names))
```

Measured after the change: 21860. Within noise of the previous version (-0.3%).
